# pouryashirazian/FemBrain

Measured on AMD Instinct MI355X. Metric: FEM steps/sec (assemble+PCG) at 1M tets, higher is better.
Workload: dtype f64 arithmetic / f32 stored matrix

## Files before the change

### fembrain_amd/csrc/fem_handle.h

```cpp
#pragma once
#include "comm.h"
#include "common.h"
#include "fem_kernels.h"
#include "fem_plan.h"
#include "plan_device.h"
#include "renumber.h"
#include "delta.h"
#include "subdivide.h"
#include "surface.h"
#include "haptic.h"

namespace fb {

struct PipeKernel;

struct PersistState {
  int pipe_mir_knob = -1;
  int persist_fallbacks = 0;
  int persist_launches = 0;
  int persist_rearms = 0;
  double persist_seconds = 0;
  long long persist_iterations = 0;

  int pipe_lines_nodes = 0;
  double pipe_gather_lines[2] = {0, 0};

  bool persist = false;
  int persist_blocks = 0, persist_waves = 0;
  const PipeKernel* kernel = nullptr;
  int pipe_rows = 1;
  int pipe_wmax = 0;
  int pipe_slots_dealt = 0;
  int pipe_help_waves = 0;
  int pipe_n_help = 0, pipe_help_tasks = 0;
  bool pipe_xyz = false;
  int pipe_plain_local = 0;
  int pipe_flag_extra = 0;
  int pipe_max_producers = 0;
  bool pipe_stats_pending = false;
  int pipe_timing_level = 0;
  long long persist_timeout_ticks = 0;
  bool persist_broken = false;
  int rearm_after = 32, clean_solves = 0;
  bool shard_persist = false;
  int sh_n_proxy = 1, sh_relief = 0;
  char* sbox = nullptr;
  void* sbox_opened[kP2PMaxRanks] = {nullptr};
  long long sbox_halo_cap = 0;
  int pipe_mir_got[3] = {0, 0, 0};
  bool pipe_mir_pending = false;

  DevBuf<int> pipe_wg_first;
  std::vector<int> pipe_wg_first_host;
  DevBuf<int4> pipe_mir;
  DevBuf<int> sh_halo_off, sh_row_send_off, sh_row_send_rank, sh_row_send_pos, sh_proxy_wg, sh_wg_duty;
  DevBuf<int2> sh_wg_range;
  DevBuf<unsigned int> sh_wg_send_mask;
  DevBuf<int4> pipe_tasks;
  DevBuf<long long> persist_timing;
  DevBuf<unsigned short> pipe_mir_addr;
  DevBuf<int2> pipe_mir_wg;
  DevBuf<int> pipe_mir_pool;
  DevBuf<int> pipe_mir_stats;
  DevBuf<unsigned long long> pipe_lines;
  DevBuf<unsigned long long> pipe_post;
  DevBuf<unsigned int> pipe_flags;
  DevBuf<int> pipe_prod, pipe_prod_count, pipe_prod_xcd;
  DevBuf<unsigned int> pipe_xcc;
  DevBuf<double> pipe_planes, pipe_z, pipe_s, pipe_state;
  DevBuf<int> pipe_owner, pipe_stats;
  DevBuf<unsigned int> pipe_mask;
  DevBuf<char*> sbox_peers;
  DevBuf<int> sh_peer_seg, sh_n_senders;

  void reset_plan(int rearm) {
    persist = false;
    kernel = nullptr;
    pipe_mir.release(); pipe_mir_pending = false;
    pipe_mir_got[0] = pipe_mir_got[1] = pipe_mir_got[2] = 0;
    shard_persist = false;
    persist_broken = false;
    pipe_stats_pending = false;
    clean_solves = 0;
    rearm_after = rearm;
    sh_halo_off.release(); sh_row_send_off.release(); sh_row_send_rank.release(); sh_row_send_pos.release(); sh_proxy_wg.release();
    sh_wg_duty.release(); sh_wg_range.release(); sh_wg_send_mask.release();
    pipe_wg_first_host.clear();
    pipe_wg_first.release();
  }
};

}

using namespace fb;

struct fb_fem_s {
  fb_fem_params prm;
  hipStream_t stream = nullptr;
  hipStream_t side = nullptr;
  hipEvent_t ev_side[2] = {nullptr, nullptr};
  fb_comm_s* comm = nullptr;
  P2P* p2p = nullptr;
  int xch_mode = FB_XCH_COLLECTIVE;
  DevBuf<int> send_off_dev, halo_off_dev;
  DevBuf<unsigned char> slice_halo;
  FemPlan plan;
  double lambda = 0, mu = 0;
  int grid = 8;
  bool f64 = false;
  DevBuf<int4> tets;
  DevBuf<double> x0, rest, fe;
  DevBuf<char> rec;
  DevBuf<char> kcorr;
  DevBuf<double> qacc, q1, qvel1, qacc1;
  double nm_beta = 0.25, nm_gamma = 0.5, nm_eps = 1e-6;
  int nm_max_newton = 1;
  bool pcg_warm = false;
  DevBuf<int> slice_off, colidx, slot_coff, slot_ccnt, send_local;
  DevBuf<uint32_t> contrib;
  DevBuf<short> coldelta;
  int c16 = 0;
  DevBuf<int> halo_base;
  PlanWorkspace plan_ws;
  MeshDelta delta;
  CutWork cut;
  DevBuf<double> carry;
  SurfaceWork surf;
  HapticWork hap;
  std::vector<int> fixed_caller;
  DevBuf<int4> tets_next, tets_caller;
  DevBuf<double> x0_next;
  DevBuf<int> map_next_a, map_next_b;
  int last_resync_path = FB_RESYNC_FULL;
  int ren_nodes_at_build = 0;
  DevBuf<int> flat_flag;
  DevBuf<int> inc_off;
  DevBuf<uint32_t> inc, inc_slot;
  bool asm_tets = false;
  int asm_lds = 0, asm_grid = 0, asm_max_width = 0;
  int asm_wide = 0;
  int asm_wide_slots = 0, asm_wide_grid = 0;
  DevBuf<int> wide_list;
  DevBuf<double> res_all;
  DevBuf<double> wide_scratch;
  bool asm_staged = false;
  int asm_lds_st = 0, asm_grid_st = 0;
  bool mass_valid = false;
  Renumbering ren;
  DevBuf<double> xyz_in;
  DevBuf<double> io;
  bool x0_ready = false;
  bool masks_ready = false;
  std::vector<int> l2c;
  unsigned long long order_sum = 0;
  int n_cu_device = 256;
  bool shard_auto_on = false;
  int shard_vote_neighbours = 0;
  DevBuf<int> fixed_stage;
  std::vector<int> c_bptr, c_bcol, c_src;
  bool caller_pattern = false;
  std::vector<double> x0_stage;
  DevBuf<int> d_bptr, d_bcol, d_blk_slot;
  DevBuf<unsigned int> d_ucnt;
  bool span_stale = false;
  bool csr_ready = false;
  bool device_plan = false, host_pattern = true;
  DevBuf<uint8_t> dofmask;
  DevBuf<uint8_t> nodemask;
  DevBuf<char> vals;
  DevBuf<char> dlo;
  DevBuf<double> mblk;
  DevBuf<float> volf;
  DevBuf<double> invblk;
  DevBuf<double> q, qvel, fext, fint, rhs, x, r, d, Ad, invdiag, tmp, sendbuf;
  DevBuf<double> part_a, part_b, part_c, scal;
  DevBuf<CGState> st;
  DevBuf<int> counter;
  CGState* st_host = nullptr;
  hipEvent_t ev[3] = {nullptr, nullptr, nullptr}, ev_batch[2] = {nullptr, nullptr};
  bool system_valid = false;
  bool poisoned = false;
  double last_assembly_s = 0, last_solve_s = 0;
  int split = 0;
  int sgrid = 8;
  bool spmv_nt = false;
  int vgrid = 8;
  hipGraphExec_t batch_graph = nullptr;
  const double* graph_rhs = nullptr;
  bool use_graph = true;
  bool literal_now = false, graph_literal = false;
  fb::PersistState ps;
  int last_pcg_path = 0;
  int cu_limit = 0;
  hipEvent_t ev_p[2] = {nullptr, nullptr};
};

namespace fb {

inline SellView sell_view(const fb_fem_s* h) {
  SellView sv;
  sv.slice_off = h->slice_off.p; sv.colidx = h->colidx.p; sv.n_slices = h->plan.n_slices; sv.n_owned = h->plan.n_owned;
  sv.coldelta = h->c16 ? h->coldelta.p : nullptr;
  sv.halo_base = h->c16 == 2 ? h->halo_base.p : nullptr;
  return sv;
}

#define CHECK_HANDLE(h)                                                                                                        \
  if (!(h)) return fail(FB_EINVAL, "null FEM handle");                                                                        \
  if ((h)->poisoned) return fail(FB_EINVAL, "handle unusable after a failed fb_fem_resync: re-sync it with a valid mesh or destroy it"); \
  FB_HIP(hipSetDevice((h)->prm.device))

constexpr int kZeroMax = 24;
struct ZeroBatch {
  unsigned int* p[kZeroMax]; unsigned long long end[kZeroMax]; unsigned int tail_words[kZeroMax]; int n = 0;
  hipStream_t s;
  int rc = FB_OK;
  explicit ZeroBatch(hipStream_t stream) : s(stream) {}
  void add(void* p, size_t bytes);
  template <typename T>
  void add(DevBuf<T>& b) { add(b.p, b.n * sizeof(T)); }
  int flush();
};

int assemble_system(fb_fem_s* h);

bool auto_matrix_f64(const fb_fem_s* h, int n_nodes, int n_ranks);
int setup_persist(fb_fem_s* h);
int attach_pipe_shard(fb_fem_s* h);
void release_shard_persist(fb_fem_s* h);
void read_persist_timeout(fb_fem_s* h);
int launch_pipe(fb_fem_s* h, const double* b, int start, int n_iters, double eps, int max_iter);
void print_pipe_timing(fb_fem_s* h);
// ... 4 lines not shown
```

### fembrain_amd/csrc/fem_persist.hip

```cpp
#include <cmath>
#include <cstring>

#include "fem_handle.h"
#include "pcg_pipe.hip.h"
#include "pcg_pipe2.hip.h"
#include "pcg_pipe_plan.h"

using namespace fb;

namespace fb {

struct PipeKernel {
  int rows;
  bool c16;
  int wmax, klt;
  bool timing, shard, bj, help, xyz;
  const void* fn;
};

namespace {

#define FB_PIPE1(C16, WMAX, KLT, TIMING, SHARD, BJ, HELP, XYZ) \
  {1, C16, WMAX, KLT, TIMING, SHARD, BJ, HELP, XYZ, (const void*)k_pcg_pipe<float, C16, WMAX, KLT, TIMING, SHARD, BJ, HELP, XYZ>}
#define FB_PIPE2(C16, SHARD, XYZ) {2, C16, 12, kPipe2Klt, false, SHARD, false, false, XYZ, (const void*)k_pcg_pipe2<C16, SHARD, XYZ>}
const PipeKernel kPipeKernels[] = {
    FB_PIPE1(true, 5, 16, false, false, false, false, false),  FB_PIPE1(false, 5, 16, false, false, false, false, false),
    FB_PIPE1(true, 8, 8, false, false, false, false, false),   FB_PIPE1(false, 8, 8, false, false, false, false, false),
    FB_PIPE1(true, 12, 6, false, false, false, false, false),  FB_PIPE1(false, 12, 6, false, false, false, false, false),
    FB_PIPE1(true, 12, 7, false, false, false, false, false),  FB_PIPE1(false, 12, 7, false, false, false, false, false),
    FB_PIPE1(true, 5, 16, true, false, false, false, false),
    FB_PIPE1(true, 8, 8, true, false, false, false, false),    FB_PIPE1(false, 8, 8, true, false, false, false, false),
    FB_PIPE1(true, 12, 6, true, false, false, false, false),   FB_PIPE1(false, 12, 6, true, false, false, false, false),
    FB_PIPE1(false, 8, 8, false, true, false, false, false),   FB_PIPE1(false, 12, 6, false, true, false, false, false),
    FB_PIPE1(true, 8, 8, false, false, true, false, false),    FB_PIPE1(false, 8, 8, false, false, true, false, false),
    FB_PIPE1(true, 12, 6, false, false, true, false, false),   FB_PIPE1(false, 12, 6, false, false, true, false, false),
    FB_PIPE1(true, 12, 6, false, false, false, true, false),   FB_PIPE1(false, 12, 6, false, false, false, true, false),
    FB_PIPE1(true, 12, 6, false, false, false, true, true),    FB_PIPE1(false, 12, 6, false, false, false, true, true),
    FB_PIPE1(true, 12, 6, true, false, false, true, false),    FB_PIPE1(false, 12, 6, true, false, false, true, false),
    FB_PIPE1(true, 12, 6, true, false, false, true, true),     FB_PIPE1(false, 12, 6, true, false, false, true, true),
    FB_PIPE2(true, false, false),  FB_PIPE2(false, false, false),  FB_PIPE2(true, false, true),  FB_PIPE2(false, false, true),
    FB_PIPE2(false, true, false),
};
#undef FB_PIPE2
#undef FB_PIPE1
static_assert(sizeof(double) * kPipeSyncDoubles + (size_t)kPipeMaxWaves * 2 * kPipe2LdsWordsPerRow * 64 * 4 <= 160 * 1024, "LDS budget of k_pcg_pipe2");

int env_int(const char* name, int unset) {
  const char* e = getenv(name);
  return e ? atoi(e) : unset;
}

PersistKnobs read_persist_knobs() {
  PersistKnobs k;
  k.pcg_persist = env_int("FEMBRAIN_PCG_PERSIST", -1);
  k.min_waves = env_int("FEMBRAIN_PERSIST_MIN_WAVES", 2);
  k.rows2 = env_int("FEMBRAIN_PERSIST_ROWS", 0) == 2;
  k.rearm = std::max(0, env_int("FEMBRAIN_PERSIST_REARM", 32));
  k.timing = getenv("FEMBRAIN_PERSIST_TIMING") ? std::max(1, env_int("FEMBRAIN_PERSIST_TIMING", 1)) : 0;
  k.poll_all = env_int("FEMBRAIN_PERSIST_POLL_ALL", 0) != 0;
  k.sharded = env_int("FEMBRAIN_SHARDED_PERSIST", 0) != 0;
  k.shard_relief = env_int("FEMBRAIN_SHARD_RELIEF", -1);
  k.balance = env_int("FEMBRAIN_PIPE_BALANCE", -1);
  k.small = env_int("FEMBRAIN_PIPE_SMALL", 0) != 0;
  k.klt7 = env_int("FEMBRAIN_PIPE_KLT7", 1) != 0;
  k.helpers = env_int("FEMBRAIN_PIPE_HELPERS", -1);
  k.help_minlen = env_int("FEMBRAIN_PIPE_HELP_MINLEN", 16);
  k.xyz = env_int("FEMBRAIN_PIPE_XYZ", -1);
  k.lds_by_width = env_int("FEMBRAIN_PIPE_LDS_BY_WIDTH", 0) != 0;
  k.lds_cap = getenv("FEMBRAIN_PIPE_LDS_CAP") ? std::max(1, env_int("FEMBRAIN_PIPE_LDS_CAP", 1)) : 0;
  k.plain_stores = env_int("FEMBRAIN_PIPE_PLAIN_STORES", -1);
  k.mirror = env_int("FEMBRAIN_PIPE_MIRROR", 1) != 0;
  k.verbose = getenv("FEMBRAIN_TIMING") != nullptr;
  return k;
}

int resolve_pipe_kernel(fb_fem_s* h, const PersistKnobs& kn) {
  PersistState& ps = h->ps;
  PipeKernel want;
  want.rows = ps.pipe_rows;
  want.shard = ps.shard_persist;
  want.bj = h->prm.pcg_variant == FB_PCG_BLOCK_JACOBI;
  want.help = ps.pipe_tasks.p != nullptr;
  want.xyz = ps.pipe_xyz;
  want.c16 = !want.shard && h->c16 != 0;
  want.timing = ps.persist_timing.p != nullptr && want.rows == 1;
  if (want.bj && want.timing) return fail(FB_EINVAL, "FEMBRAIN_PERSIST_TIMING is built for the Jacobi kernel");
  const bool klt7 = kn.klt7 && want.rows == 1 && ps.pipe_wmax == 12 && !want.shard && !want.bj && !want.help && !want.timing &&
                    (ps.persist_waves == 9 || ps.persist_waves == 10);
  want.wmax = ps.pipe_wmax;
  want.klt = want.rows == 2 ? kPipe2Klt : (want.wmax == 5 ? 16 : (want.wmax == 8 ? 8 : (klt7 ? 7 : 6)));
  ps.kernel = nullptr;
  for (const PipeKernel& k : kPipeKernels)
    if (k.rows == want.rows && k.c16 == want.c16 && k.wmax == want.wmax && k.klt == want.klt && k.timing == want.timing && k.shard == want.shard && k.bj == want.bj &&
        k.help == want.help && k.xyz == want.xyz)
      ps.kernel = &k;
  if (!ps.kernel) return fail(FB_EINVAL, "FEMBRAIN_PERSIST_TIMING is built for one row per lane: (12, 6) and (5, 16) with 16-bit column words, (8, 8)");
  return FB_OK;
}

int setup_persist_shard_local(fb_fem_s* h, int nb, int w, const PersistKnobs& kn) {
  const FemPlan& P = h->plan;
  PersistState& ps = h->ps;
  hipStream_t s = h->stream;
  const int R = P.n_ranks;
  if (R > kP2PMaxRanks) return FB_OK;
  FB_TRY(ps.sh_halo_off.upload(P.halo_off, s));
  DevBuf<int4> range;
  FB_TRY(range.alloc((size_t)std::max(1, P.n_slices)));
  hipLaunchKernelGGL(k_slice_colrange_shard, dim3(ceil_div(std::max(1, P.n_slices), kWavesPerBlock)), dim3(kBlock), 0, s, P.n_slices, P.n_owned, R, h->slice_off.p,
                     h->colidx.p, ps.sh_halo_off.p, range.p);
  FB_HIP(hipGetLastError());
  std::vector<int4> rg((size_t)std::max(1, P.n_slices));
  FB_TRY(range.download(rg.data(), rg.size(), s));
  std::vector<int2> wg_range;
  w = shard_deal(rg, P.n_slices, nb, w, kn, &wg_range, &ps.sh_relief);
  ps.pipe_rows = w < kPipeMaxWaves ? 1 : 2;
  ps.pipe_wmax = ps.pipe_rows == 2 ? 12 : (w < 8 ? 8 : 12);
  ps.pipe_slots_dealt = ps.pipe_rows == 2 ? std::min(kPipe2Klt, pipe2_lds_slots(w, false) / std::max(w, 1)) : std::min(ps.pipe_wmax == 8 ? 8 : 6, pipe_lds_slots(false) / std::max(w, 1));
  ps.persist_blocks = nb; ps.persist_waves = w;
  ps.pipe_flag_extra = kP2PMaxRanks * kShardProxies;
  FB_TRY(ps.sh_wg_range.upload(wg_range, s));
  FB_TRY(ps.pipe_post.alloc((size_t)2 * nb * 4));
  FB_TRY(ps.pipe_post.zero(s));
  FB_TRY(ps.pipe_flags.alloc((size_t)nb + ps.pipe_flag_extra + 16));
  FB_TRY(ps.pipe_flags.zero(s));
  const size_t n_pad = (size_t)ceil_div(P.n_local, 64) * 64, nv = (size_t)3 * P.n_local + 2;
  FB_TRY(ps.pipe_planes.alloc(2 * 3 * n_pad));
  FB_TRY(ps.pipe_planes.zero(s));
  FB_TRY(ps.pipe_z.alloc(nv));
  FB_TRY(ps.pipe_s.alloc(nv));
  FB_TRY(ps.pipe_state.alloc(2));
  FB_TRY(ps.pipe_state.zero(s));
  ps.persist_timing.release();
  std::vector<int> owner((size_t)P.n_slices, 0);
  for (int b = 0; b < nb; b++)
    for (int k = 0; k < wg_range[b].y; k++) owner[wg_range[b].x + k] = b;
  const ShardSendLists sl = shard_send_lists(P, owner, nb);
  FB_TRY(ps.sh_row_send_off.upload(sl.row_off, s));
  FB_TRY(ps.sh_row_send_rank.upload(sl.row_rank, s));
  FB_TRY(ps.sh_row_send_pos.upload(sl.row_pos, s));
  FB_TRY(ps.sh_wg_send_mask.upload(sl.wg_mask, s));
  std::vector<int> proxy, duty, prod, cnt, far((size_t)nb, 1);
  const int K = shard_proxies(P, nb, &proxy, &duty);
  ps.sh_n_proxy = K;
  FB_TRY(ps.sh_proxy_wg.upload(proxy, s));
  FB_TRY(ps.sh_wg_duty.upload(duty, s));
  ps.pipe_max_producers = shard_producers(rg, wg_range, owner, proxy, P.n_slices, nb, R, K, &prod, &cnt);
  ps.pipe_stats_pending = false;
  FB_TRY(ps.pipe_prod.upload(prod, s));
  FB_TRY(ps.pipe_prod_count.upload(cnt, s));
  FB_TRY(ps.pipe_prod_xcd.upload(far, s));
  ps.pipe_plain_local = 0;
  ps.shard_persist = true;
  return resolve_pipe_kernel(h, kn);
}

int setup_pipe_mirror(fb_fem_s* h) {
  const FemPlan& P = h->plan;
  PersistState& ps = h->ps;
  hipStream_t s = h->stream;
  const PipeKernel& K = *ps.kernel;
  ps.pipe_mir_pending = false;
  ps.pipe_mir_got[0] = ps.pipe_mir_got[1] = ps.pipe_mir_got[2] = 0;
  if (ps.pipe_mir_knob == 0 || K.rows != 1 || K.wmax != 12 || K.shard || K.help || K.bj || ps.pipe_xyz || P.n_slices <= 0) {
    ps.pipe_mir.release(); ps.pipe_mir_addr.release(); ps.pipe_mir_wg.release(); ps.pipe_mir_pool.release();
    return FB_OK;
  }
  const int nb = ps.persist_blocks;
  FB_TRY(ps.pipe_mir.alloc((size_t)nb * kMirWaves));
  FB_TRY(ps.pipe_mir_addr.alloc((size_t)P.n_slices * kMirMax * 64));
  FB_TRY(ps.pipe_mir_wg.alloc((size_t)nb));
  FB_TRY(ps.pipe_mir_pool.alloc((size_t)nb * kMirPoolMax));
  FB_TRY(ps.pipe_mir_stats.alloc(3));
  FB_HIP(hipMemsetAsync(ps.pipe_mir_stats.p, 0, 2 * sizeof(int), s));
  FB_HIP(hipMemsetAsync(ps.pipe_mir_stats.p + 2, 0x7f, sizeof(int), s));
  hipLaunchKernelGGL(k_pipe_mirror_plan, dim3(nb), dim3(64 * kMirWaves), 0, s, P.n_slices, P.n_owned, h->slice_off.p, h->colidx.p, ps.pipe_wg_first.p, K.klt,
                     h->c16 ? 1 : 0, ps.pipe_mir.p, ps.pipe_mir_addr.p, ps.pipe_mir_pool.p, ps.pipe_mir_wg.p, ps.pipe_mir_stats.p);
  FB_HIP(hipGetLastError());
  ps.pipe_mir_pending = true;
  return FB_OK;
}

int pipe_layout(fb_fem_s* h, const PersistKnobs& kn, bool* want_xyz) {
  const FemPlan& P = h->plan;
  PersistState& ps = h->ps;
  hipStream_t s = h->stream;
  *want_xyz = false;
  const bool keep_lines = ps.pipe_gather_lines[0] > 0.0 && ps.pipe_lines_nodes > 0 && std::abs(P.n_local - ps.pipe_lines_nodes) * 20 <= ps.pipe_lines_nodes;
  bool measured = keep_lines;
  if (!keep_lines) {
    ps.pipe_gather_lines[0] = ps.pipe_gather_lines[1] = 0.0;
    ps.pipe_lines_nodes = 0;
    if (P.n_local >= (1 << 24) || !h->colidx.p) return FB_OK;
    FB_TRY(ps.pipe_lines.alloc(4));
    FB_HIP(hipMemsetAsync(ps.pipe_lines.p, 0, 4 * sizeof(unsigned long long), s));
    hipLaunchKernelGGL(k_gather_lines, dim3(64), dim3(256), 0, s, P.n_slices, 8, h->slice_off.p, h->colidx.p, ps.pipe_lines.p);
    FB_HIP(hipGetLastError());
    unsigned long long got[3] = {0, 0, 0};
    FB_HIP(hipMemcpyAsync(got, ps.pipe_lines.p, sizeof got, hipMemcpyDeviceToHost, s));
    FB_HIP(hipStreamSynchronize(s));
    measured = got[2] != 0;
    if (measured) { ps.pipe_gather_lines[0] = 3.0 * (double)got[0] / (double)got[2]; ps.pipe_gather_lines[1] = (double)got[1] / (double)got[2]; ps.pipe_lines_nodes = P.n_local; }
  }
  *want_xyz = P.n_local < (1 << 24) &&
              (kn.xyz >= 0 ? kn.xyz != 0 : (measured && ps.pipe_gather_lines[0] >= 30.0 && ps.pipe_gather_lines[0] >= 1.5 * ps.pipe_gather_lines[1]));
  return FB_OK;
}

int setup_pipe_tasks(fb_fem_s* h, int nb, int w, const PersistKnobs& kn) {
  const FemPlan& P = h->plan;
  PersistState& ps = h->ps;
  int mx = 0;
  long long tot = 0;
  for (int sl = 0; sl < P.n_slices; sl++) { const int wd = P.slice_off[sl + 1] - P.slice_off[sl]; mx = std::max(mx, wd); tot += wd; }
  const double mean = P.n_slices ? (double)tot / P.n_slices : 0.0;
  const bool want_h = ps.pipe_rows == 1 && (kn.helpers >= 0 ? kn.helpers != 0 : (mx > 24 && (double)mx >= 1.5 * mean));
  bool want_xyz = false;
  FB_TRY(pipe_layout(h, kn, &want_xyz));
  ps.pipe_xyz = ps.pipe_rows == 2 && want_xyz;
  if (ps.pipe_rows != 1 || !(want_h || want_xyz) || w > kPipeMaxWaves) return FB_OK;
  const PipeTasks T = pipe_help_tasks(P.slice_off.data(), P.n_slices, ps.pipe_wg_first_host.empty() ? nullptr : ps.pipe_wg_first_host.data(), nb, w, h->c16 != 0, want_h,
                                      want_xyz, kn);
  if (!(T.all > 0 || T.deepest > 6 || want_xyz || kn.helpers == 2)) return FB_OK;
  FB_TRY(ps.pipe_tasks.upload(T.tasks, h->stream));
  ps.pipe_wmax = 12;
  ps.pipe_slots_dealt = T.deepest;
  ps.pipe_help_waves = T.help_waves; ps.pipe_n_help = T.most; ps.pipe_help_tasks = T.all;
  ps.pipe_xyz = want_xyz;
  if (kn.verbose) fprintf(stderr, "[fembrain] persistent solver: %d helper tasks (at most %d per workgroup), widest slice %d slots, mean %.1f, up to %d slots of a slice in LDS; a slot's gathers touch %.1f lines in planes, %.1f node by node -> %s\n", T.all, T.most, mx, mean, T.deepest, ps.pipe_gather_lines[0], ps.pipe_gather_lines[1], want_xyz ? "node by node" : "planes");
  return FB_OK;
}

int alloc_persist(fb_fem_s* h, int nb, const PersistKnobs& kn) {
  const FemPlan& P = h->plan;
  PersistState& ps = h->ps;
  hipStream_t s = h->stream;
  ZeroBatch zb(s);
  FB_TRY(ps.pipe_post.alloc((size_t)2 * nb * 4));
  zb.add(ps.pipe_post);
  ps.pipe_flag_extra = P.n_ranks > 1 ? kP2PMaxRanks : 0;
  FB_TRY(ps.pipe_flags.alloc((size_t)nb + ps.pipe_flag_extra + 16));
  zb.add(ps.pipe_flags);
  const size_t n_pad = (size_t)P.n_slices * 64, nv = (size_t)3 * P.n_local + 2;
  FB_TRY(ps.pipe_planes.alloc(2 * 3 * n_pad));
  zb.add(ps.pipe_planes);
  FB_TRY(ps.pipe_z.alloc(nv));
  FB_TRY(ps.pipe_s.alloc(nv));
  FB_TRY(ps.pipe_state.alloc(2));
  zb.add(ps.pipe_state);
  if (kn.timing) {
    FB_TRY(ps.persist_timing.alloc((size_t)nb * kPipeMaxWaves * kPipeTimingSlots));
    FB_TRY(ps.persist_timing.zero(s));
  } else {
    ps.persist_timing.release();
  }
  static_assert(kPipeMaxBlocks <= 256, "k_slice_producers holds 256 workgroups in its 8 mask words");
  FB_TRY(ps.pipe_owner.alloc((size_t)std::max(1, P.n_slices)));
  FB_TRY(ps.pipe_mask.alloc((size_t)std::max(1, P.n_slices) * 8));
  FB_TRY(ps.pipe_prod.alloc((size_t)nb * kPipeMaxProducers));
  FB_TRY(ps.pipe_prod_count.alloc((size_t)nb));
  FB_TRY(ps.pipe_prod_xcd.alloc((size_t)nb));
  FB_TRY(ps.pipe_stats.alloc(2));
  zb.add(ps.pipe_stats);
  FB_TRY(zb.flush());
  hipLaunchKernelGGL(k_slice_owner, dim3(ceil_div(nb, kBlock)), dim3(kBlock), 0, s, P.n_slices, nb, ps.pipe_wg_first.p, ps.pipe_owner.p);
  hipLaunchKernelGGL(k_slice_producers, dim3(ceil_div(std::max(1, P.n_slices), kWavesPerBlock)), dim3(kBlock), 0, s, P.n_slices, P.n_owned, h->slice_off.p, h->colidx.p,
                     ps.pipe_owner.p, ps.pipe_mask.p);
  hipLaunchKernelGGL(k_wg_producers, dim3(ceil_div(nb, kBlock)), dim3(kBlock), 0, s, P.n_slices, nb, ps.pipe_wg_first.p, ps.pipe_mask.p, kn.poll_all ? 1 : 0, ps.pipe_prod.p, ps.pipe_prod_count.p,
                     ps.pipe_prod_xcd.p, ps.pipe_stats.p);
  FB_HIP(hipGetLastError());
  ps.pipe_stats_pending = true;
  ps.pipe_max_producers = 0;
  FB_TRY(ps.pipe_xcc.alloc((size_t)nb));
  zb.add(ps.pipe_xcc);
  return zb.flush();
}

}

bool auto_matrix_f64(const fb_fem_s* h, int n_nodes, int n_ranks) {
  const int cus = h->cu_limit > 0 ? std::min(h->cu_limit, h->n_cu_device) : h->n_cu_device;
  const int nb = std::min(kPipeMaxBlocks, (cus / 8) * 8);
  const int w = nb >= 8 ? ceil_div(ceil_div(ceil_div(n_nodes, 64), 8), nb / 8) : 0;
  const bool shard_persist_asked = n_ranks > 1 && read_persist_knobs().sharded;
  return h->prm.pcg_variant != FB_PCG_PERSISTENT && !shard_persist_asked && w < 2;
}

void release_shard_persist(fb_fem_s* h) {
  for (auto& o : h->ps.sbox_opened) { if (o) (void)hipIpcCloseMemHandle(o); o = nullptr; }
  if (h->ps.sbox) (void)hipFree(h->ps.sbox);
  h->ps.sbox = nullptr;
  h->ps.shard_persist = false;
}

void read_persist_timeout(fb_fem_s* h) {
  const char* t = getenv("FEMBRAIN_PERSIST_TIMEOUT_MS");
  const double ms = t ? atof(t) : (h->plan.n_ranks > 1 ? 2000.0 : 50.0);
  h->ps.persist_timeout_ticks = std::max(1LL, (long long)(ms * 1e5));
}

int setup_persist(fb_fem_s* h) {
  const FemPlan& P = h->plan;
  PersistState& ps = h->ps;
  const PersistKnobs kn = read_persist_knobs();
  if (ps.pipe_mir_knob < 0) ps.pipe_mir_knob = kn.mirror ? 1 : 0;
  ps.pipe_timing_level = kn.timing;
  ps.reset_plan(kn.rearm);
  hipDeviceProp_t prop;
  FB_HIP(hipGetDeviceProperties(&prop, h->prm.device));
  const int nb = std::min(kPipeMaxBlocks, ((h->cu_limit > 0 ? std::min(h->cu_limit, prop.multiProcessorCount) : prop.multiProcessorCount) / 8) * 8);
  int w = nb >= 8 ? ceil_div(ceil_div(P.n_slices, 8), nb / 8) : 0;
  if (P.n_ranks == 1 && !P.slice_off.empty()) {
    w = pipe_deal_by_slots(P.slice_off.data(), P.n_slices, nb, w, kn, &ps.pipe_wg_first_host);
    if (!ps.pipe_wg_first_host.empty()) FB_TRY(ps.pipe_wg_first.upload(ps.pipe_wg_first_host, h->stream));
  }
  read_persist_timeout(h);
  const bool explicit_p = h->prm.pcg_variant == FB_PCG_PERSISTENT;
  const bool shard_opt = P.n_ranks > 1 && kn.sharded;
  if (explicit_p && P.n_ranks > 1 && !shard_opt) return fail(FB_EINVAL, "FB_PCG_PERSISTENT on a sharded handle needs FEMBRAIN_SHARDED_PERSIST=1 (unmeasured on multi-GPU hardware)");
  if (explicit_p && h->f64) return fail(FB_EINVAL, "FB_PCG_PERSISTENT needs FB_MATRIX_F32 storage (part of the matrix is kept in LDS as fp32 words)");
  if (explicit_p && (nb < 8 || w < 1 || w > 2 * kPipeMaxWaves))
    return fail(FB_EINVAL, "FB_PCG_PERSISTENT needs at most %d slices per CU, this mesh has %d on %d CUs", 2 * kPipeMaxWaves, w, nb);
  const bool eligible = !h->f64 && nb >= 8 && w >= 1 && (P.n_ranks == 1 ? w <= 2 * kPipeMaxWaves : (shard_opt && w <= 2 * (kPipeMaxWaves - 1)));
  const bool bj = h->prm.pcg_variant == FB_PCG_BLOCK_JACOBI;
  const bool by_default = (h->prm.pcg_variant == FB_PCG_MERGED || bj) && w >= kn.min_waves;
  const bool want_p = kn.pcg_persist >= 0 ? kn.pcg_persist != 0 && (h->prm.pcg_variant == FB_PCG_MERGED || explicit_p || bj) : (explicit_p || by_default);
  if (!want_p || !eligible) return FB_OK;
  if (bj && (w > kPipeMaxWaves || kn.rows2 || P.n_ranks > 1)) return FB_OK;
  if (P.n_ranks > 1) return setup_persist_shard_local(h, nb, w, kn);
  ps.persist = true; ps.persist_blocks = nb; ps.persist_waves = w;
  ps.pipe_rows = w > kPipeMaxWaves || kn.rows2 ? 2 : 1;
  const bool small = ps.pipe_rows == 1 && w <= 4 && !bj && kn.small;
  ps.pipe_wmax = ps.pipe_rows == 2 ? 12 : (small ? 5 : (w <= 8 ? 8 : 12));
  ps.pipe_slots_dealt = ps.pipe_rows == 2 ? std::min(kPipe2Klt, pipe2_lds_slots(w, h->c16 != 0) / std::max(w, 1))
                                          : std::min(small ? 16 : (w <= 8 ? 8 : 6), pipe_lds_slots(h->c16 != 0) / std::max(w, 1));
  ps.pipe_tasks.release();
  ps.pipe_help_waves = 0; ps.pipe_n_help = 0; ps.pipe_help_tasks = 0;
  ps.pipe_xyz = false;
  if (!bj && !small && !P.slice_off.empty()) FB_TRY(setup_pipe_tasks(h, nb, w, kn));
  FB_TRY(alloc_persist(h, nb, kn));
  ps.pipe_plain_local = kn.plain_stores >= 0 ? kn.plain_stores : (w <= 8 ? 1 : 0);
  FB_TRY(resolve_pipe_kernel(h, kn));
  return setup_pipe_mirror(h);
}

int attach_pipe_shard(fb_fem_s* h) {
  const FemPlan& P = h->plan;
  PersistState& ps = h->ps;
  const int R = P.n_ranks, me = P.rank;
  if (R < 2 || !h->comm) return FB_OK;
  const PersistKnobs kn = read_persist_knobs();
  if (!kn.sharded) return FB_OK;
  {
    const bool keep = ps.shard_persist;
    release_shard_persist(h);
    ps.shard_persist = keep;
  }
  struct Meta { hipIpcMemHandle_t handle; long long n_halo; int halo_off[kP2PMaxRanks + 1]; int senders_to[kP2PMaxRanks]; int ok; };
  Meta mine;
  memset(&mine, 0, sizeof mine);
  bool ok = ps.shard_persist && R <= kP2PMaxRanks;
  long long nh = ok ? P.n_local - P.n_owned : -1;
  std::vector<long long> nhs((size_t)R);
  FB_TRY(comm_allgather_bytes(h->comm, &nh, nhs.data(), sizeof nh, h->stream));
  long long cap = 1;
  for (int q = 0; q < R; q++) { if (nhs[q] < 0) ok = false; cap = std::max(cap, nhs[q]); }
  const ShardBoxLayout BL = shard_box_layout(cap);
  if (ok) {
    ok = hipExtMallocWithFlags((void**)&ps.sbox, BL.bytes, hipDeviceMallocFinegrained) == hipSuccess;
    ok = ok && hipMemsetAsync(ps.sbox, 0, BL.bytes, h->stream) == hipSuccess && hipStreamSynchronize(h->stream) == hipSuccess;
    ok = ok && hipIpcGetMemHandle(&mine.handle, ps.sbox) == hipSuccess;
    (void)hipGetLastError();
    mine.n_halo = P.n_local - P.n_owned;
    for (int q = 0; q <= R; q++) mine.halo_off[q] = P.halo_off[q];
    std::vector<unsigned int> wg_mask((size_t)ps.persist_blocks);
    ok = ok && ps.sh_wg_send_mask.download(wg_mask.data(), wg_mask.size(), h->stream) == FB_OK;
    for (unsigned int m : wg_mask)
      for (int q = 0; q < R; q++) mine.senders_to[q] += (m >> q) & 1u;
  }
  mine.ok = ok ? 1 : 0;
  std::vector<Meta> all((size_t)R);
  FB_TRY(comm_allgather_bytes(h->comm, &mine, all.data(), sizeof(Meta), h->stream));
  bool all_ok = true;
  for (int q = 0; q < R; q++) all_ok = all_ok && all[q].ok;
  int opened_ok = 1;
  std::vector<char*> peers((size_t)R, nullptr);
  std::vector<int> seg((size_t)R, 0), senders((size_t)R, 0);
  if (all_ok) {
    for (int q = 0; q < R; q++) {
      seg[q] = all[q].halo_off[me];
      senders[q] = all[q].senders_to[me];
      if (q == me) { peers[q] = ps.sbox; continue; }
      void* ptr = nullptr;
      if (hipIpcOpenMemHandle(&ptr, all[q].handle, hipIpcMemLazyEnablePeerAccess) != hipSuccess) { (void)hipGetLastError(); opened_ok = 0; break; }
      ps.sbox_opened[q] = ptr;
      peers[q] = (char*)ptr;
    }
  }
  std::vector<int> oks((size_t)R);
  FB_TRY(comm_allgather_bytes(h->comm, &opened_ok, oks.data(), sizeof(int), h->stream));
  for (int q = 0; q < R; q++) all_ok = all_ok && oks[q];
  if (!all_ok) { release_shard_persist(h); ps.persist = false; return FB_OK; }
  ps.sbox_halo_cap = cap;
  FB_TRY(ps.sbox_peers.upload(peers.data(), peers.size(), h->stream));
  FB_TRY(ps.sh_peer_seg.upload(seg, h->stream));
  FB_TRY(ps.sh_n_senders.upload(senders, h->stream));
  ps.persist = true;
  if (kn.verbose) fprintf(stderr, "[fembrain] rank %d: sharded persistent solver attached (%d workgroups, up to %d slices per CU, %d fewer where halo rows are gathered, %d proxies per source rank, halo %lld of cap %lld)\n", me, ps.persist_blocks, ps.persist_waves, ps.sh_relief, ps.sh_n_proxy, (long long)(P.n_local - P.n_owned), cap);
  return FB_OK;
}

int launch_pipe(fb_fem_s* h, const double* b, int start, int n_iters, double eps, int max_iter) {
  PersistState& ps = h->ps;
  if (!ps.kernel) return fail(FB_EINVAL, "internal: persistent launch on a handle whose plan resolved no kernel");
  const PipeKernel& K = *ps.kernel;
  PipeArgs pa;
  pa.post = ps.pipe_post.p; pa.flags = ps.pipe_flags.p; pa.error = ps.pipe_flags.p + ps.persist_blocks + ps.pipe_flag_extra + 4; pa.seqs = ps.pipe_flags.p + ps.persist_blocks + ps.pipe_flag_extra + 8;
  pa.producers = ps.pipe_prod.p; pa.prod_count = ps.pipe_prod_count.p; pa.prod_xcd = ps.pipe_prod_xcd.p; pa.plain_local = ps.pipe_plain_local; pa.xcc = ps.pipe_xcc.p;
  pa.start = start; pa.n_iters = n_iters; pa.eps2 = eps * eps; pa.max_iter = max_iter;
  pa.timeout_ticks = ps.persist_timeout_ticks;
  pa.timing = ps.persist_timing.p;
  pa.planes = ps.pipe_planes.p; pa.n_pad = ps.shard_persist ? (size_t)ceil_div(h->plan.n_local, 64) * 64 : (size_t)h->plan.n_slices * 64;
  pa.pstate = ps.pipe_state.p;
  pa.tasks = ps.pipe_tasks.p; pa.n_help = ps.pipe_n_help;
  pa.wg_first = ps.pipe_wg_first.p;
  pa.mirror = ps.pipe_mir.p; pa.mir_addr = ps.pipe_mir_addr.p; pa.mir_wg = ps.pipe_mir_wg.p; pa.mir_pool = ps.pipe_mir_pool.p;
  const int cwaves = K.rows == 2 ? ceil_div(ps.persist_waves, 2) : ps.persist_waves;
  pa.service = cwaves + ps.pipe_help_waves < ps.pipe_wmax ? 1 : 0;
  pa.prefetch_slots = ps.persist_waves >= 9 ? (K.rows == 2 ? 3 : 4) : 0;
  ShardArgs sa;
  memset(&sa, 0, sizeof sa);
  if (ps.shard_persist) {
    sa.rank = h->plan.rank; sa.n_ranks = h->plan.n_ranks; sa.n_owned = h->plan.n_owned; sa.n_halo = h->plan.n_local - h->plan.n_owned;
    sa.box = ps.sbox; sa.peer_box = ps.sbox_peers.p; sa.peer_seg = ps.sh_peer_seg.p; sa.halo_cap = ps.sbox_halo_cap;
    sa.halo_off = ps.sh_halo_off.p; sa.row_send_off = ps.sh_row_send_off.p; sa.row_send_rank = ps.sh_row_send_rank.p; sa.row_send_pos = ps.sh_row_send_pos.p;
    sa.wg_send_mask = ps.sh_wg_send_mask.p; sa.n_senders = ps.sh_n_senders.p; sa.proxy_wg = ps.sh_proxy_wg.p; sa.n_proxy = ps.sh_n_proxy; sa.wg_duty = ps.sh_wg_duty.p; sa.wg_range = ps.sh_wg_range.p;
    sa.delay_ticks = remote_delay_ticks();
  }
  SellView sv = sell_view(h);
  const float *vals = (const float*)h->vals.p, *dlo = (const float*)h->dlo.p;
  const double* inv = K.bj ? h->invblk.p : h->invdiag.p;
  void* args[] = {&sv, &vals, &dlo, &inv, &b, &h->x.p, &h->r.p, &h->Ad.p, &ps.pipe_z.p, &ps.pipe_s.p, &h->d.p, &h->st.p, &pa, &sa};
  const size_t lds = 160 * 1024;
  const dim3 grid(ps.persist_blocks), block(64 * (cwaves + ps.pipe_help_waves + pa.service));
  FB_HIP(hipEventRecord(h->ev_p[0], h->stream));
  FB_HIP(hipFuncSetAttribute(K.fn, hipFuncAttributeMaxDynamicSharedMemorySize, (int)lds));
  FB_HIP(hipLaunchKernel(K.fn, grid, block, args, lds, h->stream));
  FB_HIP(hipEventRecord(h->ev_p[1], h->stream));
  return FB_OK;
}

void print_pipe_timing(fb_fem_s* h) {
  std::vector<long long> tm((size_t)h->ps.persist_blocks * kPipeMaxWaves * kPipeTimingSlots);
  if (h->ps.persist_timing.download(tm.data(), tm.size(), h->stream) != FB_OK) return;
  (void)h->ps.persist_timing.zero(h->stream);
  const char* names[5] = {"publish (drained)", "flag+wait+acquire", "product", "sums sweep", "recurrences(+refresh)"};
  for (int k = 0; k < 5; k++) {
    double mn = 1e30, mx = 0, av = 0;
    int cnt = 0;
    for (int b = 0; b < h->ps.persist_blocks; b++)
      for (int w = 0; w < h->ps.persist_waves; w++) {
        const long long* t = &tm[((size_t)b * kPipeMaxWaves + w) * kPipeTimingSlots];
        if (t[5] <= 0) continue;
        const double us = (double)t[k] / (double)t[5] * 0.01;
        mn = std::min(mn, us); mx = std::max(mx, us); av += us; cnt++;
      }
    fprintf(stderr, "[fembrain] pipelined PCG %-22s per iteration: avg %.2f us  min %.2f  max %.2f (over %d waves)\n", names[k], av / std::max(cnt, 1), mn, mx, cnt);
  }
  if (h->ps.kernel && h->ps.kernel->wmax == 12 && !h->ps.kernel->help) {
    const char* parts[3] = {"product: streamed [0,a)", "product: on-chip run", "product: streamed rest"};
    for (int k = 0; k < 3; k++) {
      double av = 0, mx = 0, sav = 0;
      int cnt = 0, wgs = 0;
      for (int b = 0; b < h->ps.persist_blocks; b++) {
        double slowest = -1, part = 0;
        for (int w = 0; w < h->ps.persist_waves; w++) {
          const long long* t = &tm[((size_t)b * kPipeMaxWaves + w) * kPipeTimingSlots];
          if (t[5] <= 0) continue;
          const double us = (double)(k == 0 ? t[6] : (k == 1 ? t[7] : t[2] - t[6] - t[7])) / (double)t[5] * 0.01;
          av += us; mx = std::max(mx, us); cnt++;
          if ((double)t[2] > slowest) { slowest = (double)t[2]; part = us; }
        }
        if (slowest >= 0) { sav += part; wgs++; }
      }
      fprintf(stderr, "[fembrain] pipelined PCG %-24s per iteration: avg %.2f us  max %.2f; in the slowest wavefront of a workgroup: avg %.2f\n", parts[k], av / std::max(cnt, 1), mx,
              sav / std::max(wgs, 1));
    }
  }
  if (h->ps.pipe_timing_level >= 2) {
    for (int k = 1; k <= 2; k++) {
      fprintf(stderr, "[fembrain] %s by wavefront:", names[k]);
      for (int w = 0; w < h->ps.persist_waves; w++) {
        double av = 0; int cnt = 0;
        for (int b = 0; b < h->ps.persist_blocks; b++) { const long long* t = &tm[((size_t)b * kPipeMaxWaves + w) * kPipeTimingSlots]; if (t[5] > 0) { av += (double)t[k] / (double)t[5] * 0.01; cnt++; } }
        fprintf(stderr, " %.2f", av / std::max(cnt, 1));
      }
      fprintf(stderr, "\n[fembrain] %s by XCD (avg / max over its workgroups' slowest wavefront):", names[k]);
      for (int x = 0; x < 8; x++) {
        double av = 0, mx = 0; int cnt = 0;
        for (int b = x; b < h->ps.persist_blocks; b += 8) {
          double wmx = 0;
          for (int w = 0; w < h->ps.persist_waves; w++) { const long long* t = &tm[((size_t)b * kPipeMaxWaves + w) * kPipeTimingSlots]; if (t[5] > 0) wmx = std::max(wmx, (double)t[k] / (double)t[5] * 0.01); }
          av += wmx; mx = std::max(mx, wmx); cnt++;
        }
        fprintf(stderr, " %.2f/%.2f", av / std::max(cnt, 1), mx);
      }
      fprintf(stderr, "\n");
    }
    std::vector<std::pair<double, int>> slow;
    for (int b = 0; b < h->ps.persist_blocks; b++) {
      double wmx = 0;
      for (int w = 0; w < h->ps.persist_waves; w++) { const long long* t = &tm[((size_t)b * kPipeMaxWaves + w) * kPipeTimingSlots]; if (t[5] > 0) wmx = std::max(wmx, (double)t[2] / (double)t[5] * 0.01); }
      slow.push_back({wmx, b});
    }
    std::sort(slow.begin(), slow.end());
    fprintf(stderr, "[fembrain] slowest product of a workgroup: median %.2f us, fastest", slow[slow.size() / 2].first);
    for (int k = 0; k < 6 && k < (int)slow.size(); k++) fprintf(stderr, " wg%d %.2f", slow[k].second, slow[k].first);
    fprintf(stderr, "; slowest");
    for (int k = 0; k < 12 && k < (int)slow.size(); k++) fprintf(stderr, " wg%d %.2f", slow[slow.size() - 1 - k].second, slow[slow.size() - 1 - k].first);
    fprintf(stderr, "\n");
  }
}

int persist_plan_array(fb_fem_s* h, const char* name, std::vector<int>* out) {
  PersistState& ps = h->ps;
  const std::string n(name);
  out->clear();
  if (!ps.persist) return 0;
  if (n == "pipe_tasks" && ps.pipe_tasks.p) {
    out->resize((size_t)4 * ps.persist_blocks * kPipeTaskStride);
    FB_TRY(ps.pipe_tasks.download((int4*)out->data(), (size_t)ps.persist_blocks * kPipeTaskStride, h->stream));
    return 1;
  }
  if (n == "pipe_wg_first" && !ps.pipe_wg_first_host.empty()) { *out = ps.pipe_wg_first_host; return 1; }
  if (n == "pipe_windows" && ps.pipe_mir.p) {
    const int nb = ps.persist_blocks, ns = h->plan.n_slices;
    std::vector<int4> mt((size_t)nb * kPipeMaxWaves);
    FB_TRY(ps.pipe_mir.download(mt.data(), mt.size(), h->stream));
    out->assign((size_t)3 * ns, 0);
    for (int b = 0; b < nb; b++) {
      int first, count;
      pipe_deal(ps.pipe_wg_first_host.empty() ? nullptr : ps.pipe_wg_first_host.data(), ns, nb, b, &first, &count);
      for (int w = 0; w < count && w < kPipeMaxWaves && first + w < ns; w++) {
        const int x = mt[(size_t)b * kPipeMaxWaves + w].x;
        int* o = &(*out)[(size_t)3 * (first + w)];
        o[0] = x & 0xff; o[1] = (x >> 8) & 0xff; o[2] = (x >> 16) & 0xff;
      }
    }
    return 1;
  }
  return 0;
}

}

extern "C" {

int fb_fem_sharded_persist(fb_fem_t h) {
  if (!h) return 0;
  return h->ps.shard_persist && h->ps.persist ? 1 : 0;
}

int fb_fem_set_sharded_persist(fb_fem_t h, int on) {
  CHECK_HANDLE(h);
  if (!h->ps.shard_persist || !h->ps.sbox) return fail(FB_EINVAL, "the sharded persistent solver is not attached to this handle (FEMBRAIN_SHARDED_PERSIST=1 at creation, <= %d slices per CU)", 2 * (kPipeMaxWaves - 1));
  if (on && h->ps.persist_broken) return fail(FB_EDEVICE, "the sharded persistent solver of this handle timed out before; it stays with the two-launch iteration");
  FB_HIP(hipStreamSynchronize(h->stream));
  h->ps.persist = on != 0;
  return FB_OK;
}

int fb_fem_persist_info(fb_fem_t h, int* waves_per_cu, int* workgroups, int* lds_slots) {
  if (!h) return fail(FB_EINVAL, "null FEM handle");
  if (waves_per_cu) *waves_per_cu = h->ps.persist ? h->ps.persist_waves : 0;
  if (workgroups) *workgroups = h->ps.persist ? h->ps.persist_blocks : 0;
  if (lds_slots) {
    *lds_slots = 0;
    if (h->ps.persist) *lds_slots = h->ps.pipe_slots_dealt;
  }
  return h->ps.persist ? 1 : 0;
}

int fb_fem_pcg_path(fb_fem_t h, char* name, int name_len, int* persist_launches, int* persist_fallbacks, int* max_producers) {
  if (!h) return fail(FB_EINVAL, "null FEM handle");
  if (name && name_len > 0) {
    const PipeKernel* K = h->ps.persist ? h->ps.kernel : nullptr;
    if (!K) name[0] = 0;
    else if (K->shard && K->rows == 2) snprintf(name, name_len, "k_pcg_pipe2_shard");
    else if (K->shard) snprintf(name, name_len, "k_pcg_pipe_shard<%d,%d>", K->wmax, K->klt);
    else if (K->rows == 2) snprintf(name, name_len, "k_pcg_pipe2<%s>", K->c16 ? "c16" : "c32");
    else snprintf(name, name_len, "k_pcg_pipe<float,%s,%d,%d%s>", K->c16 ? "c16" : "c32", K->wmax, K->klt, K->bj ? ",bj" : "");
  }
  if (persist_launches) *persist_launches = h->ps.persist_launches;
  if (persist_fallbacks) *persist_fallbacks = h->ps.persist_fallbacks;
  if (max_producers && h->ps.persist && h->ps.pipe_stats_pending) {
    int st[2] = {0, 0};
    FB_TRY(h->ps.pipe_stats.download(st, 2, h->stream));
    h->ps.pipe_max_producers = st[1] ? -1 : st[0];
    h->ps.pipe_stats_pending = false;
  }
  if (max_producers) *max_producers = h->ps.persist ? h->ps.pipe_max_producers : 0;
  return h->last_pcg_path;
}

int fb_fem_persist_rearms(fb_fem_t h) { return h ? h->ps.persist_rearms : 0; }
int fb_fem_persist_helpers(fb_fem_t h) { return h && h->ps.persist ? h->ps.pipe_help_tasks : 0; }
int fb_fem_persist_mirror(fb_fem_t h, int* mirror_layers, int* pool_entries, int* plain_slots) {
  if (!h) return fail(FB_EINVAL, "null FEM handle");
  if (h->ps.pipe_mir_pending) {
    FB_TRY(h->ps.pipe_mir_stats.download(h->ps.pipe_mir_got, 3, h->stream));
    h->ps.pipe_mir_pending = false;
  }
  const bool on = h->ps.persist && h->ps.pipe_mir.p;
  if (mirror_layers) *mirror_layers = on ? h->ps.pipe_mir_got[0] : 0;
  if (pool_entries) *pool_entries = on ? h->ps.pipe_mir_got[1] : 0;
  if (plain_slots) *plain_slots = on ? h->ps.pipe_mir_got[2] : 0;
  return on && h->ps.pipe_mir_got[0] > 0 ? 1 : 0;
}

int fb_fem_persist_gather(fb_fem_t h, double* lines_planes, double* lines_records) {
  if (lines_planes) *lines_planes = h && h->ps.persist ? h->ps.pipe_gather_lines[0] : 0.0;
  if (lines_records) *lines_records = h && h->ps.persist ? h->ps.pipe_gather_lines[1] : 0.0;
  return h && h->ps.persist && h->ps.pipe_xyz ? 1 : 0;
}

int fb_fem_persist_stats(fb_fem_t h, int* launches, double* seconds, long long* iterations) {
  if (!h) return fail(FB_EINVAL, "null FEM handle");
  if (launches) *launches = h->ps.persist_launches;
  if (seconds) *seconds = h->ps.persist_seconds;
  if (iterations) *iterations = h->ps.persist_iterations;
  return FB_OK;
}

int fb_fem_time_persist(fb_fem_t h, int reps, int n_iters, double* seconds_per_launch) {
  CHECK_HANDLE(h);
  if (reps < 1 || n_iters < 1 || n_iters > 100000 || !seconds_per_launch) return fail(FB_EINVAL, "bad arguments");
  if (!h->ps.persist) return fail(FB_EINVAL, "this handle does not run the persistent PCG iterations");
  if (!h->system_valid) FB_TRY(assemble_system(h));
  double total = 0.0;
  for (int r = -1; r < reps; r++) {
    float ms = 0;
    FB_HIP(hipEventRecord(h->ev[0], h->stream));
    FB_TRY(launch_pipe(h, h->rhs.p, 1, n_iters, 1e-30, 1 << 30));
    FB_HIP(hipEventRecord(h->ev[1], h->stream));
    FB_HIP(hipStreamSynchronize(h->stream));
    FB_HIP(hipEventElapsedTime(&ms, h->ev[0], h->ev[1]));
    if (r >= 0) total += ms * 1e-3;
  }
  unsigned int err = 0;
  FB_HIP(hipMemcpy(&err, h->ps.pipe_flags.p + h->ps.persist_blocks + h->ps.pipe_flag_extra + 4, sizeof err, hipMemcpyDeviceToHost));
  if (err) {
    FB_TRY(h->ps.pipe_flags.zero(h->stream));
    FB_TRY(h->ps.pipe_post.zero(h->stream));
    if (h->ps.shard_persist) {
      h->ps.persist = false;
      h->ps.persist_broken = true;
    }
    return fail(FB_EDEVICE, "persistent PCG: a wait inside the launch timed out");
  }
  h->system_valid = false;
  *seconds_per_launch = total / reps;
  return FB_OK;
}

}
```

### fembrain_amd/csrc/pcg_pipe.hip.h

```cpp
#pragma once
#include "fem_kernels.h"
#include "pcg_pipe_stream.hip.h"
#include "pcg_pipe_onchip.hip.h"
#include "pcg_pipe_mirror.h"

namespace fb {

constexpr int kPipeMaxWaves = 12;
constexpr int kPipeMaxBlocks = 256;
constexpr int kPipeSyncDoubles = 2 * 16 + 2 * kPipeMaxBlocks + 8;
constexpr int kPipeMaxProducers = 64;
constexpr int pipe_slot_bytes(bool c16) { return c16 ? 9 * 256 + 128 : 10 * 256; }
constexpr int pipe_lds_slots(bool c16) { return c16 ? 65 : 62; }
static_assert(sizeof(double) * kPipeSyncDoubles + (size_t)pipe_lds_slots(false) * pipe_slot_bytes(false) <= 160 * 1024, "LDS budget of k_pcg_pipe");
static_assert(sizeof(double) * kPipeSyncDoubles + (size_t)pipe_lds_slots(true) * pipe_slot_bytes(true) <= 160 * 1024, "LDS budget of k_pcg_pipe<c16>");
static_assert(mir_slot_bytes(true) == pipe_slot_bytes(true) && mir_slot_bytes(false) == pipe_slot_bytes(false) && mir_lds_slots(true) == pipe_lds_slots(true) &&
              mir_lds_slots(false) == pipe_lds_slots(false) && kMirWaves == kPipeMaxWaves, "the LDS window's planner sees the kernel's LDS");
static_assert(pipe_lds_slots(true) * pipe_slot_bytes(true) / 4 < 65536 && pipe_lds_slots(false) * pipe_slot_bytes(false) / 4 < 65536, "16-bit LDS word addresses of the mirror layers");

struct PipeArgs {
  unsigned long long* post;
  unsigned int* flags;
  unsigned int* error;
  unsigned int* seqs;
  const int* producers;
  const int* prod_count;
  const int* prod_xcd;
  int plain_local;
  unsigned int* xcc;
  int prefetch_slots;
  int service;
  int start;
  int n_iters;
  double eps2;
  int max_iter;
  long long timeout_ticks;
  long long* timing;
  double* planes;
  size_t n_pad;
  double* pstate;
  const int* wg_first;
  const int4* tasks;
  int n_help;
  const int4* mirror;
  const unsigned short* mir_addr;
  const int2* mir_wg;
  const int* mir_pool;
};
constexpr int kPipeTaskStride = 16;
constexpr int kPipeTimingSlots = 8;
constexpr int kPipeMaxHelpers = 8;
constexpr int pipe_help_slots(bool c16) { return c16 ? 6 : 5; }
static_assert(pipe_help_slots(true) * pipe_slot_bytes(true) >= kPipeMaxHelpers * 3 * 64 * 8 && pipe_help_slots(false) * pipe_slot_bytes(false) >= kPipeMaxHelpers * 3 * 64 * 8, "helpers' hand-over area");

__device__ __forceinline__ void st_sc1_u64(unsigned long long* p, unsigned long long v) { __hip_atomic_store(p, v, __ATOMIC_RELAXED, __HIP_MEMORY_SCOPE_AGENT); }
__device__ __forceinline__ void st_sc1_u32(unsigned int* p, unsigned int v) { __hip_atomic_store(p, v, __ATOMIC_RELAXED, __HIP_MEMORY_SCOPE_AGENT); }
__device__ __forceinline__ unsigned int ld_sc1_u32(const unsigned int* p) { return __hip_atomic_load(p, __ATOMIC_RELAXED, __HIP_MEMORY_SCOPE_AGENT); }
__device__ __forceinline__ void st_sc1_f64(double* p, double v) { __hip_atomic_store(p, v, __ATOMIC_RELAXED, __HIP_MEMORY_SCOPE_AGENT); }
__device__ __forceinline__ void st_sc1_xyz(double* p, double x, double y, double z) {
  typedef double d2 __attribute__((ext_vector_type(2)));
  const d2 xy = {x, y};
  asm volatile("global_store_dwordx4 %0, %1, off sc1\n\tglobal_store_dwordx2 %0, %2, off offset:16 sc1" : : "v"(p), "v"(xy), "v"(z) : "memory");
}
__device__ __forceinline__ uint4 ld_sc1_u128(const void* p) {
  uint4 v;
  asm volatile("global_load_dwordx4 %0, %1, off sc1\n\ts_waitcnt vmcnt(0)" : "=v"(v) : "v"(p) : "memory");
  return v;
}

__device__ __forceinline__ double uniform_f64(double v) {
  const long long b = __double_as_longlong(v);
  const unsigned int lo = __builtin_amdgcn_readfirstlane((unsigned int)(b & 0xffffffffLL)), hi = __builtin_amdgcn_readfirstlane((unsigned int)((unsigned long long)b >> 32));
  return __longlong_as_double((long long)(((unsigned long long)hi << 32) | lo));
}
__device__ __forceinline__ bool uniform_flag(bool f) { return __builtin_amdgcn_readfirstlane(f ? 1 : 0) != 0; }

__host__ __device__ inline void pipe_slices(int n_slices, int n_blocks, int b, int* first, int* count) {
  const int xcd = b & 7, j = b >> 3, per = n_blocks >> 3;
  const int chunk = (n_slices + 7) >> 3;
  const int lo = xcd * chunk;
  int len = n_slices - lo;
  len = len < 0 ? 0 : (len > chunk ? chunk : len);
  const int base = len / per, rem = len - base * per;
  *first = lo + j * base + (j < rem ? j : rem);
  *count = base + (j < rem ? 1 : 0);
}

__host__ __device__ inline void pipe_deal(const int* wg_first, int n_slices, int n_blocks, int b, int* first, int* count) {
  if (wg_first) { *first = wg_first[b]; *count = wg_first[n_blocks + 1 + b]; }
  else pipe_slices(n_slices, n_blocks, b, first, count);
}

__global__ __launch_bounds__(kBlock) void k_slice_producers(int n_slices, int n_owned, const int* __restrict__ slice_off, const int* __restrict__ colidx,
                                                            const int* __restrict__ slice_owner, unsigned int* __restrict__ out) {
  const int s = blockIdx.x * kWavesPerBlock + (threadIdx.x >> 6), lane = threadIdx.x & 63;
  if (s >= n_slices) return;
  const int row = s * 64 + lane;
  unsigned int m[8] = {0u, 0u, 0u, 0u, 0u, 0u, 0u, 0u};
  if (row < n_owned) {
    const int k1 = slice_off[s + 1];
    for (int k0 = slice_off[s]; k0 < k1; k0 += 4) {
      int c[4], o[4];
#pragma unroll
      for (int j = 0; j < 4; j++) c[j] = k0 + j < k1 ? colidx[(size_t)(k0 + j) * 64 + lane] : n_owned;
#pragma unroll
      for (int j = 0; j < 4; j++) o[j] = c[j] < n_owned ? slice_owner[c[j] >> 6] : -1;
#pragma unroll
      for (int j = 0; j < 4; j++)
        if (o[j] >= 0) {
#pragma unroll
          for (int i = 0; i < 8; i++) m[i] |= (o[j] >> 5) == i ? 1u << (o[j] & 31) : 0u;
        }
    }
  }
#pragma unroll
  for (int i = 0; i < 8; i++) {
#pragma unroll
    for (int off = 32; off > 0; off >>= 1) m[i] |= __shfl_xor(m[i], off, 64);
    if (lane == 0) out[(size_t)s * 8 + i] = m[i];
  }
}

__global__ __launch_bounds__(kBlock) void k_slice_owner(int n_slices, int nb, const int* __restrict__ wg_first, int* __restrict__ owner) {
  const int b = blockIdx.x * kBlock + threadIdx.x;
  if (b >= nb) return;
  int first, count;
  pipe_deal(wg_first, n_slices, nb, b, &first, &count);
  for (int k = 0; k < count; k++) owner[first + k] = b;
}

__global__ __launch_bounds__(kBlock) void k_wg_producers(int n_slices, int nb, const int* __restrict__ wg_first, const unsigned int* __restrict__ mask, int poll_all,
                                                         int* __restrict__ prod, int* __restrict__ cnt, int* __restrict__ far, int* __restrict__ stats) {
  const int b = blockIdx.x * kBlock + threadIdx.x;
  if (b >= nb) return;
  int first, count;
  pipe_deal(wg_first, n_slices, nb, b, &first, &count);
  unsigned int m[8] = {0u, 0u, 0u, 0u, 0u, 0u, 0u, 0u};
  for (int k = 0; k < count; k++)
#pragma unroll
    for (int i = 0; i < 8; i++) m[i] |= mask[(size_t)(first + k) * 8 + i];
#pragma unroll
  for (int i = 0; i < 8; i++)
    if ((b >> 5) == i) m[i] &= ~(1u << (b & 31));
  int n = 0;
#pragma unroll
  for (int i = 0; i < 8; i++) n += __popc(m[i]);
  int* mine = prod + (size_t)b * kPipeMaxProducers;
  if (n > kPipeMaxProducers || poll_all) {
    for (int k = 0; k < kPipeMaxProducers; k++) mine[k] = -1;
    cnt[b] = -1; far[b] = 1;
    atomicOr(&stats[1], 1);
    return;
  }
  int k = 0, f = 0;
#pragma unroll
  for (int i = 0; i < 8; i++) {
    unsigned int w = m[i];
    while (w) {
      const int o = 32 * i + __ffs((int)w) - 1;
      w &= w - 1u;
      mine[k++] = o;
      if ((o & 7) != (b & 7)) f = 1;
    }
  }
  for (; k < kPipeMaxProducers; k++) mine[k] = -1;
  cnt[b] = n; far[b] = f;
  atomicMax(&stats[0], n);
}

__global__ __launch_bounds__(64 * kMirWaves) void k_pipe_mirror_plan(int n_slices, int n_owned, const int* __restrict__ slice_off, const int* __restrict__ colidx,
                                                                   const int* __restrict__ wg_first, int klt, int c16i, int4* __restrict__ wave_out,
                                                                   unsigned short* __restrict__ addr_out, int* __restrict__ pool_src, int2* __restrict__ wg_out,
                                                                   int* __restrict__ stats) {
  const bool c16 = c16i != 0;
  __shared__ MirWave mw[kMirWaves];
  __shared__ int cnt[kMirWaves];
  __shared__ int ok;
  const int b = blockIdx.x, nb = gridDim.x, lane = threadIdx.x & 63, w = threadIdx.x >> 6;
  int first, count;
  pipe_deal(wg_first, n_slices, nb, b, &first, &count);
  count = min(count, kMirWaves);
  const int lo = first * 64, hi = min((first + count) * 64, n_owned);
  if (w < count) {
    const int sl = first + w, width = slice_off[sl + 1] - slice_off[sl];
    const int dk = mir_lane_diag(slice_off, colidx, sl, lane, n_owned);
    int d = -1, best = 0;
    for (int k = 0; k < width; k++) {
      const int c = __popcll(__ballot(dk == k));
      if (c > best) { best = c; d = k; }
    }
    int m = 0;
    if (d >= 0)
      for (; m < kMirMax && d - 1 - m >= 0; m++)
        if (__popcll(__ballot(mir_lane_lower(slice_off, colidx, sl, d - 1 - m, lane, lo, hi))) < kMirLanes) break;
    if (lane == 0) { mw[w].d = d; mw[w].m = m; mw[w].width = width; }
  }
  __syncthreads();
  if (threadIdx.x == 0) ok = count > 0 && mir_wg_layout(mw, count, klt, c16, 0, false) ? 1 : 0;
  __syncthreads();
  for (int pass = 0; pass < 2; pass++) {
    if (ok && w < count) {
      int e = 0;
      for (int k = 0; k < mw[w].m; k++) e += __popcll(__ballot(mir_lane_addr(slice_off, colidx, first, mw, w, k, lane, lo, hi, c16) < 0));
      if (lane == 0) cnt[w] = e;
    }
    __syncthreads();
    if (threadIdx.x == 0 && ok) {
      int E = 0;
      for (int v = 0; v < count; v++) E += cnt[v];
      if (pass == 0) ok = E <= kMirPoolMax && mir_wg_layout(mw, count, klt, c16, E, true) ? 1 : 0;
      else ok = mir_wg_gains(mw, count, klt, c16) ? 1 : 0;
    }
    __syncthreads();
  }
  if (threadIdx.x == 0) {
    if (!ok) mir_wg_plain(mw, count, klt, c16);
    int E = 0, layers = 0, fewest = 1 << 30;
    for (int v = 0; v < count; v++) {
      const int e = ok ? cnt[v] : 0;
      cnt[v] = E;
      E += e; layers += mw[v].m; fewest = min(fewest, mw[v].p);
    }
    wg_out[b] = make_int2(mir_pool_at(mw, count, c16) / 4, E);
    atomicAdd(&stats[0], layers); atomicAdd(&stats[1], E);
    if (count > 0) atomicMin(&stats[2], fewest);
  }
  __syncthreads();
  if (w < count) {
    const int sl = first + w, pool_at = mir_pool_at(mw, count, c16) / 4;
    int e = cnt[w];
    for (int k = 0; k < mw[w].m; k++) {
      int addr = mir_lane_addr(slice_off, colidx, first, mw, w, k, lane, lo, hi, c16);
      const unsigned long long miss = __ballot(addr < 0);
      if (addr < 0) {
        const int idx = e + __popcll(miss & ((1ULL << lane) - 1ULL));
        pool_src[(size_t)b * kMirPoolMax + idx] = (slice_off[sl] + mw[w].a + k) * 9 * 64 + lane;
        addr = pool_at + (idx >> 6) * 9 * 64 + (idx & 63);
      }
      e += __popcll(miss);
      addr_out[((size_t)sl * kMirMax + k) * 64 + lane] = (unsigned short)addr;
    }
  }
  if (w < kMirWaves && lane == 0)
    wave_out[(size_t)b * kMirWaves + w] = w < count ? make_int4(mw[w].a | mw[w].m << 8 | mw[w].p << 16, mw[w].at, mw[w].tab, 0) : make_int4(0, 0, 0, 0);
}

__device__ __forceinline__ void pipe_collect_posts(const PipeArgs& pa, unsigned int sums, int nb, int lane, int stride, int l0, long long t0, long long t_limit, bool& failed,
                                                   double& t0s, double& t1s) {
  const unsigned long long* post = pa.post + (size_t)(sums & 1u) * nb * 4;
  for (int b = l0; b - lane < nb && !failed; b += stride) {
    const bool mine = b < nb;
    uint4 q4[2] = {make_uint4(0, 0, 0, 0), make_uint4(0, 0, 0, 0)};
    for (;;) {
      bool ok = true;
      if (mine) {
        asm volatile("global_load_dwordx4 %0, %2, off sc1\n\tglobal_load_dwordx4 %1, %2, off offset:16 sc1\n\ts_waitcnt vmcnt(0)"
                     : "=&v"(q4[0]), "=&v"(q4[1]) : "v"(post + (size_t)b * 4) : "memory");
        ok = q4[0].y == sums && q4[0].w == sums && q4[1].y == sums && q4[1].w == sums;
      }
      if (__ballot(!ok) == 0ULL) break;
      if (ld_sc1_u32(pa.error) != 0u || wall_clock64() - t0 > t_limit) { failed = true; break; }
      __builtin_amdgcn_s_sleep(1);
    }
    if (mine && !failed) {
      t0s += __longlong_as_double((long long)(((unsigned long long)q4[0].x << 32) | (unsigned long long)q4[0].z));
      t1s += __longlong_as_double((long long)(((unsigned long long)q4[1].x << 32) | (unsigned long long)q4[1].z));
    }
  }
}

__global__ __launch_bounds__(256) void k_gather_lines(int n_slices, int step, const int* __restrict__ slice_off, const int* __restrict__ colidx,
                                                      unsigned long long* __restrict__ out) {
  const int lane = threadIdx.x & 63;
  const int wave = (int)((blockIdx.x * blockDim.x + threadIdx.x) >> 6), n_waves = (int)((gridDim.x * blockDim.x) >> 6);
  unsigned long long planes = 0, records = 0, slots = 0;
  for (int s = wave * step; s < n_slices; s += n_waves * step) {
    for (int slot = slice_off[s]; slot < slice_off[s + 1]; slot++) {
      const unsigned int col = (unsigned int)colidx[(size_t)slot * 64 + lane];
      const unsigned int kp = col >> 4, k0 = (col * 24u) >> 7, k1 = (col * 24u + 23u) >> 7;
      bool first_p = true, first_0 = true, first_1 = k1 != k0;
      for (int l = 0; l < 64; l++) {
        const unsigned int op = __builtin_amdgcn_readlane(kp, l), o0 = __builtin_amdgcn_readlane(k0, l), o1 = __builtin_amdgcn_readlane(k1, l);
        if (l < lane) {
          first_p = first_p && op != kp;
          first_0 = first_0 && o0 != k0 && o1 != k0;
          first_1 = first_1 && o0 != k1 && o1 != k1;
        }
      }
      planes += __popcll(__ballot(first_p));
      records += __popcll(__ballot(first_0)) + __popcll(__ballot(first_1));
      slots++;
    }
  }
  if (lane == 0 && slots) { atomicAdd(out, planes); atomicAdd(out + 1, records); atomicAdd(out + 2, slots); }
}

}
#include "pcg_shard_box.hip.h"
namespace fb {

template <typename MT, bool C16, int WMAX, int KLT, bool TIMING, bool SHARD, bool BJ = false, bool HELP = false, bool XYZ = false>
__global__ __launch_bounds__(64 * WMAX) void k_pcg_pipe(SellView sv, const MT* __restrict__ vals, const MT* __restrict__ dlo,
                                                        const double* __restrict__ invdiag, const double* __restrict__ bvec, double* __restrict__ xg,
                                                        double* __restrict__ rg, double* __restrict__ wg, double* __restrict__ zg,
                                                        double* __restrict__ sg, double* __restrict__ pg, CGState* __restrict__ st, PipeArgs pa,
                                                        ShardArgs sa) {
  static_assert(!SHARD || (!C16 && !TIMING), "a shard's columns are 32-bit local ids; the phase clocks are built for the unsharded kernel");
  static_assert(!BJ || (!SHARD && !TIMING), "block-Jacobi is for unsharded handles");
  static_assert(!HELP || (!SHARD && !BJ), "helper wavefronts: unsharded handles, the Jacobi preconditioner");
  static_assert(sizeof(MT) == 4, "k_pcg_pipe keeps part of the matrix in LDS as fp32 words and streams the rest as fp32");
  extern __shared__ double lds[];
  double* wsum = lds;
  double* gath = lds + 32;
  double* bc = gath + 2 * kPipeMaxBlocks;
  const int n_waves = blockDim.x >> 6, nb = gridDim.x;
  if (pa.start == 0 && st->done) return;
  if (threadIdx.x == 0) bc[4] = 0.0;
  const int lane = threadIdx.x & 63, wv = threadIdx.x >> 6;
  int first, count;
  if constexpr (SHARD) { first = sa.wg_range[blockIdx.x].x; count = sa.wg_range[blockIdx.x].y; }
  else pipe_deal(pa.wg_first, sv.n_slices, nb, blockIdx.x, &first, &count);
  const bool spare = SHARD && wv == n_waves - 1;
  const bool live = wv < count && !spare;
  const int sl = first + wv;
  const int row = sl * 64 + lane;
  const bool rvalid = live && row < sv.n_owned;
  const size_t dof = 3 * (size_t)(rvalid ? row : 0);
  int so = 0, width = 0;
  if (live) { so = sv.slice_off[sl]; width = sv.slice_off[sl + 1] - so; }
  so = __builtin_amdgcn_readfirstlane(so); width = __builtin_amdgcn_readfirstlane(width);
  const MT* v = vals + (size_t)so * 9 * 64 + lane;
  const int* ci = sv.colidx + (size_t)so * 64 + lane;
  const short* cd = C16 ? sv.coldelta + (size_t)so * 64 + lane : nullptr;
  MT m00 = 0, m01 = 0, m02 = 0, m11 = 0, m12 = 0, m22 = 0;
  double iv[BJ ? 6 : 3] = {0};
  int send_beg = 0, send_end = 0;
  if (rvalid) {
    const MT* l = dlo + (size_t)sl * 9 * 64 + lane;
    m00 = l[0 * 64]; m01 = l[1 * 64]; m02 = l[2 * 64]; m11 = l[4 * 64]; m12 = l[5 * 64]; m22 = l[8 * 64];
    if constexpr (BJ) {
      const double* B = invdiag + 3 * dof;
      iv[0] = B[0]; iv[1] = B[1]; iv[2] = B[2]; iv[3] = B[4]; iv[4] = B[5]; iv[5] = B[8];
    } else {
#pragma unroll
      for (int a = 0; a < 3; a++) iv[a] = invdiag[dof + a];
    }
    if constexpr (SHARD) { send_beg = sa.row_send_off[row]; send_end = sa.row_send_off[row + 1]; }
  }
  int klt_w, lres_at;
  constexpr bool kMir = !HELP && !SHARD && !BJ && !XYZ && WMAX == 12 && (KLT == 6 || KLT == 7);
  int mir_a = 0, mir_m = 0, mir_tab = 0;
  if constexpr (HELP) {
    const int4 tk = pa.tasks[(size_t)blockIdx.x * kPipeTaskStride + wv];
    klt_w = __builtin_amdgcn_readfirstlane(live ? tk.x : 0);
    lres_at = __builtin_amdgcn_readfirstlane(live ? tk.y : 0);
  } else {
    constexpr int kSlots = pipe_lds_slots(C16);
    const int lbase = min(KLT, kSlots / max(count, 1)), lrem = lbase < KLT ? min(count, kSlots - lbase * count) : 0;
    klt_w = __builtin_amdgcn_readfirstlane(live ? lbase + (wv < lrem ? 1 : 0) : 0);
    lres_at = wv * lbase + min(wv, lrem);
    if constexpr (kMir) {
      if (pa.mirror) {
        const int4 mt = live ? pa.mirror[(size_t)blockIdx.x * kPipeMaxWaves + wv] : make_int4(0, 0, 0, 0);
        klt_w = __builtin_amdgcn_readfirstlane((mt.x >> 16) & 0xff);
        lres_at = __builtin_amdgcn_readfirstlane(mt.y);
        mir_a = __builtin_amdgcn_readfirstlane(mt.x & 0xff);
        mir_m = __builtin_amdgcn_readfirstlane((mt.x >> 8) & 0xff);
        mir_tab = __builtin_amdgcn_readfirstlane(mt.z);
      }
    }
  }
  const int kp = mir_a + mir_m, k_after = kp + klt_w;
  const int KL = min(klt_w, width - kp);
  constexpr int kValWords = C16 ? 9 : 10;
  char* lwave = (char*)(lds + kPipeSyncDoubles) + (size_t)lres_at * pipe_slot_bytes(C16);
  unsigned int* lres = (unsigned int*)lwave + lane;
  short* lcd = (short*)(lwave + (size_t)klt_w * 9 * 256) + lane;
  auto lds_col = [&](int k) -> unsigned int {
    if constexpr (C16) return (unsigned int)(row + (int)lcd[k * 64]);
    else return lres[(k * 10 + 9) * 64];
  };
  if (sizeof(MT) == 4) {
    for (int k = 0; k < KL; k++) {
      const MT* vk = v + (size_t)(kp + k) * 9 * 64;
#pragma unroll
      for (int j = 0; j < 9; j++) lres[(k * kValWords + j) * 64] = __float_as_uint((float)vk[j * 64]);
      if constexpr (C16) lcd[k * 64] = cd[(size_t)(kp + k) * 64];
      else lres[(k * 10 + 9) * 64] = (unsigned int)ci[(size_t)(kp + k) * 64];
    }
  }
  if constexpr (kMir) {
    if (pa.mirror) {
      unsigned int* lmt = (unsigned int*)((char*)(lds + kPipeSyncDoubles) + mir_tab) + lane;
      const unsigned short* ma = pa.mir_addr + (size_t)(live ? sl : 0) * kMirMax * 64 + lane;
      for (int k = 0; k < mir_m; k++) {
        const unsigned int addr = ma[k * 64];
        if constexpr (C16) lmt[k * 64] = addr << 16 | (unsigned short)cd[(size_t)(mir_a + k) * 64];
        else { lmt[k * 96] = (unsigned int)ci[(size_t)(mir_a + k) * 64]; ((unsigned short*)(lmt - lane + k * 96 + 64))[lane] = (unsigned short)addr; }
      }
      const int2 pw = pa.mir_wg[blockIdx.x];
      unsigned int* lmat = (unsigned int*)(lds + kPipeSyncDoubles);
      for (int e = threadIdx.x; e < pw.y; e += blockDim.x) {
        const MT* src = vals + pa.mir_pool[(size_t)blockIdx.x * kMirPoolMax + e];
        unsigned int* pe = lmat + pw.x + (e >> 6) * 9 * 64 + (e & 63);
#pragma unroll
        for (int j = 0; j < 9; j++) pe[(3 * (j % 3) + j / 3) * 64] = __float_as_uint((float)src[j * 64]);
      }
    }
  }
  double* ypart = (double*)((char*)(lds + kPipeSyncDoubles) + (size_t)(pipe_lds_slots(C16) - pipe_help_slots(C16)) * pipe_slot_bytes(C16));
  int own_k1 = width, help_sl = -1, hk0 = 0, hk1 = 0, help_idx = 0, help_so = 0;
  unsigned int help_mask = 0u;
  if constexpr (HELP) {
    const int4 tk = pa.tasks[(size_t)blockIdx.x * kPipeTaskStride + wv];
    const bool helper = !live && !spare && tk.x >= 0;
    own_k1 = __builtin_amdgcn_readfirstlane(live ? tk.z : width);
    help_mask = (unsigned int)__builtin_amdgcn_readfirstlane(live ? tk.w : 0);
    help_sl = __builtin_amdgcn_readfirstlane(helper ? first + tk.x : -1);
    hk0 = __builtin_amdgcn_readfirstlane(helper ? tk.y : 0); hk1 = __builtin_amdgcn_readfirstlane(helper ? tk.z : 0);
    help_idx = __builtin_amdgcn_readfirstlane(helper ? tk.w : 0);
    help_so = __builtin_amdgcn_readfirstlane(sv.slice_off[help_sl < 0 ? 0 : help_sl]);
  }
  const int n_prod = pa.prod_count[blockIdx.x];
  int my_prod = -1;
  if (wv == 0 && n_prod >= 0 && lane < n_prod) my_prod = pa.producers[(size_t)blockIdx.x * kPipeMaxProducers + lane];

  unsigned int send_mask = 0u;
  ShardBoxLayout BL = {};
  if constexpr (SHARD) { send_mask = sa.wg_send_mask[blockIdx.x]; BL = shard_box_layout(sa.halo_cap); }
  unsigned int pub = pa.seqs[0], sums = pa.seqs[1];
  const long long t_limit = pa.timeout_ticks;
  bool failed = false;
  long long tm[TIMING ? 7 : 1] = {0}, tprev = TIMING ? wall_clock64() : 0;
  auto seam = [&](int k, long long& t) { if (TIMING) { const long long u = wall_clock64(); tm[k] += u - t; t = u; } };
  auto lap = [&](int k) { if (TIMING) { const long long t = wall_clock64(); tm[k] += t - tprev; tprev = t; } };

  const bool plain_cand = !SHARD && pa.plain_local != 0 && pa.prod_xcd[blockIdx.x] == 0;
  bool through = true, xcc_known = false;
  unsigned int my_xcc = 0u;
  if constexpr (!SHARD) {
    asm volatile("s_getreg_b32 %0, hwreg(HW_REG_XCC_ID, 0, 4)" : "=s"(my_xcc));
    if (threadIdx.x == 0) st_sc1_u32(pa.xcc + blockIdx.x, ((pub + 1u) << 4) | my_xcc);
  }
  static_assert(!XYZ || HELP, "the node-by-node vector comes with the table-driven instantiation");
  const size_t xs = XYZ ? 1 : pa.n_pad, cs = XYZ ? 3 : 1;
  auto publish = [&](const double* vin) {
    pub++;
    double* pl = pa.planes + (size_t)(pub & 1u) * 3 * pa.n_pad;
    if (rvalid) {
      if (XYZ && through) {
        st_sc1_xyz(pl + 3 * (size_t)row, vin[0], vin[1], vin[2]);
      } else if (through) {
#pragma unroll
        for (int a = 0; a < 3; a++) st_sc1_f64(pl + a * xs + cs * (size_t)row, vin[a]);
      } else {
#pragma unroll
        for (int a = 0; a < 3; a++) pl[a * xs + cs * (size_t)row] = vin[a];
      }
      if constexpr (SHARD) shard_send_row(sa, BL, pub, send_beg, send_end, vin);
    }
  };
  auto product = [&](const double* vin, double* y, bool post_sums, bool late_acquire) {
    double* pl = pa.planes + (size_t)(pub & 1u) * 3 * pa.n_pad;
    asm volatile("s_waitcnt vmcnt(0)" ::: "memory");
    __syncthreads();
    lap(0);
    if (post_sums) sums++;
    if (wv != 0 && live && pa.prefetch_slots > 0 && (mir_a > 0 || own_k1 > k_after)) {
      int so_k = so + (mir_a > 0 ? 0 : k_after);
      asm volatile("" : "+s"(so_k));
      pipe_prefetch_values(min(pa.prefetch_slots, mir_a > 0 ? mir_a : own_k1 - k_after), ((unsigned int)so_k * 9u * 64u + (unsigned int)lane) * (unsigned int)sizeof(float), vals);
    }
    if constexpr (SHARD) {
      if (spare) shard_service_product(sa, BL, pa, pub, pl, nb, lane, send_mask, t_limit, bc, failed);
    }
    if (wv == 0) {
      if (lane == 0) st_sc1_u32(pa.flags + blockIdx.x, pub);
      if (post_sums && lane < 2) {
        double t = 0.0;
        for (int w = 0; w < n_waves; w++) t += wsum[lane * 16 + w];
        const unsigned long long bits = (unsigned long long)__double_as_longlong(t), tag = (unsigned long long)sums << 32;
        unsigned long long* post = pa.post + ((size_t)(sums & 1u) * nb + blockIdx.x) * 4 + 2 * lane;
        st_sc1_u64(post, (bits >> 32) | tag);
        st_sc1_u64(post + 1, (bits & 0xffffffffULL) | tag);
      }
      if (!late_acquire) __builtin_amdgcn_fence(__ATOMIC_ACQUIRE, "agent");
      const long long t0 = wall_clock64();
      if (n_prod >= 0) {
        for (;;) {
          bool ok = true;
          if (my_prod >= 0) ok = (int)(ld_sc1_u32(pa.flags + my_prod) - pub) >= 0;
          if (__ballot(!ok) == 0ULL) break;
          if (ld_sc1_u32(pa.error) != 0u || wall_clock64() - t0 > t_limit) { failed = true; break; }
          __builtin_amdgcn_s_sleep(1);
        }
      } else if constexpr (SHARD) {
        shard_poll_all(sa, pa, pub, nb, lane, t0, t_limit, failed);
      } else {
        for (int b = 4 * lane; b - 4 * lane < nb && !failed; b += 256) {
          for (;;) {
            bool ok = true;
            if (b < nb) {
              const uint4 f = ld_sc1_u128(pa.flags + b);
              ok = (int)(f.x - pub) >= 0 && (b + 1 >= nb || (int)(f.y - pub) >= 0) && (b + 2 >= nb || (int)(f.z - pub) >= 0) && (b + 3 >= nb || (int)(f.w - pub) >= 0);
            }
            if (__ballot(!ok) == 0ULL) break;
            if (ld_sc1_u32(pa.error) != 0u || wall_clock64() - t0 > t_limit) { failed = true; break; }
            __builtin_amdgcn_s_sleep(1);
          }
        }
      }
      if (failed && lane == 0) st_sc1_u32(pa.error, 1u);
      if (late_acquire) __builtin_amdgcn_fence(__ATOMIC_ACQUIRE, "agent");
      if (plain_cand && !xcc_known && !failed) {
        const bool same = my_prod < 0 || ld_sc1_u32(pa.xcc + my_prod) == ((pub << 4) | my_xcc);
        const bool all_same = __ballot(!same) == 0ULL;
        if (lane == 0) bc[5] = all_same ? 1.0 : 0.0;
      }
      asm volatile("s_waitcnt vmcnt(0)" ::: "memory");
      if (lane == 0) bc[3] = (failed || ld_sc1_u32(pa.error) != 0u) ? 1.0 : 0.0;
    }
    __syncthreads();
    lap(1);
    if (uniform_flag(bc[3] != 0.0 || (SHARD && bc[4] != 0.0))) { failed = true; return; }
    if (plain_cand && !xcc_known) { through = !uniform_flag(bc[5] != 0.0); xcc_known = true; }
    double y0 = 0, y1 = 0, y2 = 0;
    if (rvalid) {
      MT u00 = m00, u01 = m01, u02 = m02, u11 = m11, u12 = m12, u22 = m22;
      asm volatile("" : "+v"(u00), "+v"(u01), "+v"(u02), "+v"(u11), "+v"(u12), "+v"(u22));
      const double l00 = (double)u00, l01 = (double)u01, l02 = (double)u02, l11 = (double)u11, l12 = (double)u12, l22 = (double)u22;
      y0 = l00 * vin[0] + l01 * vin[1] + l02 * vin[2];
      y1 = l01 * vin[0] + l11 * vin[1] + l12 * vin[2];
      y2 = l02 * vin[0] + l12 * vin[1] + l22 * vin[2];
    }
    long long tseam = tprev;
    if (live) {
      if constexpr (kMir) {
        if (mir_a > 0) {
          int so_k = so;
          asm volatile("" : "+s"(so_k));
          pipe_stream_slots<C16, XYZ>(mir_a, ((unsigned int)so_k * 9u * 64u + (unsigned int)lane) * (unsigned int)sizeof(float),
                                      ((unsigned int)so_k * 64u + (unsigned int)lane) * (unsigned int)(C16 ? sizeof(short) : sizeof(int)), vals,
                                      C16 ? (const void*)sv.coldelta : (const void*)sv.colidx, pl, pl + xs, pl + 2 * xs, row, y0, y1, y2);
        }
        seam(5, tseam);
        const char* lbase = (const char*)(lds + kPipeSyncDoubles);
        pipe_onchip_slots<C16>(mir_m, max(KL, 0), (const unsigned int*)(lbase + mir_tab) + lane, (const unsigned short*)(lbase + mir_tab) + lane, lres, lcd, lbase, pl, pl + xs,
                               pl + 2 * xs, row, y0, y1, y2);
      }
      if (sizeof(MT) == 4 && KLT >= 16) {
        double gx[KLT][3];
#pragma unroll
        for (int k = 0; k < KLT; k++) {
          const unsigned int col = k < KL ? lds_col(k) : 0u;
          const double* xp = pl + cs * (size_t)col;
          gx[k][0] = k < KL ? xp[0] : 0.0; gx[k][1] = k < KL ? xp[xs] : 0.0; gx[k][2] = k < KL ? xp[2 * xs] : 0.0;
        }
#pragma unroll
        for (int k = 0; k < KLT; k++) if (k < KL) {
          const unsigned int* lk = lres + (size_t)k * kValWords * 64;
          const double x0 = gx[k][0], x1 = gx[k][1], x2 = gx[k][2];
          y0 += (double)__uint_as_float(lk[0 * 64]) * x0 + (double)__uint_as_float(lk[1 * 64]) * x1 + (double)__uint_as_float(lk[2 * 64]) * x2;
          y1 += (double)__uint_as_float(lk[3 * 64]) * x0 + (double)__uint_as_float(lk[4 * 64]) * x1 + (double)__uint_as_float(lk[5 * 64]) * x2;
          y2 += (double)__uint_as_float(lk[6 * 64]) * x0 + (double)__uint_as_float(lk[7 * 64]) * x1 + (double)__uint_as_float(lk[8 * 64]) * x2;
        }
      } else if (sizeof(MT) == 4 && !kMir) {
#pragma unroll
        for (int k = 0; k < KLT; k++) if (k < KL) {
          const unsigned int* lk = lres + (size_t)k * kValWords * 64;
          const double* xp = pl + cs * (size_t)lds_col(k);
          const double x0 = xp[0], x1 = xp[xs], x2 = xp[2 * xs];
          y0 += (double)__uint_as_float(lk[0 * 64]) * x0 + (double)__uint_as_float(lk[1 * 64]) * x1 + (double)__uint_as_float(lk[2 * 64]) * x2;
          y1 += (double)__uint_as_float(lk[3 * 64]) * x0 + (double)__uint_as_float(lk[4 * 64]) * x1 + (double)__uint_as_float(lk[5 * 64]) * x2;
          y2 += (double)__uint_as_float(lk[6 * 64]) * x0 + (double)__uint_as_float(lk[7 * 64]) * x1 + (double)__uint_as_float(lk[8 * 64]) * x2;
        }
        if constexpr (HELP) {
          for (int kb = KLT; kb < KL; kb += KLT) {
            double gx[KLT][3];
#pragma unroll
            for (int j = 0; j < KLT; j++) {
              const int k = min(kb + j, KL - 1);
              const double* xp = pl + cs * (size_t)lds_col(k);
              gx[j][0] = xp[0]; gx[j][1] = xp[xs]; gx[j][2] = xp[2 * xs];
            }
#pragma unroll
            for (int j = 0; j < KLT; j++) if (kb + j < KL) {
              const unsigned int* lk = lres + (size_t)(kb + j) * kValWords * 64;
              const double x0 = gx[j][0], x1 = gx[j][1], x2 = gx[j][2];
              y0 += (double)__uint_as_float(lk[0 * 64]) * x0 + (double)__uint_as_float(lk[1 * 64]) * x1 + (double)__uint_as_float(lk[2 * 64]) * x2;
              y1 += (double)__uint_as_float(lk[3 * 64]) * x0 + (double)__uint_as_float(lk[4 * 64]) * x1 + (double)__uint_as_float(lk[5 * 64]) * x2;
              y2 += (double)__uint_as_float(lk[6 * 64]) * x0 + (double)__uint_as_float(lk[7 * 64]) * x1 + (double)__uint_as_float(lk[8 * 64]) * x2;
            }
          }
        }
      }
      if constexpr (kMir) {
        if (TIMING) asm volatile("" : "+v"(y0), "+v"(y1), "+v"(y2));
        seam(6, tseam);
      }
      const int n_str = own_k1 - k_after;
      if (n_str > 0) {
        int so_k = so + k_after;
        asm volatile("" : "+s"(so_k));
        pipe_stream_slots<C16, XYZ>(n_str, ((unsigned int)so_k * 9u * 64u + (unsigned int)lane) * (unsigned int)sizeof(float),
                               ((unsigned int)so_k * 64u + (unsigned int)lane) * (unsigned int)(C16 ? sizeof(short) : sizeof(int)), vals,
                               C16 ? (const void*)sv.coldelta : (const void*)sv.colidx, pl, pl + xs, pl + 2 * xs, row, y0, y1, y2);
      }
    }
    if constexpr (HELP) if (help_sl >= 0) {
      double h0 = 0, h1 = 0, h2 = 0;
      int so_k = help_so + hk0;
      asm volatile("" : "+s"(so_k));
      if (hk1 > hk0)
      pipe_stream_slots<C16, XYZ>(hk1 - hk0, ((unsigned int)so_k * 9u * 64u + (unsigned int)lane) * (unsigned int)sizeof(float),
                             ((unsigned int)so_k * 64u + (unsigned int)lane) * (unsigned int)(C16 ? sizeof(short) : sizeof(int)), vals,
                             C16 ? (const void*)sv.coldelta : (const void*)sv.colidx, pl, pl + xs, pl + 2 * xs, help_sl * 64 + lane, h0, h1, h2);
      double* hp = ypart + (size_t)help_idx * 3 * 64 + lane;
      hp[0] = h0; hp[64] = h1; hp[128] = h2;
    }
    y[0] = y0; y[1] = y1; y[2] = y2;
    lap(2);
  };
  auto add_helpers = [&](double* y) {
    unsigned int m = help_mask;
    while (m) {
      const int hi = __ffs((int)m) - 1;
      m &= m - 1u;
      const double* hp = ypart + (size_t)hi * 3 * 64 + lane;
      y[0] += hp[0]; y[1] += hp[64]; y[2] += hp[128];
    }
  };

  double xr[3] = {0, 0, 0}, rr[3] = {0, 0, 0}, wr[3] = {0, 0, 0}, zr[3] = {0, 0, 0}, sr[3] = {0, 0, 0}, pr[3] = {0, 0, 0};
  double rho0 = 0.0, eps2 = pa.eps2, gamma_old = 1.0, alpha_old = 1.0;
  int iter = 0, max_iter = pa.max_iter;
  enum { PH_WARM_X = 0, PH_INIT_W = 1, PH_ITER = 2, PH_REFRESH_X = 3, PH_REFRESH_W = 4 };
  int phase = PH_ITER;
  bool fresh = pa.start != 0;
  if (pa.start == 0) {
    if (rvalid) {
#pragma unroll
      for (int a = 0; a < 3; a++) { xr[a] = xg[dof + a]; rr[a] = rg[dof + a]; wr[a] = wg[dof + a]; zr[a] = zg[dof + a]; sr[a] = sg[dof + a]; pr[a] = pg[dof + a]; }
    }
    rho0 = uniform_f64(st->rho0); eps2 = uniform_f64(st->eps2); iter = st->iter; max_iter = st->max_iter;
    gamma_old = uniform_f64(pa.pstate[0]); alpha_old = uniform_f64(pa.pstate[1]);
  } else if (pa.start == 2) {
    if (rvalid) {
#pragma unroll
      for (int a = 0; a < 3; a++) xr[a] = xg[dof + a];
    }
    phase = PH_WARM_X;
  } else {
    if (rvalid) {
#pragma unroll
      for (int a = 0; a < 3; a++) rr[a] = bvec[dof + a];
    }
    phase = PH_INIT_W;
  }

  auto precond = [&](const double* vv, double* out) {
    if constexpr (BJ) {
      out[0] = iv[0] * vv[0] + iv[1] * vv[1] + iv[2] * vv[2];
      out[1] = iv[1] * vv[0] + iv[3] * vv[1] + iv[4] * vv[2];
      out[2] = iv[2] * vv[0] + iv[4] * vv[1] + iv[5] * vv[2];
    } else {
#pragma unroll
      for (int a = 0; a < 3; a++) out[a] = iv[a] * vv[a];
    }
  };
  bool done = false, published = false;
  bool unsettled = true;
  double gamma = 0.0;
  int it_done = 0;
  while (!failed) {
    if (phase == PH_ITER && it_done >= pa.n_iters) break;
    double vin[3];
    if (phase == PH_WARM_X || phase == PH_REFRESH_X) {
#pragma unroll
      for (int a = 0; a < 3; a++) vin[a] = xr[a];
    } else if (phase == PH_ITER) {
      precond(wr, vin);
    } else {
      precond(rr, vin);
    }
    if (!published) publish(vin);
    published = false;
    if (phase == PH_ITER) {
      double u[3];
      precond(rr, u);
      double a0 = rr[0] * u[0] + rr[1] * u[1] + rr[2] * u[2];
      double a1 = wr[0] * u[0] + wr[1] * u[1] + wr[2] * u[2];
      a0 = wave_sum(a0); a1 = wave_sum(a1);
      int wvo = wv;
      asm volatile("" : "+v"(wvo));
      if (lane == 0) { wsum[wvo] = a0; wsum[16 + wvo] = a1; }
    }
    double y[3];
    product(vin, y, phase == PH_ITER, phase != PH_ITER || unsettled);
    unsettled = phase != PH_ITER;
    if (failed) break;
    if constexpr (HELP) if (phase != PH_ITER) {
      __syncthreads();
      add_helpers(y);
    }
    if (phase == PH_WARM_X || phase == PH_REFRESH_X) {
      unsigned int d3 = 3u * (unsigned int)(rvalid ? row : 0);
      asm volatile("" : "+v"(d3));
#pragma unroll
      for (int a = 0; a < 3; a++) rr[a] = rvalid ? bvec[d3 + a] - y[a] : 0.0;
      phase = phase == PH_WARM_X ? PH_INIT_W : PH_REFRESH_W;
      continue;
    }
    if (phase != PH_ITER) {
#pragma unroll
      for (int a = 0; a < 3; a++) wr[a] = y[a];
      phase = PH_ITER;
      continue;
    }
    if constexpr (SHARD) {
      if (spare) shard_rank_sums(sa, BL, pa, sums, nb, lane, t_limit, bc, failed);
      __syncthreads();
    } else if (pa.service) {
      if (wv == n_waves - 1) {
        const long long t0 = wall_clock64();
        double t0s = 0, t1s = 0;
        pipe_collect_posts(pa, sums, nb, lane, 64, lane, t0, t_limit, failed, t0s, t1s);
        failed = uniform_flag(failed);
        if (failed && lane == 0) st_sc1_u32(pa.error, 1u);
        t0s = wave_sum(t0s); t1s = wave_sum(t1s);
        if (lane == 0) { bc[0] = t0s; bc[1] = t1s; bc[2] = (failed || ld_sc1_u32(pa.error) != 0u) ? 1.0 : 0.0; }
      }
      __syncthreads();
    } else {
      const int pollers = min(n_waves, 4);
      if (wv < pollers) {
        const long long t0 = wall_clock64();
        const unsigned long long* post = pa.post + (size_t)(sums & 1u) * nb * 4;
        for (int b = wv * 64 + lane; b - lane < nb && !failed; b += pollers * 64) {
          const bool mine = b < nb;
          uint4 q4[2] = {make_uint4(0, 0, 0, 0), make_uint4(0, 0, 0, 0)};
          for (;;) {
            bool ok = true;
            if (mine) {
              asm volatile("global_load_dwordx4 %0, %2, off sc1\n\tglobal_load_dwordx4 %1, %2, off offset:16 sc1\n\ts_waitcnt vmcnt(0)"
                           : "=&v"(q4[0]), "=&v"(q4[1]) : "v"(post + (size_t)b * 4) : "memory");
              ok = q4[0].y == sums && q4[0].w == sums && q4[1].y == sums && q4[1].w == sums;
            }
            if (__ballot(!ok) == 0ULL) break;
            if (ld_sc1_u32(pa.error) != 0u || wall_clock64() - t0 > t_limit) { failed = true; break; }
            __builtin_amdgcn_s_sleep(1);
          }
          if (mine && !failed) {
            gath[b] = __longlong_as_double((long long)(((unsigned long long)q4[0].x << 32) | (unsigned long long)q4[0].z));
            gath[kPipeMaxBlocks + b] = __longlong_as_double((long long)(((unsigned long long)q4[1].x << 32) | (unsigned long long)q4[1].z));
// ... 97 lines not shown
```

### fembrain_amd/csrc/pcg_pipe_plan.h

```cpp
#pragma once
#include <algorithm>
#include <cstdio>
#include <cstdlib>
#include <vector>

#include "common.h"
#include "fem_plan.h"
#include "pcg_pipe2.hip.h"

namespace fb {

struct PersistKnobs {
  int pcg_persist = -1;
  int min_waves = 2;
  bool rows2 = false;
  int rearm = 32;
  int timing = 0;
  bool poll_all = false;
  bool sharded = false;
  int shard_relief = -1;
  int balance = -1;
  bool small = false;
  bool klt7 = true;
  int helpers = -1;
  int help_minlen = 16;
  int xyz = -1;
  bool lds_by_width = false;
  int lds_cap = 0;
  int plain_stores = -1;
  bool mirror = true;
  bool verbose = false;
};

inline int pipe_deal_by_slots(const int* slice_off, int n_slices, int nb, int w, const PersistKnobs& kn, std::vector<int>* wg_first) {
  wg_first->clear();
  if (nb < 8 || w < 1 || w > 2 * kPipeMaxWaves) return w;
  const int per = nb / 8, chunk = ceil_div(n_slices, 8), cap = w <= kPipeMaxWaves ? kPipeMaxWaves : 2 * kPipeMaxWaves;
  long long total = 0, worst = 0;
  for (int b = 0; b < nb; b++) {
    int first, count;
    pipe_slices(n_slices, nb, b, &first, &count);
    const long long sl = count > 0 ? slice_off[first + count] - slice_off[first] : 0;
    total += sl;
    worst = std::max(worst, sl);
  }
  int widest = 0;
  for (int sl = 0; sl < n_slices; sl++) widest = std::max(widest, slice_off[sl + 1] - slice_off[sl]);
  const bool uneven = n_slices > 0 && (long long)widest * 2 * n_slices >= 3 * (long long)slice_off[n_slices];
  const bool want = kn.balance >= 0 ? kn.balance != 0 : (uneven && (worst * nb * 4 > total * 5 || (w <= kPipeMaxWaves && worst * nb * 100 > total * 115)));
  if (!want) return w;
  std::vector<int>& tab = *wg_first;
  tab.assign((size_t)2 * nb + 2, 0);
  int most = 0;
  for (int x = 0; x < 8; x++) {
    const int lo = std::min(x * chunk, n_slices), hi = std::min((x + 1) * chunk, n_slices);
    int at = lo;
    for (int j = 0; j < per; j++) {
      const int b = x + 8 * j, left = per - j;
      const long long rest = slice_off[hi] - slice_off[at];
      const double target = (double)rest / left;
      int n = 0;
      long long cum = 0;
      const int must = std::max(0, (hi - at) - (left - 1) * cap);
      while (at + n < hi && n < cap) {
        const long long wd = slice_off[at + n + 1] - slice_off[at + n];
        if (n >= must && left > 1 && (double)cum + 0.5 * (double)wd > target) break;
        cum += wd;
        n++;
      }
      tab[b] = at;
      tab[(size_t)nb + 1 + b] = n;
      at += n;
      most = std::max(most, n);
    }
  }
  tab[nb] = n_slices;
  if (kn.verbose) fprintf(stderr, "[fembrain] persistent solver: slices dealt by slots (fullest workgroup of the equal deal: %lld slots, average %.1f); up to %d slices per workgroup\n", worst, (double)total / nb, most);
  return std::max(1, most);
}

inline void pipe_deal_lds(const std::vector<int>& wd, int lds_slots, bool by_width, int cap, std::vector<int>* res_out) {
  std::vector<int>& res = *res_out;
  const int count = (int)wd.size();
  if (!by_width) {
    const int lbase = std::min(cap, lds_slots / std::max(count, 1)), lrem = lbase < cap ? std::min(count, lds_slots - lbase * count) : 0;
    for (int j = 0; j < count; j++) res[j] = std::min(wd[j], lbase + (j < lrem ? 1 : 0));
    return;
  }
  int L = 0, widest = 0;
  for (int j = 0; j < count; j++) widest = std::max(widest, wd[j]);
  for (L = 0; L <= widest; L++) {
    int sum = 0;
    for (int j = 0; j < count; j++) sum += std::max(0, wd[j] - L);
    if (sum <= lds_slots) break;
  }
  int used = 0;
  for (int j = 0; j < count; j++) { res[j] = std::max(0, wd[j] - L); used += res[j]; }
  for (int j = 0; j < count && used < lds_slots; j++) if (res[j] < wd[j]) { res[j]++; used++; }
}

inline int pipe_deal_streams(const std::vector<int>& wd, const std::vector<int>& res, bool want_h, int waves, int min_len, int4* tk) {
  struct Stream { int wave, slice, k0, k1, floor; };
  const int count = (int)wd.size();
  std::vector<Stream> st;
  int n_h = 0;
  for (int j = 0; j < kPipeTaskStride; j++) tk[j] = make_int4(-1, 0, 0, 0);
  for (int j = 0; j < count; j++) st.push_back({j, j, 0, wd[j], res[j]});
  std::vector<unsigned> mask(count, 0u);
  for (int hw = count; want_h && hw < waves && n_h < kPipeMaxHelpers; hw++) {
    int best = -1, len = 0;
    for (int i = 0; i < (int)st.size(); i++) {
      const int l = st[i].k1 - std::max(st[i].k0, st[i].floor);
      if (l > len) { len = l; best = i; }
    }
    if (best < 0 || len < min_len) break;
    const int lo = std::max(st[best].k0, st[best].floor), mid = lo + (st[best].k1 - lo + 1) / 2;
    const Stream up = {hw, st[best].slice, mid, st[best].k1, mid};
    st[best].k1 = mid;
    st.push_back(up);
    tk[hw] = make_int4(up.slice, up.k0, up.k1, n_h);
    mask[up.slice] |= 1u << n_h;
    n_h++;
  }
  for (const Stream& S : st) {
    if (S.wave < count) tk[S.wave] = make_int4(res[S.wave], 0, S.k1, (int)mask[S.wave]);
    else { tk[S.wave].y = S.k0; tk[S.wave].z = S.k1; }
  }
  int at = 0;
  for (int j = 0; j < count; j++) { tk[j].y = at; at += res[j]; }
  return n_h;
}

struct PipeTasks {
  std::vector<int4> tasks;
  int most = 0, all = 0, deepest = 0;
  int help_waves = 0;
};
inline PipeTasks pipe_help_tasks(const int* slice_off, int n_slices, const int* wg_first, int nb, int w, bool c16, bool want_h, bool want_xyz, const PersistKnobs& kn) {
  PipeTasks T;
  T.help_waves = std::max(0, kPipeMaxWaves - w - 1);
  T.tasks.assign((size_t)nb * kPipeTaskStride, make_int4(-1, 0, 0, 0));
  const int lds_all = pipe_lds_slots(c16), lds_help = pipe_help_slots(c16);
  const int cap = kn.lds_cap > 0 ? kn.lds_cap : (want_xyz && w >= 6 ? 12 : 6);
  for (int b = 0; b < nb; b++) {
    int first, count;
    pipe_deal(wg_first, n_slices, nb, b, &first, &count);
    int4* tk = &T.tasks[(size_t)b * kPipeTaskStride];
    std::vector<int> wd(count), res(count);
    for (int j = 0; j < count; j++) wd[j] = slice_off[first + j + 1] - slice_off[first + j];
    pipe_deal_lds(wd, lds_all - lds_help, kn.lds_by_width, cap, &res);
    int n_h = pipe_deal_streams(wd, res, want_h, w + T.help_waves, kn.help_minlen, tk);
    if (n_h == 0) {
      pipe_deal_lds(wd, lds_all, kn.lds_by_width, cap, &res);
      n_h = pipe_deal_streams(wd, res, want_h, w + T.help_waves, kn.help_minlen, tk);
    }
    for (int j = 0; j < count; j++) T.deepest = std::max(T.deepest, res[j]);
    T.most = std::max(T.most, n_h);
    T.all += n_h;
  }
  return T;
}


inline int shard_deal(const std::vector<int4>& rg, int n_slices, int nb, int w, const PersistKnobs& kn, std::vector<int2>* wg_range_out, int* relief_out) {
  std::vector<int2>& wg_range = *wg_range_out;
  wg_range.assign((size_t)nb, make_int2(0, 0));
  int halo_slices = 0;
  for (int sl = 0; sl < n_slices; sl++) halo_slices += rg[sl].z != 0 ? 1 : 0;
  const int relief_default = 12 * halo_slices <= n_slices ? std::max(0, (w * 35 + 50) / 100) : 0;
  int Q = w, relief = std::min(w - 1, kn.shard_relief >= 0 ? kn.shard_relief : relief_default);
  for (;; relief--) {
    Q = 0;
    if (relief <= 0 || (nb & 7)) {
      relief = 0;
      for (int b = 0; b < nb; b++) {
        int first, count;
        pipe_slices(n_slices, nb, b, &first, &count);
        wg_range[b] = make_int2(first, count);
        Q = std::max(Q, count);
      }
      break;
    }
    const double rho = (double)w / (double)(w - relief);
// ... 94 lines not shown
```

### fembrain_amd/csrc/pcg_pipe_stream.hip.h

```cpp
#pragma once
#include <hip/hip_runtime.h>

namespace fb {

#define FBP_LOADV(r0, r1, r2, r3, r4, r5, r6, r7, r8)                      \
  "global_load_dword " r0 ", %[voff], %[svals]\n\t"                        \
  "global_load_dword " r1 ", %[voff], %[svals] offset:256\n\t"             \
  "global_load_dword " r2 ", %[voff], %[svals] offset:512\n\t"             \
  "global_load_dword " r3 ", %[voff], %[svals] offset:768\n\t"             \
  "global_load_dword " r4 ", %[voff], %[svals] offset:1024\n\t"            \
  "global_load_dword " r5 ", %[voff], %[svals] offset:1280\n\t"            \
  "global_load_dword " r6 ", %[voff], %[svals] offset:1536\n\t"            \
  "global_load_dword " r7 ", %[voff], %[svals] offset:1792\n\t"            \
  "global_load_dword " r8 ", %[voff], %[svals] offset:2048\n\t"            \
  "v_add_u32_e32 %[voff], 0x900, %[voff]\n\t"
#define FBP_LOADV_A FBP_LOADV("v136", "v137", "v138", "v139", "v140", "v141", "v142", "v143", "v144")
#define FBP_LOADV_B FBP_LOADV("v145", "v146", "v147", "v148", "v149", "v150", "v151", "v152", "v153")
#define FBP_LOADC16(c) "global_load_sshort " c ", %[coff], %[scols]\n\t" "v_add_u32_e32 %[coff], 0x80, %[coff]\n\t"
#define FBP_LOADC32(c) "global_load_dword " c ", %[coff], %[scols]\n\t" "v_add_u32_e32 %[coff], 0x100, %[coff]\n\t"
#define FBP_GOFF16(c) "v_add_u32_e32 v122, %[row], " c "\n\t" "v_lshlrev_b32_e32 v122, 3, v122\n\t"
#define FBP_GOFF32(c) "v_lshlrev_b32_e32 v122, 3, " c "\n\t"
#define FBP_GOFF16X(c) "v_add_u32_e32 v122, %[row], " c "\n\t" "v_mul_u32_u24_e32 v122, 24, v122\n\t"
#define FBP_GOFF32X(c) "v_mul_u32_u24_e32 v122, 24, " c "\n\t"
#define FBP_GATHER(g0, g1, g2)                                             \
  "global_load_dwordx2 " g0 ", v122, %[spl0]\n\t"                          \
  "global_load_dwordx2 " g1 ", v122, %[spl1]\n\t"                          \
  "global_load_dwordx2 " g2 ", v122, %[spl2]\n\t"
#define FBP_GATHER_A FBP_GATHER("v[124:125]", "v[126:127]", "v[128:129]")
#define FBP_GATHER_B FBP_GATHER("v[130:131]", "v[132:133]", "v[134:135]")
#define FBP_GATHERX(g01, g2)                                               \
  "global_load_dwordx4 " g01 ", v122, %[spl0]\n\t"                         \
  "global_load_dwordx2 " g2 ", v122, %[spl0] offset:16\n\t"
#define FBP_GATHERX_A FBP_GATHERX("v[124:127]", "v[128:129]")
#define FBP_GATHERX_B FBP_GATHERX("v[130:133]", "v[134:135]")
#define FBP_ROW(y, a, b, c, x0, x1, x2)                                    \
  "v_cvt_f64_f32_e32 v[120:121], " a "\n\t"                                \
  "v_cvt_f64_f32_e32 v[122:123], " b "\n\t"                                \
  "v_mul_f64 v[120:121], " x0 ", v[120:121]\n\t"                           \
  "v_mul_f64 v[122:123], " x1 ", v[122:123]\n\t"                           \
  "v_add_f64 v[120:121], v[120:121], v[122:123]\n\t"                       \
  "v_cvt_f64_f32_e32 v[122:123], " c "\n\t"                                \
  "v_mul_f64 v[122:123], " x2 ", v[122:123]\n\t"                           \
  "v_add_f64 v[120:121], v[120:121], v[122:123]\n\t"                       \
  "v_add_f64 " y ", " y ", v[120:121]\n\t"
#define FBP_COMPUTE_A                                                                          \
  FBP_ROW("%[y0]", "v136", "v137", "v138", "v[124:125]", "v[126:127]", "v[128:129]")           \
  FBP_ROW("%[y1]", "v139", "v140", "v141", "v[124:125]", "v[126:127]", "v[128:129]")           \
  FBP_ROW("%[y2]", "v142", "v143", "v144", "v[124:125]", "v[126:127]", "v[128:129]")
#define FBP_COMPUTE_B                                                                          \
  FBP_ROW("%[y0]", "v145", "v146", "v147", "v[130:131]", "v[132:133]", "v[134:135]")           \
  FBP_ROW("%[y1]", "v148", "v149", "v150", "v[130:131]", "v[132:133]", "v[134:135]")           \
  FBP_ROW("%[y2]", "v151", "v152", "v153", "v[130:131]", "v[132:133]", "v[134:135]")
#define FBP_FULL(LOADC, GOFF, cX, cY, LOADV_Y, GATHER_Y, COMPUTE_X, W1, W2) \
  LOADC(cX) LOADV_Y "s_waitcnt vmcnt(" W1 ")\n\t" GOFF(cY) GATHER_Y "s_waitcnt vmcnt(" W2 ")\n\t" COMPUTE_X
#define FBP_PENULT(GOFF, cY, LOADV_Y, GATHER_Y, COMPUTE_X, W3, W4)         \
  LOADV_Y "s_waitcnt vmcnt(" W3 ")\n\t" GOFF(cY) GATHER_Y "s_waitcnt vmcnt(" W4 ")\n\t" COMPUTE_X
#define FBP_LAST(COMPUTE_X) "s_waitcnt vmcnt(0)\n\t" COMPUTE_X
#define FBP_BODY(LOADC, GOFF) FBP_BODYG(LOADC, GOFF, FBP_GATHER_A, FBP_GATHER_B, "22", "13", "21", "12")
#define FBP_BODYG(LOADC, GOFF, GATHER_A, GATHER_B, W1, W2, W3, W4)                                                                                 \
           \
  "s_nop 4\n\t"                                                                                                 \
                         \
  LOADC("v154")                                                                                                 \
  "s_cmp_lt_i32 %[n], 2\n\t"                                                                                    \
  "s_cbranch_scc1 .Lfbp_one_%=\n\t"                                                                             \
  LOADC("v155")                                                                                                 \
  FBP_LOADV_A                                                                                                   \
  "s_waitcnt vmcnt(10)\n\t"                                                                                     \
  "s_branch .Lfbp_g0_%=\n"                                                                                      \
  ".Lfbp_one_%=:\n\t"                                                                                           \
  FBP_LOADV_A                                                                                                   \
  "s_waitcnt vmcnt(9)\n"                                                                                        \
  ".Lfbp_g0_%=:\n\t"                                                                                            \
  GOFF("v154") GATHER_A                                                                                     \
                                                                                 \
  ".Lfbp_even_%=:\n\t"                                                                                          \
  "s_cmp_lt_i32 %[n], 3\n\t"                                                                                    \
  "s_cbranch_scc1 .Lfbp_even_tail_%=\n\t"                                                                       \
  FBP_FULL(LOADC, GOFF, "v154", "v155", FBP_LOADV_B, GATHER_B, FBP_COMPUTE_A, W1, W2)                               \
  "s_sub_i32 %[n], %[n], 1\n\t"                                                                                 \
                                                                                  \
  "s_cmp_lt_i32 %[n], 3\n\t"                                                                                    \
  "s_cbranch_scc1 .Lfbp_odd_tail_%=\n\t"                                                                        \
  FBP_FULL(LOADC, GOFF, "v155", "v154", FBP_LOADV_A, GATHER_A, FBP_COMPUTE_B, W1, W2)                               \
  "s_sub_i32 %[n], %[n], 1\n\t"                                                                                 \
  "s_branch .Lfbp_even_%=\n"                                                                                    \
  ".Lfbp_even_tail_%=:\n\t"                                                                                     \
  "s_cmp_lt_i32 %[n], 2\n\t"                                                                                    \
  "s_cbranch_scc1 .Lfbp_even_last_%=\n\t"                                                                       \
  FBP_PENULT(GOFF, "v155", FBP_LOADV_B, GATHER_B, FBP_COMPUTE_A, W3, W4)                                            \
  FBP_LAST(FBP_COMPUTE_B)                                                                                       \
  "s_branch .Lfbp_end_%=\n"                                                                                     \
  ".Lfbp_even_last_%=:\n\t"                                                                                     \
  FBP_LAST(FBP_COMPUTE_A)                                                                                       \
  "s_branch .Lfbp_end_%=\n"                                                                                     \
  ".Lfbp_odd_tail_%=:\n\t"                                                                                      \
  "s_cmp_lt_i32 %[n], 2\n\t"                                                                                    \
  "s_cbranch_scc1 .Lfbp_odd_last_%=\n\t"                                                                        \
  FBP_PENULT(GOFF, "v154", FBP_LOADV_A, GATHER_A, FBP_COMPUTE_B, W3, W4)                                            \
  FBP_LAST(FBP_COMPUTE_A)                                                                                       \
  "s_branch .Lfbp_end_%=\n"                                                                                     \
  ".Lfbp_odd_last_%=:\n\t"                                                                                      \
  FBP_LAST(FBP_COMPUTE_B)                                                                                       \
  ".Lfbp_end_%=:\n\t"
#define FBP_CLOBBERS                                                                                                                   \
  "memory", "scc", "v120", "v121", "v122", "v123", "v124", "v125", "v126", "v127", "v128", "v129", "v130", "v131", "v132", "v133",      \
  "v134", "v135", "v136", "v137", "v138", "v139", "v140", "v141", "v142", "v143", "v144", "v145", "v146", "v147", "v148", "v149",      \
  "v150", "v151", "v152", "v153", "v154", "v155"

__device__ __forceinline__ void pipe_prefetch_values(int n, unsigned int voff, const float* vals);

template <typename T>
__device__ __forceinline__ T* scalar_ptr(T* p) {
  const unsigned long long b = (unsigned long long)p;
  const unsigned int lo = __builtin_amdgcn_readfirstlane((unsigned int)b), hi = __builtin_amdgcn_readfirstlane((unsigned int)(b >> 32));
  return (T*)(((unsigned long long)hi << 32) | lo);
}

__device__ __forceinline__ void pipe_prefetch_values(int n, unsigned int voff, const float* vals) {
  vals = scalar_ptr(vals);
  n = __builtin_amdgcn_readfirstlane(n);
  asm volatile("s_nop 4\n\t"
               "s_cmp_lt_i32 %[n], 1\n\t"
               "s_cbranch_scc1 .Lfbp_pf_end_%=\n\t"
               FBP_LOADV("v120", "v121", "v122", "v123", "v124", "v125", "v126", "v127", "v128")
               "s_cmp_lt_i32 %[n], 2\n\t"
               "s_cbranch_scc1 .Lfbp_pf_wait_%=\n\t"
               FBP_LOADV("v129", "v130", "v131", "v132", "v133", "v134", "v135", "v136", "v137")
               "s_cmp_lt_i32 %[n], 3\n\t"
               "s_cbranch_scc1 .Lfbp_pf_wait_%=\n\t"
               FBP_LOADV("v138", "v139", "v140", "v141", "v142", "v143", "v144", "v145", "v146")
               "s_cmp_lt_i32 %[n], 4\n\t"
               "s_cbranch_scc1 .Lfbp_pf_wait_%=\n\t"
               FBP_LOADV("v147", "v148", "v149", "v150", "v151", "v152", "v153", "v154", "v155")
               ".Lfbp_pf_wait_%=:\n\t"
               "s_waitcnt vmcnt(0)\n"
               ".Lfbp_pf_end_%=:\n\t"
               : [voff] "+v"(voff)
               : [n] "s"(n), [svals] "s"(vals)
               : FBP_CLOBBERS);
}

template <bool C16, bool XYZ = false>
__device__ __forceinline__ void pipe_stream_slots(int n, unsigned int voff, unsigned int coff, const float* vals, const void* cols, const double* pl0,
                                                  const double* pl1, const double* pl2, int row, double& y0, double& y1, double& y2) {
  vals = scalar_ptr(vals); cols = scalar_ptr(cols); pl0 = scalar_ptr(pl0); pl1 = scalar_ptr(pl1); pl2 = scalar_ptr(pl2);
  n = __builtin_amdgcn_readfirstlane(n);
  if (C16 && XYZ) {
    asm volatile(FBP_BODYG(FBP_LOADC16, FBP_GOFF16X, FBP_GATHERX_A, FBP_GATHERX_B, "21", "12", "20", "11")
                 : [y0] "+v"(y0), [y1] "+v"(y1), [y2] "+v"(y2), [voff] "+v"(voff), [coff] "+v"(coff), [n] "+s"(n)
                 : [svals] "s"(vals), [scols] "s"(cols), [spl0] "s"(pl0), [spl1] "s"(pl1), [spl2] "s"(pl2), [row] "v"(row)
                 : FBP_CLOBBERS);
  } else if (XYZ) {
    asm volatile(FBP_BODYG(FBP_LOADC32, FBP_GOFF32X, FBP_GATHERX_A, FBP_GATHERX_B, "21", "12", "20", "11")
                 : [y0] "+v"(y0), [y1] "+v"(y1), [y2] "+v"(y2), [voff] "+v"(voff), [coff] "+v"(coff), [n] "+s"(n)
                 : [svals] "s"(vals), [scols] "s"(cols), [spl0] "s"(pl0), [spl1] "s"(pl1), [spl2] "s"(pl2), [row] "v"(row)
                 : FBP_CLOBBERS);
  } else if (C16) {
    asm volatile(FBP_BODY(FBP_LOADC16, FBP_GOFF16)
                 : [y0] "+v"(y0), [y1] "+v"(y1), [y2] "+v"(y2), [voff] "+v"(voff), [coff] "+v"(coff), [n] "+s"(n)
                 : [svals] "s"(vals), [scols] "s"(cols), [spl0] "s"(pl0), [spl1] "s"(pl1), [spl2] "s"(pl2), [row] "v"(row)
                 : FBP_CLOBBERS);
  } else {
    asm volatile(FBP_BODY(FBP_LOADC32, FBP_GOFF32)
                 : [y0] "+v"(y0), [y1] "+v"(y1), [y2] "+v"(y2), [voff] "+v"(voff), [coff] "+v"(coff), [n] "+s"(n)
                 : [svals] "s"(vals), [scols] "s"(cols), [spl0] "s"(pl0), [spl1] "s"(pl1), [spl2] "s"(pl2), [row] "v"(row)
                 : FBP_CLOBBERS);
  }
}

}
```

### fembrain_amd/csrc/plan_api.cpp

```cpp
#include <cstring>
#include <string>
#include <vector>

#include "../../include/fembrain_hip.h"
#include "../../include/fembrain_hip_testing.h"
#include "fem_plan.h"
#include "renumber.h"
#include "pcg_pipe_mirror.h"

namespace fb {
int fail(int code, const char* fmt, ...);
}

struct fb_plan_s {
  fb::FemPlan plan;
};

extern "C" {

int fb_plan_create(fb_plan_t* out, int n_nodes, int n_tets, const int* tets, int n_fixed_dofs, const int* fixed_dofs, int n_ranks,
                   int rank, const int* node_splits) {
  if (!out) return fb::fail(FB_EINVAL, "null output");
  fb_plan_s* p = new fb_plan_s;
  int rc = fb::build_fem_plan(p->plan, n_nodes, n_tets, tets, n_fixed_dofs, fixed_dofs, n_ranks, rank, node_splits);
  if (rc != FB_OK) {
    delete p;
    return rc;
  }
  *out = p;
  return FB_OK;
}

int fb_plan_destroy(fb_plan_t p) {
  delete p;
  return FB_OK;
}

int fb_plan_info(fb_plan_t p, int info[12]) {
  if (!p || !info) return fb::fail(FB_EINVAL, "null argument");
  const fb::FemPlan& P = p->plan;
  const int v[12] = {P.n_owned, P.n_halo, P.n_tets, P.n_blocks, P.n_slices, P.n_slots, P.n_crows, (int)P.send_local.size(),
                     P.node_lo, P.node_hi, P.n_fixed_owned, P.n_ranks};
  memcpy(info, v, sizeof v);
  return FB_OK;
}

int fb_plan_get(fb_plan_t p, const char* name, int* out, size_t capacity) {
  if (!p || !name) return fb::fail(FB_EINVAL, "null argument");
  const fb::FemPlan& P = p->plan;
  const std::string n(name);
  const std::vector<int>* v = nullptr;
  std::vector<int> tmp;
  if (n == "local2global") v = &P.local2global;
  else if (n == "halo_off") v = &P.halo_off;
  else if (n == "send_off") v = &P.send_off;
  else if (n == "send_local") v = &P.send_local;
  else if (n == "tets") v = &P.tets;
  else if (n == "tet_global") v = &P.tet_global;
  else if (n == "bptr") v = &P.bptr;
  else if (n == "bcol") v = &P.bcol;
  else if (n == "slice_off") v = &P.slice_off;
  else if (n == "colidx") v = &P.colidx;
  else if (n == "blk_slot") v = &P.blk_slot;
  else if (n == "slot_coff") v = &P.slot_coff;
  else if (n == "slot_ccnt") v = &P.slot_ccnt;
  else if (n == "contrib") { tmp.assign(P.contrib.begin(), P.contrib.end()); v = &tmp; }
  else if (n == "dofmask") { tmp.assign(P.dofmask.begin(), P.dofmask.end()); v = &tmp; }
  else return fb::fail(FB_EINVAL, "unknown plan array '%s'", name);
  if (out) {
    if (capacity < v->size()) return fb::fail(FB_EINVAL, "capacity %zu < %zu", capacity, v->size());
    memcpy(out, v->data(), v->size() * sizeof(int));
  }
  return (int)v->size();
}

int fb_plan_slab_order(int n_nodes, const double* xyz, int n_tets, const int* tets, int* old_of_new, int* span_caller, int* span_internal) {
  if (!xyz || !tets || !old_of_new || n_nodes < 1 || n_tets < 0) return fb::fail(FB_EINVAL, "bad argument");
  std::vector<int> o;
  const int rc = fb::host_slab_order(n_nodes, xyz, n_tets, tets, o, span_caller, span_internal);
  if (rc != FB_OK) return rc;
  memcpy(old_of_new, o.data(), sizeof(int) * (size_t)n_nodes);
  return FB_OK;
}

int fb_plan_shard_vote(int n_nodes, int n_tets, const int* tets, int n_ranks, int rank, const int* node_splits, int out[3]) {
  if (!tets || !out) return fb::fail(FB_EINVAL, "null argument");
  unsigned long long sum = 0;
  int splits_sum = 0;
  fb::shard_neighbour_count(n_nodes, n_tets, tets, n_ranks, rank, node_splits, &out[0], &sum, &splits_sum, &out[1], &out[2]);
  return FB_OK;
}

int fb_plan_mirror_model(fb_plan_t p, int nb, int c16, int klt, int out[4]) {
  if (!p || !out || nb < 8 || (nb & 7) || (klt != 6 && klt != 7)) return fb::fail(FB_EINVAL, "bad argument");
  const fb::FemPlan& P = p->plan;
  const int* so = P.slice_off.data();
  const int* ci = P.colidx.data();
  out[0] = out[1] = out[3] = 0;
  out[2] = 1 << 30;
  for (int b = 0; b < nb; b++) {
    const int xcd = b & 7, j = b >> 3, per = nb >> 3, chunk = (P.n_slices + 7) >> 3, lo_s = xcd * chunk;
    int len = P.n_slices - lo_s;
    len = len < 0 ? 0 : (len > chunk ? chunk : len);
    const int base = len / per, rem = len - base * per;
    const int first = lo_s + j * base + (j < rem ? j : rem);
    const int count = std::min(base + (j < rem ? 1 : 0), fb::kMirWaves);
    if (count <= 0) continue;
    const int lo = first * 64, hi = std::min((first + count) * 64, P.n_owned);
    fb::MirWave mw[fb::kMirWaves];
    for (int w = 0; w < count; w++) {
      const int sl = first + w, width = so[sl + 1] - so[sl];
      int hist[256] = {0};
      for (int l = 0; l < 64; l++) {
        const int dk = fb::mir_lane_diag(so, ci, sl, l, P.n_owned);
        if (dk >= 0 && dk < 256) hist[dk]++;
      }
      int d = -1, best = 0;
      for (int k = 0; k < width && k < 256; k++)
        if (hist[k] > best) { best = hist[k]; d = k; }
      int m = 0;
      if (d >= 0)
        for (; m < fb::kMirMax && d - 1 - m >= 0; m++) {
          int n = 0;
          for (int l = 0; l < 64; l++) n += fb::mir_lane_lower(so, ci, sl, d - 1 - m, l, lo, hi) ? 1 : 0;
          if (n < fb::kMirLanes) break;
        }
      mw[w].d = d; mw[w].m = m; mw[w].width = width;
    }
    auto misses = [&]() {
      int e = 0;
      for (int w = 0; w < count; w++)
        for (int k = 0; k < mw[w].m; k++)
          for (int l = 0; l < 64; l++) e += fb::mir_lane_addr(so, ci, first, mw, w, k, l, lo, hi, c16 != 0) < 0 ? 1 : 0;
      return e;
    };
    bool ok = fb::mir_wg_layout(mw, count, klt, c16 != 0, 0, false);
    int E = ok ? misses() : 0;
    ok = ok && E <= fb::kMirPoolMax && fb::mir_wg_layout(mw, count, klt, c16 != 0, E, true);
    if (ok) { E = misses(); ok = fb::mir_wg_gains(mw, count, klt, c16 != 0); }
    if (!ok) { fb::mir_wg_plain(mw, count, klt, c16 != 0); E = 0; }
    for (int w = 0; w < count; w++) { out[0] += mw[w].m; out[2] = std::min(out[2], mw[w].p); }
    out[1] += E;
    out[3] += ok ? 1 : 0;
  }
  return FB_OK;
}

}
```

### fembrain_amd/fem.py

```python
import ctypes as C

import numpy as np

from . import lib as _l
from .meshgen import fixed_vertices_to_dofs


class FemIntegrator:
    def __init__(self, verts, tets, fixed_dofs=(), E=1e7, nu=0.46, rho=1000.0, timestep=0.0333,
                 damping_mass=0.0, damping_stiffness=0.01, cg_eps=1e-6, cg_max_iter=10000,
                 matrix_precision=_l.FB_MATRIX_AUTO, device=0, shard=None, pcg_variant=_l.FB_PCG_MERGED, spmv_kernel=_l.FB_SPMV_AUTO,
                 linear=False, exact_tangent=False, integrator=_l.FB_INTEGRATOR_VOLUME_CONSERVING, renumber=_l.FB_RENUMBER_AUTO, expect_cuts=False,
                 reserve_nodes=0, reserve_elements=0):
        L = _l.lib()
        self._L = L
        self.verts = np.ascontiguousarray(verts, dtype=np.float64).reshape(-1, 3)
        self.tets = np.ascontiguousarray(tets, dtype=np.int32).reshape(-1, 4)
        self.n_nodes, self.n_tets_global = len(self.verts), len(self.tets)
        self.r = 3 * self.n_nodes
        fd = _l.as_i32(fixed_dofs)
        p = _l.FemParams()
        L.fb_fem_default_params(C.byref(p))
        p.E, p.nu, p.rho, p.timestep = E, nu, rho, timestep
        p.damping_mass, p.damping_stiffness = damping_mass, damping_stiffness
# ... 193 lines not shown

    def set_external_forces_to_zero(self):
        _l.check(self._L.fb_fem_set_external_forces_zero(self.h))

    def set_uniform_force(self, axis, value):
        _l.check(self._L.fb_fem_set_uniform_force(self.h, axis, value))

    def do_timestep(self):
        _l.check(self._L.fb_fem_step(self.h, C.byref(self.last)))
        return self.last.cg_iterations

    def get_q_state(self):
        q, qv, qa = np.zeros(self.r), np.zeros(self.r), np.zeros(self.r)
        _l.check(self._L.fb_fem_get_state(self.h, _l.dptr(q), _l.dptr(qv), _l.dptr(qa)))
        return q, qv, qa

    def set_q_state(self, q, qvel=None, qaccel=None):
        qv = None if qvel is None else _l.as_f64(qvel, self.r)
        qa = None if qaccel is None else _l.as_f64(qaccel, self.r)
        _l.check(self._L.fb_fem_set_state(self.h, _l.dptr(_l.as_f64(q, self.r)), _l.dptr(qv), _l.dptr(qa)))

    def set_newmark(self, beta=0.25, gamma=0.5, max_newton_iterations=1, epsilon=1e-6):
        _l.check(self._L.fb_fem_set_newmark(self.h, beta, gamma, max_newton_iterations, epsilon))

    def reset_to_rest(self):
        _l.check(self._L.fb_fem_reset(self.h))

    def set_timestep(self, h):
        _l.check(self._L.fb_fem_set_timestep(self.h, h))

    def set_damping(self, mass_coef, stiffness_coef):
        _l.check(self._L.fb_fem_set_damping(self.h, mass_coef, stiffness_coef))

    def set_internal_force_scaling_factor(self, factor):
        _l.check(self._L.fb_fem_set_internal_force_scaling(self.h, factor))

    def set_cg(self, eps, max_iter):
        _l.check(self._L.fb_fem_set_cg(self.h, eps, max_iter))

    def set_constrained_dofs(self, fixed_dofs):
        fd = _l.as_i32(fixed_dofs)
        _l.check(self._L.fb_fem_set_constrained_dofs(self.h, len(fd), _l.iptr(fd)))

    def get_force_assembly_time(self):
        return self.last.assembly_seconds

    def get_system_solve_time(self):
        return self.last.solve_seconds

    def floor_collision(self, floor_y, restitution=0.4):
        n = C.c_int(0)
        _l.check(self._L.fb_fem_floor_collision(self.h, floor_y, restitution, C.byref(n)))
        return n.value

    def add_haptic_forces(self, indices, forces, neighborhood_size):
        ids = _l.as_i32(indices)
        f = _l.as_f64(forces, 3 * len(ids))
        _l.check(self._L.fb_fem_add_haptic_forces(self.h, len(ids), _l.iptr(ids), _l.dptr(f), int(neighborhood_size)))

    def pick_vertex(self, wpos):
        w = _l.as_f64(wpos, 3)
        idx, xyz, d2 = C.c_int(-1), np.zeros(3), C.c_double(0)
        _l.check(self._L.fb_fem_pick_vertex(self.h, _l.dptr(w), C.byref(idx), _l.dptr(xyz), C.byref(d2)))
        return idx.value, xyz, d2.value

    def pick_box(self, lo, hi, capacity=None, ids=None, xyz=None):
        lo, hi = _l.as_f64(lo, 3), _l.as_f64(hi, 3)
        cap = self.n_nodes if capacity is None else int(capacity)
        n = C.c_int(0)
        if cap == 0:
            _l.check(self._L.fb_fem_pick_box(self.h, _l.dptr(lo), _l.dptr(hi), 0, None, None, C.byref(n)))
            return n.value, None, None
        ids = np.zeros(cap, np.int32) if ids is None else ids
        xyz = np.zeros((cap, 3)) if xyz is None else xyz
        if ids.dtype != np.int32 or xyz.dtype != np.float64 or ids.size < cap or xyz.size < 3 * cap or not (ids.flags.c_contiguous and xyz.flags.c_contiguous):
            raise ValueError("ids: contiguous int32 of at least capacity, xyz: contiguous float64 of at least 3 capacity")
        _l.check(self._L.fb_fem_pick_box(self.h, _l.dptr(lo), _l.dptr(hi), cap, _l.iptr(ids), _l.dptr(xyz), C.byref(n)))
        m = min(n.value, cap)
        return n.value, ids.reshape(-1)[:m], xyz.reshape(-1)[:3 * m].reshape(m, 3)

    def volume(self, per_element=False):
        t = C.c_double(0)
        pe = np.zeros(int(self._L.fb_fem_num_tets(self.h))) if per_element else None
        _l.check(self._L.fb_fem_volume(self.h, C.byref(t), _l.dptr(pe)))
        return (t.value, pe) if per_element else t.value

    def num_tets(self):
        return self._L.fb_fem_num_tets(self.h)

    def num_blocks(self):
        return self._L.fb_fem_num_blocks(self.h)

    def matrix_precision(self):
        return int(self._L.fb_fem_matrix_precision(self.h))

    def pattern(self):
        n_owned = self.node_hi - self.node_lo
        bptr, bcol = np.empty(n_owned + 1, np.int32), np.empty(self.num_blocks(), np.int32)
        _l.check(self._L.fb_fem_pattern(self.h, _l.iptr(bptr), _l.iptr(bcol)))
        return bptr, bcol

    def element_stiffness(self, first, count):
        K0, Mi = np.empty((count, 12, 12)), np.empty((count, 4, 4))
        _l.check(self._L.fb_fem_element_stiffness(self.h, first, count, _l.dptr(K0), _l.dptr(Mi)))
        return K0, Mi

    def assemble(self, u):
        f, K = np.zeros(self.r), np.empty((self.num_blocks(), 3, 3))
        _l.check(self._L.fb_fem_assemble(self.h, _l.dptr(_l.as_f64(u, self.r)), _l.dptr(f), _l.dptr(K)))
        return f, K

    def system(self):
        rhs, K = np.zeros(self.r), np.empty((self.num_blocks(), 3, 3))
        _l.check(self._L.fb_fem_system(self.h, _l.dptr(K), _l.dptr(rhs)))
        return K, rhs

    def mass(self):
        m = np.empty(self.num_blocks())
        _l.check(self._L.fb_fem_mass(self.h, _l.dptr(m)))
        return m

    def spmv(self, x):
        y = np.zeros(self.r)
        _l.check(self._L.fb_fem_spmv(self.h, _l.dptr(_l.as_f64(x, self.r)), _l.dptr(y)))
        return y

    def pcg(self, rhs, eps=1e-6, max_iter=10000):
        x, it = np.zeros(self.r), C.c_int(0)
        _l.check(self._L.fb_fem_pcg(self.h, _l.dptr(_l.as_f64(rhs, self.r)), _l.dptr(x), eps, max_iter, C.byref(it)))
        return it.value, x

    def time_spmv(self, reps=50):
        s = C.c_double(0)
        _l.check(self._L.fb_fem_time_spmv(self.h, reps, C.byref(s)))
        return s.value

    def persist_info(self):
        w, b, k = C.c_int(0), C.c_int(0), C.c_int(0)
        on = self._L.fb_fem_persist_info(self.h, C.byref(w), C.byref(b), C.byref(k))
        return bool(on == 1), w.value, b.value, k.value

    def persist_gather(self):
        a, b = C.c_double(0), C.c_double(0)
        on = self._L.fb_fem_persist_gather(self.h, C.byref(a), C.byref(b))
        return bool(on), a.value, b.value

    def persist_mirror(self):
        m, p, k = C.c_int(0), C.c_int(0), C.c_int(0)
        on = self._L.fb_fem_persist_mirror(self.h, C.byref(m), C.byref(p), C.byref(k))
        if on < 0:
            _l.check(on)
        return bool(on == 1), m.value, p.value, k.value

    def pcg_path(self):
        name = C.create_string_buffer(96)
        nl, nf, mp = C.c_int(0), C.c_int(0), C.c_int(0)
        path = self._L.fb_fem_pcg_path(self.h, name, 96, C.byref(nl), C.byref(nf), C.byref(mp))
        return dict(path=path, kernel=name.value.decode(), launches=nl.value, fallbacks=nf.value, max_producers=mp.value)

    def persist_stats(self):
        n, sec, it = C.c_int(0), C.c_double(0), C.c_longlong(0)
        _l.check(self._L.fb_fem_persist_stats(self.h, C.byref(n), C.byref(sec), C.byref(it)))
        return n.value, sec.value, it.value

    def time_persist(self, reps=10, n_iters=29):
        s = C.c_double(0)
        _l.check(self._L.fb_fem_time_persist(self.h, reps, n_iters, C.byref(s)))
        return s.value

    def iteration_bytes(self):
        b = C.c_double(0)
        _l.check(self._L.fb_fem_iteration_bytes(self.h, C.byref(b)))
        return b.value

    def time_assembly(self, reps=10):
        s = C.c_double(0)
        _l.check(self._L.fb_fem_time_assembly(self.h, reps, C.byref(s)))
        return s.value

    def spmv_bytes(self):
        b = C.c_double(0)
        _l.check(self._L.fb_fem_spmv_bytes(self.h, C.byref(b)))
        return b.value

    def assembly_bytes(self):
        b = C.c_double(0)
        _l.check(self._L.fb_fem_assembly_bytes(self.h, C.byref(b)))
        return b.value


def bsr_to_scipy(bptr, bcol, blocks, n_cols_nodes=None):
    import scipy.sparse as sp
    n_rows = len(bptr) - 1
    n_cols = n_cols_nodes if n_cols_nodes is not None else n_rows
    return sp.bsr_matrix((np.asarray(blocks).reshape(-1, 3, 3), bcol, bptr), shape=(3 * n_rows, 3 * n_cols)).tocsr()


def spread_haptic_forces(bptr, bcol, indices, forces, neighborhood_size, ext_forces):
    for idx, frc in zip(indices, forces):
        ext_forces[3 * idx:3 * idx + 3] += frc
    for idx, frc in zip(indices, forces):
        affected, last = {int(idx)}, {int(idx)}
        for j in range(1, neighborhood_size):
            mag = 1.0 * (neighborhood_size - j) / float(neighborhood_size)
            new = set()
            for vtx in last:
                for nb in bcol[bptr[vtx]:bptr[vtx + 1]]:
                    nb = int(nb)
                    if nb != vtx and nb not in affected:
                        new.add(nb)
            last = set()
            for nb in sorted(new):
                ext_forces[3 * nb:3 * nb + 3] += mag * np.asarray(frc, dtype=np.float64)
                last.add(nb)
                affected.add(nb)
    return ext_forces


class Deformable:

    GRAVITY_FORCE = -10000.0

    def __init__(self, verts, tets, fixed_vertices=(), floor_y=None, gravity=True, haptic_on_device=True, **kw):
        self.fixed_vertices = sorted(int(v) for v in fixed_vertices)
        fd = fixed_vertices_to_dofs(self.fixed_vertices) if len(self.fixed_vertices) else np.zeros(0, np.int32)
        self.integrator = FemIntegrator(verts, tets, fd, **kw)
        self.dof = self.integrator.r
        self.gravity = bool(gravity)
        self.floor_y = floor_y
        self.ct_collided = 0
        self.ct_timestep = 0
        self.haptic_indices, self.haptic_forces = [], []
        self.haptic_in_progress = False
        self.haptic_force_neighborhood_size = 5
        self._pattern = None
        self.haptic_on_device = bool(haptic_on_device) and kw.get("shard") is None
        self.on_deform = None

    def set_deform_callback(self, fn):
        self.on_deform = fn

    def haptic_set_current_forces(self, indices, forces):
        self.haptic_indices, self.haptic_forces = list(indices), [tuple(f) for f in forces]

    def set_haptic_force_radius(self, radius):
        self.haptic_force_neighborhood_size = int(radius)

    def get_haptic_force_radius(self):
        return self.haptic_force_neighborhood_size

    def haptic_start(self, index):
        self.haptic_in_progress = True

    def haptic_end(self):
        self.haptic_in_progress = False
        self.haptic_indices, self.haptic_forces = [], []

    def timestep(self):
        it = self.integrator
        apply_gravity = self.gravity and self.ct_collided == 0
        if self.haptic_in_progress and self.haptic_indices and self.haptic_on_device and len(self.haptic_indices) <= _l.FB_HAPTIC_MAX_SOURCES:
            if apply_gravity:
                it.set_uniform_force(1, self.GRAVITY_FORCE)
            else:
                it.set_external_forces_to_zero()
            it.add_haptic_forces(self.haptic_indices, self.haptic_forces, self.haptic_force_neighborhood_size)
        elif self.haptic_in_progress and self.haptic_indices:
            if self.dof != it.r:
                self.dof, self._pattern = it.r, None
            f = np.zeros(self.dof)
            if apply_gravity:
                f[1::3] += self.GRAVITY_FORCE
            if self._pattern is None:
                self._pattern = it.pattern()
            spread_haptic_forces(self._pattern[0], self._pattern[1], self.haptic_indices, self.haptic_forces,
                                 self.haptic_force_neighborhood_size, f)
            it.set_external_forces(f)
        elif apply_gravity:
            it.set_uniform_force(1, self.GRAVITY_FORCE)
        else:
            it.set_external_forces_to_zero()
        iters = it.do_timestep()
        if self.floor_y is not None:
            self.ct_collided = it.floor_collision(self.floor_y, 0.4)
        self.ct_timestep += 1
        if self.on_deform is not None:
            q, _, _ = it.get_q_state()
            self.on_deform(self.dof, q)
        return iters

    def get_solver_time(self):
        return self.integrator.get_system_solve_time()

    def surface_mesh(self, update=False):
        return self.integrator.surface_update() if update else self.integrator.surface()

    def reset_deformations(self):
        self.integrator.reset_to_rest()

    def cut(self, strip, mode="bake"):
        info, delta = self.integrator.cut(strip, mode=mode)
        self.dof, self._pattern = self.integrator.r, None
        return info, delta

    def _positions(self):
        it = self.integrator
# ... 35 lines not shown
```

### fembrain_amd/lib.py

```python
import ctypes as C
import os
import subprocess

import numpy as np

_HERE = os.path.dirname(os.path.abspath(__file__))
LIB_PATH = os.path.join(_HERE, "libfembrain_hip.so")

FB_OK, FB_EINVAL, FB_EDEVICE, FB_ENOMEM, FB_ESOLVER, FB_ECOMM = 0, -1, -2, -3, -4, -5
FB_MATRIX_F32, FB_MATRIX_F64, FB_MATRIX_AUTO = 0, 1, 2
FB_XCH_COLLECTIVE, FB_XCH_P2P, FB_XCH_P2P_SUMS, FB_XCH_P2P_FUSED = 1, 2, 3, 4
FB_PCG_MERGED, FB_PCG_REFERENCE, FB_PCG_PERSISTENT, FB_PCG_BLOCK_JACOBI = 0, 1, 3, 4
FB_PCG_PATH_TWO_LAUNCH, FB_PCG_PATH_PERSISTENT, FB_PCG_PATH_FALLBACK, FB_PCG_PATH_RESOLVED = 0, 1, 2, 3
FB_SPMV_AUTO, FB_SPMV_ROWS, FB_SPMV_SPLIT = 0, 1, 2
FB_INTEGRATOR_VOLUME_CONSERVING, FB_INTEGRATOR_NEWMARK = 0, 1
FB_RENUMBER_AUTO, FB_RENUMBER_ON, FB_RENUMBER_OFF = 0, 1, -1
FB_RESYNC_FULL, FB_RESYNC_DELTA_MERGED, FB_RESYNC_DELTA_REBUILT = 0, 1, 2
FB_CUT_BAKE, FB_CUT_CARRY = 0, 1
FB_CUT_NOTHING, FB_CUT_DONE, FB_CUT_UNHANDLED, FB_CUT_DRY = 0, 1, 2, 3
FB_CUT_UNHANDLED_IDS = 64
FB_HAPTIC_MAX_SOURCES = 256

_dp = C.POINTER(C.c_double)
_fp = C.POINTER(C.c_float)
# ... 4 lines not shown

class FbError(RuntimeError):
    def __init__(self, code, text):
        super().__init__("fembrain_hip error %d: %s" % (code, text))
        self.code = code


class FemParams(C.Structure):
    _fields_ = [("E", C.c_double), ("nu", C.c_double), ("rho", C.c_double), ("timestep", C.c_double),
                ("damping_mass", C.c_double), ("damping_stiffness", C.c_double), ("cg_eps", C.c_double),
                ("cg_max_iter", C.c_int), ("matrix_precision", C.c_int), ("device", C.c_int),
                ("pcg_variant", C.c_int), ("spmv_kernel", C.c_int), ("linear", C.c_int), ("exact_tangent", C.c_int), ("integrator", C.c_int), ("renumber", C.c_int),
                ("expect_cuts", C.c_int), ("reserve_nodes", C.c_int), ("reserve_elements", C.c_int)]


class StepInfo(C.Structure):
    _fields_ = [("cg_iterations", C.c_int), ("converged", C.c_int), ("assembly_seconds", C.c_double),
                ("solve_seconds", C.c_double), ("rho0", C.c_double), ("rho", C.c_double), ("pcg_path", C.c_int),
                ("persist_fallbacks", C.c_int), ("newton_iterations", C.c_int)]


class CutResult(C.Structure):
    _fields_ = [("status", C.c_int), ("n_quads", C.c_int), ("n_cut_edges", C.c_int), ("n_case_a", C.c_int), ("n_case_b", C.c_int),
                ("n_unhandled", C.c_int), ("n_removed", C.c_int), ("n_added", C.c_int), ("n_new_nodes", C.c_int), ("min_volume_ratio", C.c_double)]


class SurfaceInfo(C.Structure):
    _fields_ = [("n_faces", C.c_int), ("n_vertices", C.c_int), ("n_builds", C.c_int), ("aabb_lo", C.c_float * 3), ("aabb_hi", C.c_float * 3)]


class PolyCounts(C.Structure):
    _fields_ = [("grid", C.c_int * 3), ("n_points", C.c_int), ("n_cells", C.c_int), ("n_crossed_edges", C.c_int),
                ("n_surface_cells", C.c_int), ("n_included_cells", C.c_int),
                ("n_tet_vertices", C.c_int), ("n_tets", C.c_int), ("n_surface_vertices", C.c_int),
                ("n_surface_indices", C.c_int)]


def source_sha256(part=None):
    import hashlib
    h = hashlib.sha256()
    d = os.path.join(_HERE, "csrc")
    for name in sorted(os.listdir(d)):
        if not name.endswith((".hip", ".h", ".cpp")):
            continue
        if part == "fem" and name in ("poly.hip", "cut.hip"):
            continue
        if part == "poly" and name not in ("poly.hip", "common.h"):
            continue
        h.update(name.encode())
        h.update(open(os.path.join(d, name), "rb").read())
    return h.hexdigest()


def build(force=False):
    mk = os.path.join(_HERE, "csrc", "Makefile")
    if force:
        subprocess.check_call(["make", "-s", "-f", mk, "clean"])
    subprocess.check_call(["make", "-s", "-j4", "-f", mk])


_lib = None


def lib():
    global _lib
    if _lib is not None:
        return _lib
    if not os.path.exists(LIB_PATH):
        raise FbError(FB_EDEVICE, "%s is missing: run `python -c 'import __graft_entry__ as g; g.build()'` "
                                  "(there is no CPU fallback for the HIP path)" % LIB_PATH)
    L = C.CDLL(LIB_PATH)
    L.fb_last_error.restype = C.c_char_p
    vp = C.c_void_p
    sig = {
        "fb_device_count": (C.c_int, []),
        "fb_device_info": (C.c_int, [C.c_int, C.c_char_p, C.c_int, C.c_char_p, C.c_int, _ip]),
        "fb_host_register": (C.c_int, [C.c_void_p, C.c_ulonglong]),
        "fb_host_unregister": (C.c_int, [C.c_void_p]),
        "fb_fem_default_params": (None, [C.POINTER(FemParams)]),
        "fb_fem_create": (C.c_int, [C.POINTER(vp), C.c_int, _dp, C.c_int, _ip, C.c_int, _ip, C.POINTER(FemParams)]),
        "fb_fem_create_sharded": (C.c_int, [C.POINTER(vp), C.c_int, _dp, C.c_int, _ip, C.c_int, _ip, C.POINTER(FemParams),
                                            C.c_int, C.c_int, _ip, vp]),
        "fb_fem_destroy": (C.c_int, [vp]),
        "fb_fem_resync": (C.c_int, [vp, C.c_int, _dp, C.c_int, _ip, C.c_int, _ip]),
        "fb_fem_resync_sharded": (C.c_int, [vp, C.c_int, _dp, C.c_int, _ip, C.c_int, _ip, _ip]),
        "fb_fem_resync_delta": (C.c_int, [vp, C.c_int, _ip, C.c_int, _ip, _ip, C.c_int, _ip, C.c_int, _dp, C.c_int, _ip]),
        "fb_fem_resync_path": (C.c_int, [vp]),
        "fb_fem_cut": (C.c_int, [vp, C.c_int, _dp, C.c_int, C.c_int, C.POINTER(CutResult)]),
        "fb_fem_read_cut": (C.c_int, [vp, _ip, _ip, _dp, _ip, _dp, _ip, _ip]),
        "fb_fem_read_mesh": (C.c_int, [vp, _dp, _ip]),
        "fb_fem_surface": (C.c_int, [vp, C.POINTER(SurfaceInfo)]),
        "fb_fem_read_surface": (C.c_int, [vp, _ip, _ip, _ip]),
        "fb_fem_surface_update": (C.c_int, [vp, _fp, _fp, C.POINTER(SurfaceInfo)]),
        "fb_fem_time_surface": (C.c_int, [vp, C.c_int, _dp, _dp]),
        "fb_fem_rebuild_elements": (C.c_int, [vp]),
        "fb_fem_set_external_forces": (C.c_int, [vp, _dp]),
        "fb_fem_add_external_forces": (C.c_int, [vp, _dp]),
        "fb_fem_set_external_forces_zero": (C.c_int, [vp]),
        "fb_fem_set_uniform_force": (C.c_int, [vp, C.c_int, C.c_double]),
        "fb_fem_step": (C.c_int, [vp, C.POINTER(StepInfo)]),
        "fb_fem_get_state": (C.c_int, [vp, _dp, _dp, _dp]),
        "fb_fem_set_state": (C.c_int, [vp, _dp, _dp, _dp]),
        "fb_fem_reset": (C.c_int, [vp]),
        "fb_fem_set_timestep": (C.c_int, [vp, C.c_double]),
        "fb_fem_set_damping": (C.c_int, [vp, C.c_double, C.c_double]),
        "fb_fem_set_internal_force_scaling": (C.c_int, [vp, C.c_double]),
        "fb_fem_set_cg": (C.c_int, [vp, C.c_double, C.c_int]),
        "fb_fem_set_constrained_dofs": (C.c_int, [vp, C.c_int, _ip]),
        "fb_fem_floor_collision": (C.c_int, [vp, C.c_double, C.c_double, _ip]),
        "fb_fem_add_haptic_forces": (C.c_int, [vp, C.c_int, _ip, _dp, C.c_int]),
        "fb_fem_pick_vertex": (C.c_int, [vp, _dp, _ip, _dp, _dp]),
        "fb_fem_pick_box": (C.c_int, [vp, _dp, _dp, C.c_int, _ip, _dp, _ip]),
        "fb_fem_volume": (C.c_int, [vp, _dp, _dp]),
        "fb_fem_num_nodes": (C.c_int, [vp]),
        "fb_fem_num_tets": (C.c_int, [vp]),
        "fb_fem_num_blocks": (C.c_int, [vp]),
        "fb_fem_matrix_precision": (C.c_int, [vp]),
        "fb_fem_owned_range": (C.c_int, [vp, C.POINTER(C.c_int)]),
        "fb_fem_pattern": (C.c_int, [vp, _ip, _ip]),
        "fb_fem_element_stiffness": (C.c_int, [vp, C.c_int, C.c_int, _dp, _dp]),
        "fb_fem_assemble": (C.c_int, [vp, _dp, _dp, _dp]),
        "fb_fem_system": (C.c_int, [vp, _dp, _dp]),
        "fb_fem_mass": (C.c_int, [vp, _dp]),
        "fb_fem_spmv": (C.c_int, [vp, _dp, _dp]),
        "fb_fem_pcg": (C.c_int, [vp, _dp, _dp, C.c_double, C.c_int, _ip]),
        "fb_fem_time_spmv": (C.c_int, [vp, C.c_int, _dp]),
        "fb_fem_time_assembly": (C.c_int, [vp, C.c_int, _dp]),
        "fb_fem_spmv_bytes": (C.c_int, [vp, _dp]),
        "fb_fem_assembly_bytes": (C.c_int, [vp, _dp]),
        "fb_fem_set_newmark": (C.c_int, [vp, C.c_double, C.c_double, C.c_int, C.c_double]),
        "fb_fem_persist_info": (C.c_int, [vp, _ip, _ip, _ip]),
        "fb_fem_pcg_path": (C.c_int, [vp, C.c_char_p, C.c_int, _ip, _ip, _ip]),
        "fb_fem_persist_stats": (C.c_int, [vp, _ip, _dp, C.POINTER(C.c_longlong)]),
        "fb_fem_time_persist": (C.c_int, [vp, C.c_int, C.c_int, _dp]),
        "fb_fem_iteration_bytes": (C.c_int, [vp, _dp]),
        "fb_comm_unique_id": (C.c_int, [_bp]),
        "fb_comm_create": (C.c_int, [C.POINTER(vp), C.c_int, C.c_int, _bp, C.c_int]),
        "fb_comm_destroy": (C.c_int, [vp]),
        "fb_comm_info": (C.c_int, [vp, _ip, _ip, _ip]),
        "fb_comm_create_local": (C.c_int, [C.POINTER(vp), C.c_int, C.c_int, C.c_char_p, C.c_size_t, C.c_int]),
        "fb_comm_test_allgather": (C.c_int, [vp, C.c_void_p, C.c_void_p, C.c_size_t]),
        "fb_fem_create_from_poly": (C.c_int, [C.POINTER(vp), vp, C.c_int, _ip, C.POINTER(FemParams)]),
        "fb_fem_device_plan_get": (C.c_longlong, [vp, C.c_char_p, _ip, C.c_longlong]),
        "fb_fem_plan_on_device": (C.c_int, [vp]),
        "fb_fem_assembly_kernel": (C.c_int, [vp]),
        "fb_fem_assembly_wide_slices": (C.c_int, [vp]),
        "fb_plan_create": (C.c_int, [C.POINTER(vp), C.c_int, C.c_int, _ip, C.c_int, _ip, C.c_int, C.c_int, _ip]),
        "fb_plan_destroy": (C.c_int, [vp]),
        "fb_plan_slab_order": (C.c_int, [C.c_int, _dp, C.c_int, _ip, _ip, _ip, _ip]),
        "fb_plan_shard_vote": (C.c_int, [C.c_int, C.c_int, _ip, C.c_int, C.c_int, _ip, _ip]),
        "fb_plan_info": (C.c_int, [vp, _ip]),
        "fb_plan_get": (C.c_int, [vp, C.c_char_p, _ip, C.c_size_t]),
        "fb_plan_mirror_model": (C.c_int, [vp, C.c_int, C.c_int, C.c_int, _ip]),
    }
    poly_sig = {
        "fb_fem_transport": (C.c_int, [vp]),
        "fb_fem_set_exchange_mode": (C.c_int, [vp, C.c_int]),
        "fb_fem_persist_rearms": (C.c_int, [vp]),
        "fb_fem_persist_helpers": (C.c_int, [vp]),
        "fb_fem_persist_gather": (C.c_int, [vp, C.POINTER(C.c_double), C.POINTER(C.c_double)]),
        "fb_fem_persist_mirror": (C.c_int, [vp, _ip, _ip, _ip]),
        "fb_fem_renumbering": (C.c_int, [vp, _ip, _ip]),
        "fb_fem_owned_nodes": (C.c_int, [vp, _ip]),
        "fb_fem_halo_info": (C.c_int, [vp, _ip, _ip]),
        "fb_fem_sharded_persist": (C.c_int, [vp]),
        "fb_fem_set_sharded_persist": (C.c_int, [vp, C.c_int]),
        "fb_fem_time_exchange": (C.c_int, [vp, C.c_int, _dp, _dp]),
        "fb_fem_time_element_stiffness": (C.c_int, [vp, C.c_int, _dp]),
        "fb_poly_create": (C.c_int, [C.POINTER(vp), C.c_int, _fp, C.c_int, _fp, C.c_int, _fp, C.c_int, _fp]),
        "fb_poly_destroy": (C.c_int, [vp]),
        "fb_poly_field_array": (C.c_int, [vp, C.c_int, _fp]),
        "fb_poly_set_field_semantics": (C.c_int, [vp, C.c_int, _fp]),
        "fb_poly_field_semantics": (C.c_int, [vp]),
        "fb_poly_sweep": (C.c_int, [vp, C.c_float, _ip]),
        "fb_poly_sweep_grid": (C.c_int, [vp, _fp, C.c_float, _ip]),
        "fb_poly_read_grid": (C.c_int, [vp, _fp]),
        "fb_poly_classify": (C.c_int, [vp, C.POINTER(PolyCounts)]),
        "fb_poly_read_classification": (C.c_int, [vp, _bp, _up, _bp]),
        "fb_poly_tetrahedralize": (C.c_int, [vp, C.POINTER(PolyCounts)]),
        "fb_poly_read_tetmesh": (C.c_int, [vp, _fp, _up]),
        "fb_poly_time_pipeline": (C.c_int, [vp, C.c_int, _dp, _dp]),
        "fb_poly_time_grid": (C.c_int, [vp, C.c_int, _dp]),
        "fb_poly_time_stages": (C.c_int, [vp, C.c_int, _dp]),
        "fb_poly_surface": (C.c_int, [vp, C.POINTER(PolyCounts)]),
        "fb_poly_read_surface": (C.c_int, [vp, _fp, _fp, _up]),
        "fb_poly_cube_table": (C.c_int, [_bp, _bp]),
        "fb_poly_time_surface": (C.c_int, [vp, C.c_int, _dp]),
        "fb_poly_off_surface": (C.c_int, [vp, C.c_float, _fp]),
        "fb_poly_read_surface_colors": (C.c_int, [vp, _fp]),
        "fb_poly_field_color_array": (C.c_int, [vp, C.c_int, _fp, _fp]),
        "fb_poly_interpolate_displacements": (C.c_int, [vp, C.c_int, _dp, _fp]),
        "fb_poly_read_surface_binding": (C.c_int, [vp, _up, _fp]),
        "fb_poly_compile_info": (C.c_int, [C.c_int, _fp, C.c_int, _fp, _ip, _ip]),
        "fb_poly_apply_displacements": (C.c_int, [vp, C.c_int, C.c_int, _dp, _fp]),
        "fb_poly_sweep_slab": (C.c_int, [vp, _fp, C.c_float, _ip, C.c_int, C.c_int]),
        "fb_poly_slab_counts": (C.c_int, [vp, C.c_int, C.c_int, C.c_int, _ip, _ip]),
        "fb_poly_read_tetmesh_slab": (C.c_int, [vp, C.c_int, C.c_int, C.c_int, C.c_uint, _fp, _up]),
        "fb_cut_create": (C.c_int, [C.POINTER(vp), C.c_int, C.c_int, _dp, C.c_int, _up]),
        "fb_cut_destroy": (None, [vp]),
        "fb_cut_set_vertices": (C.c_int, [vp, C.c_int, _dp]),
        "fb_cut_face_centroids": (C.c_int, [vp]),
        "fb_cut_face_intersections": (C.c_int, [vp, _dp, _dp, _ip]),
        "fb_cut_edge_intersections": (C.c_int, [vp, _dp, _ip]),
        "fb_cut_read": (C.c_int, [vp, C.c_int, _up, _fp]),
        "fb_cut_read_hits": (C.c_int, [vp, C.c_int, C.c_int, _up, _fp, _ip]),
        "fb_cut_segment_triangles": (C.c_int, [C.c_int, C.c_int, _fp, _fp, _fp, _fp]),
        "fb_cut_time": (C.c_int, [vp, C.c_int, _dp, _dp, C.c_int, _dp]),
    }
    sig.update(poly_sig)
    for name, (res, args) in sig.items():
        fn = getattr(L, name)
        fn.restype = res
        fn.argtypes = args
    _lib = L
    return L


def check(code):
    if code != FB_OK:
        raise FbError(code, lib().fb_last_error().decode("utf-8", "replace"))


def dptr(a):
    return None if a is None else a.ctypes.data_as(_dp)


def fptr(a):
    return None if a is None else a.ctypes.data_as(_fp)


def iptr(a):
    return None if a is None else a.ctypes.data_as(_ip)


def uptr(a):
    return None if a is None else a.ctypes.data_as(_up)


def bptr(a):
    return None if a is None else a.ctypes.data_as(_bp)


def as_f64(a, n=None):
    a = np.ascontiguousarray(a, dtype=np.float64).reshape(-1)
    if n is not None and a.size != n:
        raise ValueError("expected %d values, got %d" % (n, a.size))
    return a


def as_i32(a):
    return np.ascontiguousarray(a, dtype=np.int32).reshape(-1)
```

### include/fembrain_hip.h

```cpp
#ifndef FEMBRAIN_HIP_H
#define FEMBRAIN_HIP_H

#ifdef __cplusplus
extern "C" {
#endif

#define FB_OK 0
#define FB_EINVAL (-1)
#define FB_EDEVICE (-2)
#define FB_ENOMEM (-3)
#define FB_ESOLVER (-4)
#define FB_ECOMM (-5)

#define FB_MATRIX_F32 0
#define FB_MATRIX_F64 1
#define FB_MATRIX_AUTO 2

#define FB_PCG_MERGED 0
#define FB_PCG_REFERENCE 1
#define FB_PCG_PERSISTENT 3
#define FB_PCG_BLOCK_JACOBI 4

const char* fb_last_error(void);
int fb_device_count(void);
// ... 12 lines not shown
  int cg_max_iter;
  int matrix_precision;
  int device;
  int pcg_variant;
  int spmv_kernel;
  int linear;
  int exact_tangent;
  int integrator;
  int renumber;
  int expect_cuts;
  int reserve_nodes;
  int reserve_elements;
} fb_fem_params;
#define FB_RENUMBER_AUTO 0
#define FB_RENUMBER_ON 1
#define FB_RENUMBER_OFF (-1)
#define FB_INTEGRATOR_VOLUME_CONSERVING 0
#define FB_INTEGRATOR_NEWMARK 1
#define FB_SPMV_ROWS 1
#define FB_SPMV_SPLIT 2

void fb_fem_default_params(fb_fem_params* p);

int fb_fem_create(fb_fem_t* out, int n_nodes, const double* xyz, int n_tets, const int* tets,
                  int n_fixed_dofs, const int* fixed_dofs, const fb_fem_params* params);

typedef struct fb_comm_s* fb_comm_t;
int fb_fem_create_sharded(fb_fem_t* out, int n_nodes, const double* xyz, int n_tets, const int* tets,
                          int n_fixed_dofs, const int* fixed_dofs, const fb_fem_params* params,
                          int n_ranks, int rank, const int* node_splits, fb_comm_t comm);
int fb_fem_destroy(fb_fem_t h);
#define FB_XCH_COLLECTIVE 1
#define FB_XCH_P2P 2
#define FB_XCH_P2P_SUMS 3
#define FB_XCH_P2P_FUSED 4
int fb_fem_transport(fb_fem_t h);
int fb_fem_set_exchange_mode(fb_fem_t h, int mode);
int fb_fem_sharded_persist(fb_fem_t h);
int fb_fem_set_sharded_persist(fb_fem_t h, int on);

int fb_fem_resync(fb_fem_t h, int n_nodes, const double* xyz, int n_tets, const int* tets,
                  int n_fixed_dofs, const int* fixed_dofs);
int fb_fem_resync_sharded(fb_fem_t h, int n_nodes, const double* xyz, int n_tets, const int* tets,
                          int n_fixed_dofs, const int* fixed_dofs, const int* node_splits);

#define FB_RESYNC_FULL 0
#define FB_RESYNC_DELTA_MERGED 1
#define FB_RESYNC_DELTA_REBUILT 2
int fb_fem_resync_delta(fb_fem_t h, int n_removed, const int* removed, int n_changed, const int* changed_ids, const int* changed_nodes,
                        int n_added, const int* added_tets, int n_new_nodes, const double* new_xyz, int n_fixed_dofs, const int* fixed_dofs);
int fb_fem_resync_path(fb_fem_t h);

#define FB_CUT_BAKE 0
#define FB_CUT_CARRY 1
#define FB_CUT_NOTHING 0
#define FB_CUT_DONE 1
#define FB_CUT_UNHANDLED 2
#define FB_CUT_DRY 3
typedef struct fb_cut_result {
  int status;
  int n_quads;
  int n_cut_edges;
  int n_case_a, n_case_b;
  int n_unhandled;
  int n_removed, n_added, n_new_nodes;
  double min_volume_ratio;
} fb_cut_result;
int fb_fem_cut(fb_fem_t h, int n_strip_points, const double* strip_xyz, int mode, int modify, fb_cut_result* out);
int fb_fem_read_cut(fb_fem_t h, int* removed, int* added_tets, double* new_xyz, int* edge_nodes, double* edge_frac, int* unhandled_ids, int* unhandled_codes);
int fb_fem_read_mesh(fb_fem_t h, double* rest_xyz, int* tets);

typedef struct fb_fem_surface_info {
  int n_faces, n_vertices, n_builds;
  float aabb_lo[3], aabb_hi[3];
} fb_fem_surface_info;
int fb_fem_surface(fb_fem_t h, fb_fem_surface_info* out);
int fb_fem_read_surface(fb_fem_t h, int* faces, int* vertex_ids, int* face_tets);
int fb_fem_surface_update(fb_fem_t h, float* xyz, float* normals, fb_fem_surface_info* out);
int fb_fem_time_surface(fb_fem_t h, int reps, double* seconds_build, double* seconds_update);


int fb_fem_rebuild_elements(fb_fem_t h);

int fb_fem_set_external_forces(fb_fem_t h, const double* f);
int fb_fem_add_external_forces(fb_fem_t h, const double* f);
int fb_fem_set_external_forces_zero(fb_fem_t h);
int fb_fem_set_uniform_force(fb_fem_t h, int axis, double value);

typedef struct fb_step_info {
  int cg_iterations;
  int converged;
  double assembly_seconds;
  double solve_seconds;
  double rho0, rho;
  int pcg_path;
  int persist_fallbacks;
  int newton_iterations;
} fb_step_info;
#define FB_PCG_PATH_TWO_LAUNCH 0
#define FB_PCG_PATH_PERSISTENT 1
#define FB_PCG_PATH_FALLBACK 2
#define FB_PCG_PATH_RESOLVED 3

int fb_fem_step(fb_fem_t h, fb_step_info* info);

int fb_fem_get_state(fb_fem_t h, double* q, double* qvel, double* qaccel);
int fb_fem_set_state(fb_fem_t h, const double* q, const double* qvel, const double* qaccel);
int fb_fem_reset(fb_fem_t h);
int fb_fem_set_timestep(fb_fem_t h, double timestep);
int fb_fem_set_damping(fb_fem_t h, double damping_mass, double damping_stiffness);
int fb_fem_set_internal_force_scaling(fb_fem_t h, double factor);
int fb_fem_set_cg(fb_fem_t h, double eps, int max_iter);
int fb_fem_set_newmark(fb_fem_t h, double beta, double gamma, int max_newton_iterations, double epsilon);
int fb_fem_set_constrained_dofs(fb_fem_t h, int n_fixed_dofs, const int* fixed_dofs);

int fb_fem_floor_collision(fb_fem_t h, double floor_y, double restitution, int* n_collided);

#define FB_HAPTIC_MAX_SOURCES 256
int fb_fem_add_haptic_forces(fb_fem_t h, int n, const int* node_ids, const double* forces3, int neighbourhood_size);
int fb_fem_pick_vertex(fb_fem_t h, const double wpos[3], int* index, double xyz[3], double* dist2);
int fb_fem_pick_box(fb_fem_t h, const double lo[3], const double hi[3], int capacity, int* ids, double* xyz, int* n_found);
int fb_fem_volume(fb_fem_t h, double* total, double* per_element);

int fb_fem_num_nodes(fb_fem_t h);
int fb_fem_num_tets(fb_fem_t h);
int fb_fem_num_blocks(fb_fem_t h);
int fb_fem_matrix_precision(fb_fem_t h);
int fb_fem_owned_range(fb_fem_t h, int lo_hi[2]);
int fb_fem_renumbering(fb_fem_t h, int* span_caller, int* span_internal);
int fb_fem_halo_info(fb_fem_t h, int* n_halo_nodes, int* n_neighbour_ranks);
int fb_fem_owned_nodes(fb_fem_t h, int* ids);
int fb_fem_pattern(fb_fem_t h, int* bptr, int* bcol);
int fb_fem_element_stiffness(fb_fem_t h, int first, int count, double* K0, double* Minv);
int fb_fem_assemble(fb_fem_t h, const double* u, double* f, double* K_blocks);
int fb_fem_system(fb_fem_t h, double* Keff_blocks, double* rhs);
int fb_fem_mass(fb_fem_t h, double* m_blocks);
int fb_fem_spmv(fb_fem_t h, const double* x, double* y);
int fb_fem_pcg(fb_fem_t h, const double* rhs, double* x, double eps, int max_iter, int* iterations_out);

long long fb_fem_device_plan_get(fb_fem_t h, const char* name, int* out, long long capacity);
int fb_fem_plan_on_device(fb_fem_t h);
int fb_fem_assembly_kernel(fb_fem_t h);
int fb_fem_assembly_wide_slices(fb_fem_t h);
int fb_fem_time_spmv(fb_fem_t h, int reps, double* seconds_per_spmv);
int fb_fem_time_assembly(fb_fem_t h, int reps, double* seconds_per_assembly);
int fb_fem_time_exchange(fb_fem_t h, int reps, double* seconds_per_halo, double* seconds_per_sum);
int fb_fem_time_element_stiffness(fb_fem_t h, int reps, double* seconds_per_pass);
int fb_fem_persist_info(fb_fem_t h, int* waves_per_cu, int* workgroups, int* lds_slots);
int fb_fem_pcg_path(fb_fem_t h, char* name, int name_len, int* persist_launches, int* persist_fallbacks, int* max_producers);
int fb_fem_persist_rearms(fb_fem_t h);
int fb_fem_persist_helpers(fb_fem_t h);
int fb_fem_persist_gather(fb_fem_t h, double* lines_planes, double* lines_records);
int fb_fem_persist_mirror(fb_fem_t h, int* mirror_layers, int* pool_entries, int* plain_slots);
int fb_fem_time_persist(fb_fem_t h, int reps, int n_iters, double* seconds_per_launch);
int fb_fem_persist_stats(fb_fem_t h, int* launches, double* seconds, long long* iterations);
int fb_fem_iteration_bytes(fb_fem_t h, double* bytes);
int fb_fem_spmv_bytes(fb_fem_t h, double* bytes);
int fb_fem_assembly_bytes(fb_fem_t h, double* bytes);

int fb_comm_unique_id(unsigned char id[128]);
int fb_comm_create(fb_comm_t* out, int rank, int n_ranks, const unsigned char id[128], int device);
int fb_comm_destroy(fb_comm_t c);
int fb_comm_info(fb_comm_t c, int* ranks, int* rccl_ranks, int* transport);

typedef struct fb_poly_s* fb_poly_t;

int fb_poly_create(fb_poly_t* out, int device, const float* header12, int n_ops, const float* ops16,
                   int n_prims, const float* prims20, int n_mtx, const float* mtx12);
int fb_poly_destroy(fb_poly_t h);

#define FB_FIELD_CPU 0
#define FB_FIELD_CPU_BOX 1
#define FB_FIELD_OPENCL 2
int fb_poly_set_field_semantics(fb_poly_t h, int semantics, const float* prim_boxes6);
int fb_poly_field_semantics(fb_poly_t h);

int fb_poly_field_array(fb_poly_t h, int n, float* xyzf);

int fb_poly_sweep(fb_poly_t h, float cellsize, int dims_out[3]);
int fb_poly_sweep_grid(fb_poly_t h, const float lower[3], float cellsize, const int dims[3]);
int fb_poly_read_grid(fb_poly_t h, float* xyzf);

typedef struct fb_poly_counts {
  int grid[3];
  int n_points, n_cells;
  int n_crossed_edges;
  int n_surface_cells;
  int n_included_cells;
  int n_tet_vertices;
  int n_tets;
  int n_surface_vertices;
  int n_surface_indices;
} fb_poly_counts;

int fb_poly_classify(fb_poly_t h, fb_poly_counts* counts);
int fb_poly_read_classification(fb_poly_t h, unsigned char* edge_flags, unsigned int* edge_counts,
                                unsigned char* cell_configs);
int fb_poly_tetrahedralize(fb_poly_t h, fb_poly_counts* counts);
int fb_poly_read_tetmesh(fb_poly_t h, float* xyz, unsigned int* tets);

int fb_poly_surface(fb_poly_t h, fb_poly_counts* counts);
int fb_poly_read_surface(fb_poly_t h, float* xyz, float* normals, unsigned int* indices);
int fb_poly_cube_table(unsigned char tri[4096], unsigned char nvert[256]);

#define FB_MESH_SURFACE 0
#define FB_MESH_TET 1
int fb_poly_apply_displacements(fb_poly_t h, int mesh, int n_dof, const double* displacements, float* xyz_out);

int fb_poly_interpolate_displacements(fb_poly_t h, int n_tet_dof, const double* tet_displacements, float* xyz_out);
int fb_poly_read_surface_binding(fb_poly_t h, unsigned int* tet_vertex_pairs, float* weights);

int fb_poly_read_surface_colors(fb_poly_t h, float* rgba);
int fb_poly_field_color_array(fb_poly_t h, int n, float* xyzf, float* rgb);
int fb_poly_off_surface(fb_poly_t h, float len, float* xyzf_pairs);
int fb_poly_time_surface(fb_poly_t h, int reps, double* seconds);
int fb_poly_time_pipeline(fb_poly_t h, int reps, double* sweep_seconds, double* pipeline_seconds);
int fb_poly_time_grid(fb_poly_t h, int reps, double* sweep_and_grid_seconds);
int fb_poly_time_stages(fb_poly_t h, int reps, double seconds[5]);

int fb_fem_create_from_poly(fb_fem_t* out, fb_poly_t poly, int n_fixed_dofs, const int* fixed_dofs, const fb_fem_params* params);

int fb_poly_sweep_slab(fb_poly_t h, const float lower[3], float cellsize, const int dims[3], int z_first, int z_count);
int fb_poly_slab_counts(fb_poly_t h, int own_first_plane, int own_planes, int own_layers, int* n_vertices, int* n_tets);
int fb_poly_read_tetmesh_slab(fb_poly_t h, int own_first_plane, int own_planes, int own_layers, unsigned int vertex_base, float* xyz, unsigned int* tets);

typedef struct fb_cut_s* fb_cut_t;
#define FB_CUT_FACES 0
#define FB_CUT_EDGES 1
int fb_cut_create(fb_cut_t* out, int device, int n_vertices, const double* xyz, int n_tets, const unsigned int* tets);
void fb_cut_destroy(fb_cut_t h);
int fb_cut_set_vertices(fb_cut_t h, int n_vertices, const double* xyz);
int fb_cut_face_centroids(fb_cut_t h);
int fb_cut_face_intersections(fb_cut_t h, const double* s0, const double* s1, int* n_hits);
int fb_cut_edge_intersections(fb_cut_t h, const double* quad12, int* n_hits);
int fb_cut_read(fb_cut_t h, int what, unsigned int* flags, float* points_xyzw);
int fb_cut_read_hits(fb_cut_t h, int what, int capacity, unsigned int* ids, float* points_xyzw, int* n_out);
int fb_cut_segment_triangles(int device, int n_tris, const float* tri_xyzw, const float* s0, const float* s1, float* points_xyzw);
int fb_cut_time(fb_cut_t h, int what, const double* a, const double* b, int reps, double* ms_per_pass);

#ifdef __cplusplus
}
#endif
#endif
```

### include/fembrain_hip_testing.h

```cpp
#ifndef FEMBRAIN_HIP_TESTING_H
#define FEMBRAIN_HIP_TESTING_H
#include <stddef.h>
#ifdef __cplusplus
extern "C" {
#endif

typedef struct fb_plan_s* fb_plan_t;

int fb_plan_create(fb_plan_t* out, int n_nodes, int n_tets, const int* tets, int n_fixed_dofs, const int* fixed_dofs,
                   int n_ranks, int rank, const int* node_splits);
int fb_plan_destroy(fb_plan_t p);
int fb_plan_info(fb_plan_t p, int info[12]);
int fb_plan_get(fb_plan_t p, const char* name, int* out, size_t capacity);

int fb_plan_mirror_model(fb_plan_t p, int nb, int c16, int klt, int out[4]);

int fb_plan_slab_order(int n_nodes, const double* xyz, int n_tets, const int* tets, int* old_of_new, int* span_caller, int* span_internal);

int fb_plan_shard_vote(int n_nodes, int n_tets, const int* tets, int n_ranks, int rank, const int* node_splits, int out[3]);

struct fb_comm_s;
int fb_comm_create_local(struct fb_comm_s** out, int rank, int n_ranks, const char* shm_name, size_t outbox_bytes, int device);
int fb_comm_test_allgather(struct fb_comm_s* c, const void* mine, void* all, size_t bytes);

int fb_poly_compile_info(int n_ops, const float* ops16, int n_prims, const float* prims20, int* n_steps, int* n_slots);

#ifdef __cplusplus
}
#endif
#endif
```

Measured before the change: 67.08.

## Alias symmetric upper-triangle SpMV blocks to transposed mirrored blocks in persistent PCG

Adds a planning pass that, for streamed slots after the mirrored window, maps each lane's 3x3 block to the transposed block already stored for the symmetric partner row. When a whole slot layer can be aliased, the persistent PCG SpMV loads values through the alias index with a transposed register order. The goal is better cache reuse of matrix values shared across symmetric pairs, which cuts unique HBM traffic. The cost is an extra alias-index load per slot, more inline-asm branching, and plan-time kernels. A diagnostic API and a host model are also added.

```diff
diff --git a/fembrain_amd/csrc/fem_handle.h b/fembrain_amd/csrc/fem_handle.h
--- a/fembrain_amd/csrc/fem_handle.h
+++ b/fembrain_amd/csrc/fem_handle.h
@@ -16,6 +16,7 @@
 
 struct PersistState {
   int pipe_mir_knob = -1;
+  int pipe_alias_knob = -1;
   int persist_fallbacks = 0;
   int persist_launches = 0;
   int persist_rearms = 0;
@@ -49,6 +50,8 @@
   long long sbox_halo_cap = 0;
   int pipe_mir_got[3] = {0, 0, 0};
   bool pipe_mir_pending = false;
+  int pipe_alias_got[2] = {0, 0};
+  bool pipe_alias_pending = false;
 
   DevBuf<int> pipe_wg_first;
   std::vector<int> pipe_wg_first_host;
@@ -61,7 +64,9 @@
   DevBuf<unsigned short> pipe_mir_addr;
   DevBuf<int2> pipe_mir_wg;
   DevBuf<int> pipe_mir_pool;
-  DevBuf<int> pipe_mir_stats;
+  DevBuf<unsigned int> pipe_alias, pipe_alias_mask;
+  DevBuf<int> pipe_alias_win;
+  DevBuf<int> pipe_mir_stats, pipe_alias_stats;
   DevBuf<unsigned long long> pipe_lines;
   DevBuf<unsigned long long> pipe_post;
   DevBuf<unsigned int> pipe_flags;
@@ -78,6 +83,8 @@
     kernel = nullptr;
     pipe_mir.release(); pipe_mir_pending = false;
     pipe_mir_got[0] = pipe_mir_got[1] = pipe_mir_got[2] = 0;
+    pipe_alias.release(); pipe_alias_pending = false;
+    pipe_alias_got[0] = pipe_alias_got[1] = 0;
     shard_persist = false;
     persist_broken = false;
     pipe_stats_pending = false;
diff --git a/fembrain_amd/csrc/fem_persist.hip b/fembrain_amd/csrc/fem_persist.hip
--- a/fembrain_amd/csrc/fem_persist.hip
+++ b/fembrain_amd/csrc/fem_persist.hip
@@ -70,6 +70,7 @@
   k.lds_cap = getenv("FEMBRAIN_PIPE_LDS_CAP") ? std::max(1, env_int("FEMBRAIN_PIPE_LDS_CAP", 1)) : 0;
   k.plain_stores = env_int("FEMBRAIN_PIPE_PLAIN_STORES", -1);
   k.mirror = env_int("FEMBRAIN_PIPE_MIRROR", 1) != 0;
+  k.alias = env_int("FEMBRAIN_PIPE_ALIAS", 1) != 0;
   k.verbose = getenv("FEMBRAIN_TIMING") != nullptr;
   return k;
 }
@@ -162,6 +163,9 @@
   const PipeKernel& K = *ps.kernel;
   ps.pipe_mir_pending = false;
   ps.pipe_mir_got[0] = ps.pipe_mir_got[1] = ps.pipe_mir_got[2] = 0;
+  ps.pipe_alias_pending = false;
+  ps.pipe_alias_got[0] = ps.pipe_alias_got[1] = 0;
+  ps.pipe_alias.release(); ps.pipe_alias_mask.release(); ps.pipe_alias_win.release();
   if (ps.pipe_mir_knob == 0 || K.rows != 1 || K.wmax != 12 || K.shard || K.help || K.bj || ps.pipe_xyz || P.n_slices <= 0) {
     ps.pipe_mir.release(); ps.pipe_mir_addr.release(); ps.pipe_mir_wg.release(); ps.pipe_mir_pool.release();
     return FB_OK;
@@ -178,6 +182,21 @@
                      h->c16 ? 1 : 0, ps.pipe_mir.p, ps.pipe_mir_addr.p, ps.pipe_mir_pool.p, ps.pipe_mir_wg.p, ps.pipe_mir_stats.p);
   FB_HIP(hipGetLastError());
   ps.pipe_mir_pending = true;
+  if (ps.pipe_alias_knob == 0 || P.n_slots <= 0) return FB_OK;
+  FB_TRY(ps.pipe_alias.alloc((size_t)P.n_slots * 64));
+  FB_TRY(ps.pipe_alias_mask.alloc((size_t)P.n_slices));
+  FB_TRY(ps.pipe_alias_win.alloc((size_t)P.n_slices));
+  FB_TRY(ps.pipe_alias_stats.alloc(2));
+  FB_HIP(hipMemsetAsync(ps.pipe_alias.p, 0, (size_t)P.n_slots * 64 * sizeof(unsigned int), s));
+  FB_HIP(hipMemsetAsync(ps.pipe_alias_mask.p, 0, (size_t)P.n_slices * sizeof(unsigned int), s));
+  FB_HIP(hipMemsetAsync(ps.pipe_alias_win.p, 0, (size_t)P.n_slices * sizeof(int), s));
+  FB_HIP(hipMemsetAsync(ps.pipe_alias_stats.p, 0, 2 * sizeof(int), s));
+  hipLaunchKernelGGL(k_pipe_alias_win, dim3(nb), dim3(64 * kMirWaves), 0, s, P.n_slices, ps.pipe_wg_first.p, ps.pipe_mir.p, ps.pipe_alias_win.p);
+  FB_HIP(hipGetLastError());
+  hipLaunchKernelGGL(k_pipe_alias_plan, dim3(nb), dim3(64 * kMirWaves), 0, s, P.n_slices, P.n_owned, h->slice_off.p, h->colidx.p, ps.pipe_wg_first.p,
+                     ps.pipe_alias_win.p, ps.pipe_alias.p, ps.pipe_alias_mask.p, ps.pipe_alias_stats.p);
+  FB_HIP(hipGetLastError());
+  ps.pipe_alias_pending = true;
   return FB_OK;
 }
 
@@ -304,6 +323,7 @@
   PersistState& ps = h->ps;
   const PersistKnobs kn = read_persist_knobs();
   if (ps.pipe_mir_knob < 0) ps.pipe_mir_knob = kn.mirror ? 1 : 0;
+  if (ps.pipe_alias_knob < 0) ps.pipe_alias_knob = kn.alias ? 1 : 0;
   ps.pipe_timing_level = kn.timing;
   ps.reset_plan(kn.rearm);
   hipDeviceProp_t prop;
@@ -425,6 +445,7 @@
   pa.tasks = ps.pipe_tasks.p; pa.n_help = ps.pipe_n_help;
   pa.wg_first = ps.pipe_wg_first.p;
   pa.mirror = ps.pipe_mir.p; pa.mir_addr = ps.pipe_mir_addr.p; pa.mir_wg = ps.pipe_mir_wg.p; pa.mir_pool = ps.pipe_mir_pool.p;
+  pa.alias = ps.pipe_mir.p ? ps.pipe_alias.p : nullptr; pa.alias_mask = ps.pipe_alias_mask.p;
   const int cwaves = K.rows == 2 ? ceil_div(ps.persist_waves, 2) : ps.persist_waves;
   pa.service = cwaves + ps.pipe_help_waves < ps.pipe_wmax ? 1 : 0;
   pa.prefetch_slots = ps.persist_waves >= 9 ? (K.rows == 2 ? 3 : 4) : 0;
@@ -605,6 +626,17 @@
 
 int fb_fem_persist_rearms(fb_fem_t h) { return h ? h->ps.persist_rearms : 0; }
 int fb_fem_persist_helpers(fb_fem_t h) { return h && h->ps.persist ? h->ps.pipe_help_tasks : 0; }
+int fb_fem_persist_alias(fb_fem_t h, int* alias_layers, int* slices_with_alias) {
+  if (!h) return fail(FB_EINVAL, "null FEM handle");
+  if (h->ps.pipe_alias_pending) {
+    FB_TRY(h->ps.pipe_alias_stats.download(h->ps.pipe_alias_got, 2, h->stream));
+    h->ps.pipe_alias_pending = false;
+  }
+  const bool on = h->ps.persist && h->ps.pipe_mir.p && h->ps.pipe_alias.p;
+  if (alias_layers) *alias_layers = on ? h->ps.pipe_alias_got[0] : 0;
+  if (slices_with_alias) *slices_with_alias = on ? h->ps.pipe_alias_got[1] : 0;
+  return on && h->ps.pipe_alias_got[0] > 0 ? 1 : 0;
+}
 int fb_fem_persist_mirror(fb_fem_t h, int* mirror_layers, int* pool_entries, int* plain_slots) {
   if (!h) return fail(FB_EINVAL, "null FEM handle");
   if (h->ps.pipe_mir_pending) {
diff --git a/fembrain_amd/csrc/pcg_pipe.hip.h b/fembrain_amd/csrc/pcg_pipe.hip.h
--- a/fembrain_amd/csrc/pcg_pipe.hip.h
+++ b/fembrain_amd/csrc/pcg_pipe.hip.h
@@ -3,6 +3,7 @@
 #include "pcg_pipe_stream.hip.h"
 #include "pcg_pipe_onchip.hip.h"
 #include "pcg_pipe_mirror.h"
+#include "pcg_pipe_alias.h"
 
 namespace fb {
 
@@ -46,6 +47,8 @@
   const unsigned short* mir_addr;
   const int2* mir_wg;
   const int* mir_pool;
+  const unsigned int* alias;
+  const unsigned int* alias_mask;
 };
 constexpr int kPipeTaskStride = 16;
 constexpr int kPipeTimingSlots = 8;
@@ -243,6 +246,36 @@
   }
   if (w < kMirWaves && lane == 0)
     wave_out[(size_t)b * kMirWaves + w] = w < count ? make_int4(mw[w].a | mw[w].m << 8 | mw[w].p << 16, mw[w].at, mw[w].tab, 0) : make_int4(0, 0, 0, 0);
+}
+
+__global__ __launch_bounds__(64 * kMirWaves) void k_pipe_alias_win(int n_slices, const int* __restrict__ wg_first, const int4* __restrict__ mirror, int* __restrict__ win) {
+  const int b = blockIdx.x, nb = gridDim.x, lane = threadIdx.x & 63, w = threadIdx.x >> 6;
+  int first, count;
+  pipe_deal(wg_first, n_slices, nb, b, &first, &count);
+  if (w < min(count, kMirWaves) && lane == 0) win[first + w] = alias_win(mirror[(size_t)b * kMirWaves + w].x, b);
+}
+__global__ __launch_bounds__(64 * kMirWaves) void k_pipe_alias_plan(int n_slices, int n_owned, const int* __restrict__ slice_off, const int* __restrict__ colidx,
+                                                                  const int* __restrict__ wg_first, const int* __restrict__ win, unsigned int* __restrict__ alias,
+                                                                  unsigned int* __restrict__ alias_mask, int* __restrict__ stats) {
+  const int b = blockIdx.x, nb = gridDim.x, lane = threadIdx.x & 63, w = threadIdx.x >> 6;
+  int first, count;
+  pipe_deal(wg_first, n_slices, nb, b, &first, &count);
+  if (w >= min(count, kMirWaves)) return;
+  const int sl = first + w, so = slice_off[sl], width = slice_off[sl + 1] - so, mt = win[sl];
+  const int k_after = (mt & 0xff) + ((mt >> 8) & 0xff) + ((mt >> 16) & 0xff);
+  unsigned int mask = 0u;
+  for (int k = k_after; k < width; k++) {
+    const long long own = ((long long)so + k) * 9 * 64 + lane;
+    long long word = k - k_after < kAliasMaskSlots ? alias_lane_word(slice_off, colidx, win, sl, k, lane, n_owned, b & 7) : -1;
+    if (word >= (1LL << 30)) word = -1;
+    const bool all = __ballot(word < 0) == 0ULL;
+    alias[((size_t)so + k) * 64 + lane] = (unsigned int)(all ? word : own);
+    if (all) mask |= 1u << (k - k_after);
+  }
+  if (lane == 0) {
+    alias_mask[sl] = mask;
+    if (mask) { atomicAdd(&stats[0], __popc(mask)); atomicAdd(&stats[1], 1); }
+  }
 }
 
 __device__ __forceinline__ void pipe_collect_posts(const PipeArgs& pa, unsigned int sums, int nb, int lane, int stride, int l0, long long t0, long long t_limit, bool& failed,
@@ -371,6 +404,10 @@
     }
   }
   const int kp = mir_a + mir_m, k_after = kp + klt_w;
+  unsigned int alias_bits = 0u;
+  if constexpr (kMir) {
+    if (pa.alias) alias_bits = (unsigned int)__builtin_amdgcn_readfirstlane(live ? (int)pa.alias_mask[sl] : 0);
+  }
   const int KL = min(klt_w, width - kp);
   constexpr int kValWords = C16 ? 9 : 10;
   char* lwave = (char*)(lds + kPipeSyncDoubles) + (size_t)lres_at * pipe_slot_bytes(C16);
@@ -599,7 +636,17 @@
         seam(6, tseam);
       }
       const int n_str = own_k1 - k_after;
-      if (n_str > 0) {
+      bool aliased = false;
+      if constexpr (kMir) {
+        aliased = pa.alias != nullptr;
+        if (aliased && n_str > 0) {
+          int so_k = so + k_after;
+          asm volatile("" : "+s"(so_k));
+          pipe_stream_alias_slots<C16>(n_str, ((unsigned int)so_k * 64u + (unsigned int)lane) * (unsigned int)(C16 ? sizeof(short) : sizeof(int)), vals,
+                                       C16 ? (const void*)sv.coldelta : (const void*)sv.colidx, pa.alias, alias_bits, pl, pl + xs, pl + 2 * xs, row, y0, y1, y2);
+        }
+      }
+      if (!aliased && n_str > 0) {
         int so_k = so + k_after;
         asm volatile("" : "+s"(so_k));
         pipe_stream_slots<C16, XYZ>(n_str, ((unsigned int)so_k * 9u * 64u + (unsigned int)lane) * (unsigned int)sizeof(float),
diff --git a/fembrain_amd/csrc/pcg_pipe_alias.h b/fembrain_amd/csrc/pcg_pipe_alias.h
--- /dev/null
+++ b/fembrain_amd/csrc/pcg_pipe_alias.h
@@ -0,0 +1,28 @@
+#pragma once
+#include "pcg_pipe_mirror.h"
+
+namespace fb {
+
+constexpr int kAliasMaskSlots = 32;
+
+__host__ __device__ inline int alias_win(int amp, int b) { return (amp & 0xffffff) | (b & 7) << 24; }
+
+__host__ __device__ inline long long alias_lane_word(const int* slice_off, const int* colidx, const int* win, int sl, int k, int lane, int n_owned, int share) {
+  const int row = sl * 64 + lane;
+  const long long slot = slice_off[sl] + k;
+  if (row >= n_owned) return slot * 9 * 64 + lane;
+  const int c = colidx[(size_t)slot * 64 + lane];
+  if (c == row) {
+    const int dk = mir_lane_diag(slice_off, colidx, sl, lane, n_owned);
+    return dk >= 0 && dk < k ? slot * 9 * 64 + lane : -1;
+  }
+  if (c < row || c >= n_owned) return -1;
+  const int s2 = c >> 6, l2 = c & 63, w2 = win[s2];
+  if (share >= 0 && ((w2 >> 24) & 0xff) != share) return -1;
+  const int a2 = w2 & 0xff;
+  for (int j = 0; j < a2; j++)
+    if (colidx[(size_t)(slice_off[s2] + j) * 64 + l2] == row) return ((long long)slice_off[s2] + j) * 9 * 64 + l2;
+  return -1;
+}
+
+}
diff --git a/fembrain_amd/csrc/pcg_pipe_plan.h b/fembrain_amd/csrc/pcg_pipe_plan.h
--- a/fembrain_amd/csrc/pcg_pipe_plan.h
+++ b/fembrain_amd/csrc/pcg_pipe_plan.h
@@ -29,6 +29,7 @@
   int lds_cap = 0;
   int plain_stores = -1;
   bool mirror = true;
+  bool alias = true;
   bool verbose = false;
 };
 
diff --git a/fembrain_amd/csrc/pcg_pipe_stream.hip.h b/fembrain_amd/csrc/pcg_pipe_stream.hip.h
--- a/fembrain_amd/csrc/pcg_pipe_stream.hip.h
+++ b/fembrain_amd/csrc/pcg_pipe_stream.hip.h
@@ -103,6 +103,72 @@
   ".Lfbp_odd_last_%=:\n\t"                                                                                      \
   FBP_LAST(FBP_COMPUTE_B)                                                                                       \
   ".Lfbp_end_%=:\n\t"
+#define FBA_LOADV9(base, r0, r1, r2, r3, r4, r5, r6, r7, r8)               \
+  "global_load_dword " r0 ", " base ", %[svals]\n\t"                       \
+  "global_load_dword " r1 ", " base ", %[svals] offset:256\n\t"            \
+  "global_load_dword " r2 ", " base ", %[svals] offset:512\n\t"            \
+  "global_load_dword " r3 ", " base ", %[svals] offset:768\n\t"            \
+  "global_load_dword " r4 ", " base ", %[svals] offset:1024\n\t"           \
+  "global_load_dword " r5 ", " base ", %[svals] offset:1280\n\t"           \
+  "global_load_dword " r6 ", " base ", %[svals] offset:1536\n\t"           \
+  "global_load_dword " r7 ", " base ", %[svals] offset:1792\n\t"           \
+  "global_load_dword " r8 ", " base ", %[svals] offset:2048\n\t"
+#define FBA_LOADV(TAG, base, r0, r1, r2, r3, r4, r5, r6, r7, r8)           \
+  "v_lshlrev_b32_e32 " base ", 2, " base "\n\t"                            \
+  "s_bitcmp1_b32 %[amask], 0\n\t"                                         \
+  "s_cbranch_scc1 .Lfba_t" TAG "_%=\n\t"                                  \
+  FBA_LOADV9(base, r0, r1, r2, r3, r4, r5, r6, r7, r8)                     \
+  "s_branch .Lfba_j" TAG "_%=\n"                                          \
+  ".Lfba_t" TAG "_%=:\n\t"                                                \
+  FBA_LOADV9(base, r0, r3, r6, r1, r4, r7, r2, r5, r8)                     \
+  ".Lfba_j" TAG "_%=:\n\t"                                                \
+  "s_lshr_b32 %[amask], %[amask], 1\n\t"
+#define FBA_LOADV_A(TAG) FBA_LOADV(TAG, "%[aa]", "v136", "v137", "v138", "v139", "v140", "v141", "v142", "v143", "v144")
+#define FBA_LOADV_B(TAG) FBA_LOADV(TAG, "%[ab]", "v145", "v146", "v147", "v148", "v149", "v150", "v151", "v152", "v153")
+#define FBA_LOADCA16(c, a) "v_lshlrev_b32_e32 v123, 1, %[coff]\n\t" "global_load_sshort " c ", %[coff], %[scols]\n\t" "global_load_dword " a ", v123, %[salias]\n\t" "v_add_u32_e32 %[coff], 0x80, %[coff]\n\t"
+#define FBA_LOADCA32(c, a) "global_load_dword " c ", %[coff], %[scols]\n\t" "global_load_dword " a ", %[coff], %[salias]\n\t" "v_add_u32_e32 %[coff], 0x100, %[coff]\n\t"
+#define FBA_BODY(LOADCA, GOFF)                                                                                   \
+  "s_nop 4\n\t"                                                                                                 \
+  LOADCA("v154", "%[aa]")                                                                                       \
+  "s_cmp_lt_i32 %[n], 2\n\t"                                                                                    \
+  "s_cbranch_scc1 .Lfba_one_%=\n\t"                                                                             \
+  LOADCA("v155", "%[ab]")                                                                                       \
+  "s_waitcnt vmcnt(2)\n\t"                                                                                      \
+  FBA_LOADV_A("0")                                                                                              \
+  "s_branch .Lfba_g0_%=\n"                                                                                      \
+  ".Lfba_one_%=:\n\t"                                                                                           \
+  "s_waitcnt vmcnt(0)\n\t"                                                                                      \
+  FBA_LOADV_A("1")                                                                                              \
+  ".Lfba_g0_%=:\n\t"                                                                                            \
+  GOFF("v154") FBP_GATHER_A                                                                                     \
+  ".Lfba_even_%=:\n\t"                                                                                          \
+  "s_cmp_lt_i32 %[n], 3\n\t"                                                                                    \
+  "s_cbranch_scc1 .Lfba_even_tail_%=\n\t"                                                                       \
+  LOADCA("v154", "%[aa]") "s_waitcnt vmcnt(14)\n\t" FBA_LOADV_B("2") GOFF("v155") FBP_GATHER_B "s_waitcnt vmcnt(14)\n\t" FBP_COMPUTE_A \
+  "s_sub_i32 %[n], %[n], 1\n\t"                                                                                 \
+  "s_cmp_lt_i32 %[n], 3\n\t"                                                                                    \
+  "s_cbranch_scc1 .Lfba_odd_tail_%=\n\t"                                                                        \
+  LOADCA("v155", "%[ab]") "s_waitcnt vmcnt(14)\n\t" FBA_LOADV_A("3") GOFF("v154") FBP_GATHER_A "s_waitcnt vmcnt(14)\n\t" FBP_COMPUTE_B \
+  "s_sub_i32 %[n], %[n], 1\n\t"                                                                                 \
+  "s_branch .Lfba_even_%=\n"                                                                                    \
+  ".Lfba_even_tail_%=:\n\t"                                                                                     \
+  "s_cmp_lt_i32 %[n], 2\n\t"                                                                                    \
+  "s_cbranch_scc1 .Lfba_even_last_%=\n\t"                                                                       \
+  "s_waitcnt vmcnt(12)\n\t" FBA_LOADV_B("4") GOFF("v155") FBP_GATHER_B "s_waitcnt vmcnt(12)\n\t" FBP_COMPUTE_A    \
+  FBP_LAST(FBP_COMPUTE_B)                                                                                       \
+  "s_branch .Lfba_end_%=\n"                                                                                     \
+  ".Lfba_even_last_%=:\n\t"                                                                                     \
+  FBP_LAST(FBP_COMPUTE_A)                                                                                       \
+  "s_branch .Lfba_end_%=\n"                                                                                     \
+  ".Lfba_odd_tail_%=:\n\t"                                                                                      \
+  "s_cmp_lt_i32 %[n], 2\n\t"                                                                                    \
+  "s_cbranch_scc1 .Lfba_odd_last_%=\n\t"                                                                        \
+  "s_waitcnt vmcnt(12)\n\t" FBA_LOADV_A("5") GOFF("v154") FBP_GATHER_A "s_waitcnt vmcnt(12)\n\t" FBP_COMPUTE_B    \
+  FBP_LAST(FBP_COMPUTE_A)                                                                                       \
+  "s_branch .Lfba_end_%=\n"                                                                                     \
+  ".Lfba_odd_last_%=:\n\t"                                                                                      \
+  FBP_LAST(FBP_COMPUTE_B)                                                                                       \
+  ".Lfba_end_%=:\n\t"
 #define FBP_CLOBBERS                                                                                                                   \
   "memory", "scc", "v120", "v121", "v122", "v123", "v124", "v125", "v126", "v127", "v128", "v129", "v130", "v131", "v132", "v133",      \
   "v134", "v135", "v136", "v137", "v138", "v139", "v140", "v141", "v142", "v143", "v144", "v145", "v146", "v147", "v148", "v149",      \
@@ -169,4 +235,24 @@
   }
 }
 
-}
+template <bool C16>
+__device__ __forceinline__ void pipe_stream_alias_slots(int n, unsigned int coff, const float* vals, const void* cols, const unsigned int* alias, unsigned int amask,
+                                                        const double* pl0, const double* pl1, const double* pl2, int row, double& y0, double& y1, double& y2) {
+  vals = scalar_ptr(vals); cols = scalar_ptr(cols); alias = scalar_ptr(alias); pl0 = scalar_ptr(pl0); pl1 = scalar_ptr(pl1); pl2 = scalar_ptr(pl2);
+  n = __builtin_amdgcn_readfirstlane(n);
+  amask = (unsigned int)__builtin_amdgcn_readfirstlane((int)amask);
+  unsigned int aa, ab;
+  if (C16) {
+    asm volatile(FBA_BODY(FBA_LOADCA16, FBP_GOFF16)
+                 : [y0] "+v"(y0), [y1] "+v"(y1), [y2] "+v"(y2), [coff] "+v"(coff), [n] "+s"(n), [amask] "+s"(amask), [aa] "=&v"(aa), [ab] "=&v"(ab)
+                 : [svals] "s"(vals), [scols] "s"(cols), [salias] "s"(alias), [spl0] "s"(pl0), [spl1] "s"(pl1), [spl2] "s"(pl2), [row] "v"(row)
+                 : FBP_CLOBBERS);
+  } else {
+    asm volatile(FBA_BODY(FBA_LOADCA32, FBP_GOFF32)
+                 : [y0] "+v"(y0), [y1] "+v"(y1), [y2] "+v"(y2), [coff] "+v"(coff), [n] "+s"(n), [amask] "+s"(amask), [aa] "=&v"(aa), [ab] "=&v"(ab)
+                 : [svals] "s"(vals), [scols] "s"(cols), [salias] "s"(alias), [spl0] "s"(pl0), [spl1] "s"(pl1), [spl2] "s"(pl2), [row] "v"(row)
+                 : FBP_CLOBBERS);
+  }
+}
+
+}
diff --git a/fembrain_amd/csrc/plan_api.cpp b/fembrain_amd/csrc/plan_api.cpp
--- a/fembrain_amd/csrc/plan_api.cpp
+++ b/fembrain_amd/csrc/plan_api.cpp
@@ -7,6 +7,7 @@
 #include "fem_plan.h"
 #include "renumber.h"
 #include "pcg_pipe_mirror.h"
+#include "pcg_pipe_alias.h"
 
 namespace fb {
 int fail(int code, const char* fmt, ...);
@@ -91,9 +92,7 @@
   return FB_OK;
 }
 
-int fb_plan_mirror_model(fb_plan_t p, int nb, int c16, int klt, int out[4]) {
-  if (!p || !out || nb < 8 || (nb & 7) || (klt != 6 && klt != 7)) return fb::fail(FB_EINVAL, "bad argument");
-  const fb::FemPlan& P = p->plan;
+static void mirror_model(const fb::FemPlan& P, int nb, int c16, int klt, int out[4], std::vector<int>* win) {
   const int* so = P.slice_off.data();
   const int* ci = P.colidx.data();
   out[0] = out[1] = out[3] = 0;
@@ -140,8 +139,51 @@
     if (ok) { E = misses(); ok = fb::mir_wg_gains(mw, count, klt, c16 != 0); }
     if (!ok) { fb::mir_wg_plain(mw, count, klt, c16 != 0); E = 0; }
     for (int w = 0; w < count; w++) { out[0] += mw[w].m; out[2] = std::min(out[2], mw[w].p); }
+    if (win)
+      for (int w = 0; w < count; w++) (*win)[first + w] = fb::alias_win(mw[w].a | mw[w].m << 8 | mw[w].p << 16, b);
     out[1] += E;
     out[3] += ok ? 1 : 0;
+  }
+}
+int fb_plan_mirror_model(fb_plan_t p, int nb, int c16, int klt, int out[4]) {
+  if (!p || !out || nb < 8 || (nb & 7) || (klt != 6 && klt != 7)) return fb::fail(FB_EINVAL, "bad argument");
+  mirror_model(p->plan, nb, c16, klt, out, nullptr);
+  return FB_OK;
+}
+
+int fb_plan_alias_model(fb_plan_t p, int nb, int c16, int klt, int same_share, int out[2], int* windows) {
+  if (!p || !out || nb < 8 || (nb & 7) || (klt != 6 && klt != 7)) return fb::fail(FB_EINVAL, "bad argument");
+  const fb::FemPlan& P = p->plan;
+  std::vector<int> win(P.n_slices, 0);
+  int mo[4];
+  mirror_model(P, nb, c16, klt, mo, &win);
+  const int* so = P.slice_off.data();
+  const int* ci = P.colidx.data();
+  out[0] = out[1] = 0;
+  if (windows)
+    for (int sl = 0; sl < P.n_slices; sl++) { windows[3 * sl] = win[sl] & 0xff; windows[3 * sl + 1] = (win[sl] >> 8) & 0xff; windows[3 * sl + 2] = (win[sl] >> 16) & 0xff; }
+  for (int b = 0; b < nb; b++) {
+    const int xcd = b & 7, j = b >> 3, per = nb >> 3, chunk = (P.n_slices + 7) >> 3, lo_s = xcd * chunk;
+    int len = P.n_slices - lo_s;
+    len = len < 0 ? 0 : (len > chunk ? chunk : len);
+    const int base = len / per, rem = len - base * per;
+    const int first = lo_s + j * base + (j < rem ? j : rem);
+    const int count = std::min(base + (j < rem ? 1 : 0), fb::kMirWaves);
+    for (int w = 0; w < count; w++) {
+      const int sl = first + w, mt = win[sl], width = so[sl + 1] - so[sl];
+      const int k_after = (mt & 0xff) + ((mt >> 8) & 0xff) + ((mt >> 16) & 0xff);
+      int layers = 0;
+      for (int k = k_after; k < width && k - k_after < fb::kAliasMaskSlots; k++) {
+        bool all = true;
+        for (int l = 0; l < 64 && all; l++) {
+          const long long word = fb::alias_lane_word(so, ci, win.data(), sl, k, l, P.n_owned, same_share ? (b & 7) : -1);
+          all = word >= 0 && word < (1LL << 30);
+        }
+        layers += all ? 1 : 0;
+      }
+      out[0] += layers;
+      out[1] += layers > 0 ? 1 : 0;
+    }
   }
   return FB_OK;
 }
diff --git a/fembrain_amd/fem.py b/fembrain_amd/fem.py
--- a/fembrain_amd/fem.py
+++ b/fembrain_amd/fem.py
@@ -369,6 +369,13 @@
             _l.check(on)
         return bool(on == 1), m.value, p.value, k.value
 
+    def persist_alias(self):
+        a, n = C.c_int(0), C.c_int(0)
+        on = self._L.fb_fem_persist_alias(self.h, C.byref(a), C.byref(n))
+        if on < 0:
+            _l.check(on)
+        return a.value, n.value
+
     def pcg_path(self):
         name = C.create_string_buffer(96)
         nl, nf, mp = C.c_int(0), C.c_int(0), C.c_int(0)
diff --git a/fembrain_amd/lib.py b/fembrain_amd/lib.py
--- a/fembrain_amd/lib.py
+++ b/fembrain_amd/lib.py
@@ -180,6 +180,7 @@
         "fb_plan_info": (C.c_int, [vp, _ip]),
         "fb_plan_get": (C.c_int, [vp, C.c_char_p, _ip, C.c_size_t]),
         "fb_plan_mirror_model": (C.c_int, [vp, C.c_int, C.c_int, C.c_int, _ip]),
+        "fb_plan_alias_model": (C.c_int, [vp, C.c_int, C.c_int, C.c_int, C.c_int, _ip, _ip]),
     }
     poly_sig = {
         "fb_fem_transport": (C.c_int, [vp]),
@@ -188,6 +189,7 @@
         "fb_fem_persist_helpers": (C.c_int, [vp]),
         "fb_fem_persist_gather": (C.c_int, [vp, C.POINTER(C.c_double), C.POINTER(C.c_double)]),
         "fb_fem_persist_mirror": (C.c_int, [vp, _ip, _ip, _ip]),
+        "fb_fem_persist_alias": (C.c_int, [vp, _ip, _ip]),
         "fb_fem_renumbering": (C.c_int, [vp, _ip, _ip]),
         "fb_fem_owned_nodes": (C.c_int, [vp, _ip]),
         "fb_fem_halo_info": (C.c_int, [vp, _ip, _ip]),
diff --git a/include/fembrain_hip.h b/include/fembrain_hip.h
--- a/include/fembrain_hip.h
+++ b/include/fembrain_hip.h
@@ -188,6 +188,7 @@
 int fb_fem_persist_helpers(fb_fem_t h);
 int fb_fem_persist_gather(fb_fem_t h, double* lines_planes, double* lines_records);
 int fb_fem_persist_mirror(fb_fem_t h, int* mirror_layers, int* pool_entries, int* plain_slots);
+int fb_fem_persist_alias(fb_fem_t h, int* alias_layers, int* slices_with_alias);
 int fb_fem_time_persist(fb_fem_t h, int reps, int n_iters, double* seconds_per_launch);
 int fb_fem_persist_stats(fb_fem_t h, int* launches, double* seconds, long long* iterations);
 int fb_fem_iteration_bytes(fb_fem_t h, double* bytes);
diff --git a/include/fembrain_hip_testing.h b/include/fembrain_hip_testing.h
--- a/include/fembrain_hip_testing.h
+++ b/include/fembrain_hip_testing.h
@@ -14,6 +14,7 @@
 int fb_plan_get(fb_plan_t p, const char* name, int* out, size_t capacity);
 
 int fb_plan_mirror_model(fb_plan_t p, int nb, int c16, int klt, int out[4]);
+int fb_plan_alias_model(fb_plan_t p, int nb, int c16, int klt, int same_share, int out[2], int* windows);
 
 int fb_plan_slab_order(int n_nodes, const double* xyz, int n_tets, const int* tets, int* old_of_new, int* span_caller, int* span_internal);
 
```

Result: slower. 64.85 (-3.3%).
